# cheukwaylee/ORB_SLAM2_detailed_comments

Hardware: AMD Instinct MI355X
Metric: frames/sec ORB extract+match (1000 kp, 640x480) (higher is better)
Workload: dtype u8; 1 GPU; synthetic 640x480 mono stream, nFeatures=1000, 8 levels, scale 1.2, FAST 20/7, extract+match(t vs t-1), batch 1024 frames/GPU resident in HBM, 1 pipelines/GPU; parallelism=single GPU

## Files before the change

orb_slam2_detailed_comments_amd/csrc/orbx_api.cpp:

```cpp
#include <hip/hip_runtime.h>
#include <dlfcn.h>
#include <cstdio>
#include <cstdlib>
#include <cstring>
#include <string>
#include <vector>
#include <algorithm>
#include "orbx_internal.h"
#include "orbx_launch.h"
#include "orbx_gate.h"

static thread_local std::string g_last_error;
static orbx_status fail(orbx_status s, const std::string &msg) {
    g_last_error = msg;
    return s;
}
#define HIPCHK(expr)                                                                              \
    do {                                                                                          \
        hipError_t _e = (expr);                                                                   \
        if (_e != hipSuccess)                                                                     \
            return fail(ORBX_HIP_ERROR, std::string(#expr) + ": " + hipGetErrorString(_e));      \
    } while (0)

struct ProfPair { hipEvent_t a, b; int kid; };

struct orbx_handle {
    orbx_params p;
    OrbxTables tab;
    OrbxGeom geom;
    DGeom dg;
    bool host_only = false, configured = false;
    int dev = 0;
    hipStream_t own_stream = nullptr, stream = nullptr;
    hipStream_t side_stream = nullptr;
    hipEvent_t ev_fork = nullptr, ev_join = nullptr;
    hipEvent_t ev_stereo = nullptr;
    int fork_level = 0;
    int fork_group = 0;
    int pipeline = 2;
    bool pipe_head = true;
    bool fast_room = false;
    hipEvent_t ev_pipe[ORBX_PIPE_MAX] = {};
    uint8_t *d_pyr = nullptr, *d_blur = nullptr;
    OrbxCell *d_cells = nullptr;
    OrbxFastGroup *d_groups = nullptr;
    bool resize_legacy = false;
    int match_kernel = 0;
    int fast_stop = 0;
    int fast_lcap = 640;
    OrbxTap *d_taps = nullptr;
    uint2 *d_dense = nullptr;
    int *d_cand_count = nullptr, *d_lvl_count = nullptr, *d_status = nullptr;
    uint32_t *d_lvl_kp = nullptr;
    float *d_lvl_angle = nullptr;
    uint16_t *d_knode = nullptr;
    int max_cw = 0, max_ch = 0, ncap = 0, lds_keys = 0, lds_keys_few = 0;
    uint8_t *st_in[2] = {nullptr, nullptr}; size_t d_in_bytes = 0;
    orbx_keypoint *st_kps[2] = {nullptr, nullptr}; uint8_t *st_desc[2] = {nullptr, nullptr}; int *st_cnt[2] = {nullptr, nullptr};
    int out_cap = 0, stage_chunk = 0;
    int *pin_stat = nullptr; size_t pin_stat_ints = 0;
    hipStream_t s_in = nullptr;
    hipEvent_t ev_in[2] = {nullptr, nullptr}, ev_done[2] = {nullptr, nullptr}, ev_out[2] = {nullptr, nullptr};
    int last_batch = 0;
    int mk_w = 0, mk_h = 0, mk_total = 0;
    void *d_match_ws = nullptr; size_t match_ws_bytes = 0;
    uint32_t *d_gate_items = nullptr; size_t gate_items_cap = 0;
    uint8_t *pin = nullptr; size_t pin_bytes = 0;
    size_t gate_guess = 4096;
    uint8_t *d_scratch = nullptr; size_t scratch_bytes = 0, scratch_used = 0;
    uint2 *d_rect = nullptr; int rect_w = 0, rect_h = 0;
    int input_format = ORBX_FMT_GRAY8;
    bool blur_valid = false;
    uint32_t prof_mask = 0;
    std::vector<ProfPair> pending;
    std::vector<hipEvent_t> pool;
    float ms[ORBX_K_COUNT] = {0};
    int launches[ORBX_K_COUNT] = {0};
};

orbx_status orbx_fail(orbx_status s, const std::string &msg) { return fail(s, msg); }
int orbx_handle_fp_mode(const orbx_handle *h) { return h->p.fp_mode; }

static const char *k_names[ORBX_K_COUNT] = {"k_pyr_l0", "k_pyr_resize", "k_fast_rows", "k_quadtree", "k_orient",
                                            "k_blur",   "k_describe",   "k_match",      "misc"};

extern "C" const char *orbx_kernel_name(int k) { return (k >= 0 && k < ORBX_K_COUNT) ? k_names[k] : "?"; }
extern "C" const char *orbx_last_error(void) { return g_last_error.c_str(); }
extern "C" int orbx_abi_version(void) { return ORBX_ABI_VERSION; }
extern "C" const char *orbx_status_string(orbx_status s) {
    switch (s) {
        case ORBX_OK: return "ok";
        case ORBX_EMPTY_IMAGE: return "empty image";
        case ORBX_BAD_ARGUMENT: return "bad argument";
        case ORBX_BAD_ASPECT: return "bad aspect ratio (nIni == 0)";
        case ORBX_CAPACITY: return "capacity exceeded";
// ... 14 lines not shown

struct Roctx {
    int (*push)(const char *) = nullptr;
    int (*pop)() = nullptr;
    Roctx() {
        const char *e = getenv("ORBX_ROCTX");
        if (!e || !atoi(e)) return;
        void *lib = dlopen("librocprofiler-sdk-roctx.so", RTLD_NOW | RTLD_GLOBAL);
        if (!lib) lib = dlopen("libroctx64.so", RTLD_NOW | RTLD_GLOBAL);
        if (!lib) return;
        push = (int (*)(const char *))dlsym(lib, "roctxRangePushA");
        pop = (int (*)())dlsym(lib, "roctxRangePop");
        if (!push || !pop) push = nullptr, pop = nullptr;
    }
};
static const Roctx &roctx() { static Roctx r; return r; }

struct ProfScope {
    orbx_handle *h; int kid; bool on; hipStream_t st; hipEvent_t a = nullptr, b = nullptr; bool marked = false;
    ProfScope(orbx_handle *h_, int kid_, hipStream_t st_ = nullptr)
        : h(h_), kid(kid_), on(((h_->prof_mask >> kid_) & 1u) != 0), st(st_ ? st_ : h_->stream) {
        if (roctx().push) { roctx().push(orbx_kernel_name(kid)); marked = true; }
        if (!on) return;
        a = grab(); b = grab();
        hipEventRecord(a, st);
    }
    hipEvent_t grab() {
        if (!h->pool.empty()) { hipEvent_t e = h->pool.back(); h->pool.pop_back(); return e; }
        hipEvent_t e; hipEventCreate(&e); return e;
    }
    ~ProfScope() {
        if (marked) roctx().pop();
        if (!on) return;
        hipEventRecord(b, st);
        h->pending.push_back({a, b, kid});
    }
};

static void prof_drain(orbx_handle *h) {
    if (h->pending.empty()) return;
    hipStreamSynchronize(h->stream);
    for (auto &pp : h->pending) {
        float ms = 0;
        if (hipEventElapsedTime(&ms, pp.a, pp.b) == hipSuccess) { h->ms[pp.kid] += ms; h->launches[pp.kid]++; }
        h->pool.push_back(pp.a); h->pool.push_back(pp.b);
    }
    h->pending.clear();
}

static orbx_status pin_reserve(orbx_handle *h, size_t bytes);

static void free_geometry_buffers(orbx_handle *h) {
    hipFree(h->d_groups); h->d_groups = nullptr;
    hipFree(h->d_pyr); hipFree(h->d_blur); hipFree(h->d_cells); hipFree(h->d_taps);
    hipFree(h->d_dense); h->d_dense = nullptr;
    hipFree(h->d_cand_count); hipFree(h->d_lvl_count); hipFree(h->d_status); hipFree(h->d_lvl_kp);
    hipFree(h->d_lvl_angle); hipFree(h->d_knode);
    h->d_pyr = h->d_blur = nullptr; h->d_cells = nullptr; h->d_taps = nullptr;
    h->d_cand_count = h->d_lvl_count = h->d_status = nullptr; h->d_lvl_kp = nullptr; h->d_lvl_angle = nullptr;
    h->d_knode = nullptr;
    h->configured = false;
}

static orbx_status configure(orbx_handle *h, int width, int height) {
    if (h->configured && h->geom.width == width && h->geom.height == height) return ORBX_OK;
    if (h->host_only) return fail(ORBX_NO_DEVICE, "host-only handle (device = -2) cannot extract");
    HIPCHK(hipSetDevice(h->dev));
    if (h->configured) {
        HIPCHK(hipStreamSynchronize(h->stream));
        if (h->side_stream) HIPCHK(hipStreamSynchronize(h->side_stream));
        free_geometry_buffers(h);
    }
    const char *why = "";
    OrbxGeom g;
    orbx_status st = orbx_build_geometry(h->p, h->tab, width, height, g, &why);
    if (st != ORBX_OK) return fail(st, why);
    h->geom = g;
    const int B = h->p.max_batch, NL = h->p.nlevels;
    DGeom &d = h->dg;
    memset(&d, 0, sizeof(d));
    d.nlevels = NL; d.ncells = (int)g.cells.size(); d.kp_total = g.kp_total; d.fp_mode = h->p.fp_mode;
    d.ini_th = std::min(std::max(h->p.ini_th_fast, 0), 255);
    d.min_th = std::min(std::max(h->p.min_th_fast, 0), 255);
    d.pyr_bytes = g.pyr_bytes; d.cand_total = g.cand_total;
    for (int i = 0; i < 16; ++i) d.umax[i] = h->tab.umax[i];
    int tiles = 0;
    h->max_cw = h->max_ch = 7;
    for (const auto &c : g.cells) { h->max_cw = std::max<int>(h->max_cw, c.cw); h->max_ch = std::max<int>(h->max_ch, c.ch); }
    for (int l = 0; l < NL; ++l) {
        const OrbxLevelGeom &L = g.lv[l];
        DLevel &D = d.lv[l];
        D.pw = L.pw; D.ph = L.ph; D.pitch = L.pitch; D.sw = L.sw; D.sh = L.sh;
        D.cell_begin = L.cell_begin; D.cell_count = L.cell_count;
        D.qt_w = L.qt_w; D.qt_h = L.qt_h; D.nini = L.nini; D.hx = L.hx;
        D.nfeat = L.nfeat; D.kp_cap = L.kp_cap; D.kp_begin = L.kp_begin; D.cand_cap = L.cand_cap;
        D.tapx = L.tapx_begin; D.tapy = L.tapy_begin; D.scale = L.scale; D.size = L.size;
        D.off = L.off; D.cand_begin = L.cand_begin;
        D.blur_tx = (L.pw + 127) / 128;
        D.blur_tile_begin = tiles;
        tiles += D.blur_tx * ((L.ph + 31) / 32);
    }
    d.blur_tiles = tiles;
    h->ncap = g.node_cap;
    const size_t node_part = orbx_quadtree_smem(h->ncap, 0);
    if (node_part > 120 * 1024) return fail(ORBX_UNSUPPORTED, "nfeatures too large for the LDS quadtree node table");
    {
        const size_t want = std::min<size_t>({(size_t)4096, (size_t)g.max_cand_cap, (size_t)6 * (size_t)std::max(g.lv[0].nfeat, 1)});
        size_t keys = 0;
        auto fit_at = [&](int wg) -> size_t {
            const size_t budget = (size_t)(160 * 1024) / wg - 512;
            return budget <= node_part ? 0 : std::min<size_t>({(budget - node_part) / 6, (size_t)4096, (size_t)g.max_cand_cap});
        };
        size_t keys_few = 0;
        for (int wg = 4; wg >= 2 && keys == 0; --wg)
            if (fit_at(wg) >= want) { keys = std::max<size_t>(want, 1024); keys_few = fit_at(wg); }
        h->lds_keys_few = (int)keys_few;
        if (keys == 0 && fit_at(2) >= 1024) keys = fit_at(2);
        if (keys == 0) keys = fit_at(1);
        if (const char *e = getenv("ORBX_QT_LDS_KEYS")) keys = std::min<size_t>((size_t)std::max(atoi(e), 0), std::min<size_t>(8192, (160 * 1024 - node_part) / 6));
        h->lds_keys = (int)keys;
        if (getenv("ORBX_QT_LDS_KEYS") || h->lds_keys_few < h->lds_keys) h->lds_keys_few = h->lds_keys;
    }
    HIPCHK(orbx_quadtree_prepare(orbx_quadtree_smem(h->ncap, std::max(h->lds_keys, h->lds_keys_few))));
    if (const char *e = getenv("ORBX_RESIZE_IMPL")) h->resize_legacy = strcmp(e, "legacy") == 0;
#ifdef ORBX_TIMING_KNOBS
    if (const char *e = getenv("ORBX_FAST_STOP")) h->fast_stop = atoi(e);
#endif
    if (const char *e = getenv("ORBX_FAST_LCAP")) h->fast_lcap = std::max(64, atoi(e));
// ... 136 lines not shown
    if (inv_sigma2) memcpy(inv_sigma2, h->tab.inv_sigma2, n * sizeof(float));
    return ORBX_OK;
}
extern "C" orbx_status orbx_get_features_per_level(const orbx_handle *h, int32_t *n) {
    if (!h || !n) return fail(ORBX_BAD_ARGUMENT, "null argument");
    memcpy(n, h->tab.nfeat, h->p.nlevels * sizeof(int32_t));
    return ORBX_OK;
}
extern "C" orbx_status orbx_get_umax(const orbx_handle *h, int32_t *umax16) {
    if (!h || !umax16) return fail(ORBX_BAD_ARGUMENT, "null argument");
    memcpy(umax16, h->tab.umax, 16 * sizeof(int32_t));
    return ORBX_OK;
}
extern "C" int orbx_max_keypoints(orbx_handle *h, int width, int height) {
    if (!h || width <= 0 || height <= 0) return -(int)ORBX_BAD_ARGUMENT;
    if (h->configured && h->geom.width == width && h->geom.height == height) return h->geom.kp_total;
    if (h->mk_w == width && h->mk_h == height) return h->mk_total;
    OrbxGeom g; const char *why = "";
    const orbx_status st = orbx_build_geometry(h->p, h->tab, width, height, g, &why);
    if (st != ORBX_OK) { g_last_error = why; return -(int)st; }
    h->mk_w = width; h->mk_h = height; h->mk_total = g.kp_total;
    return g.kp_total;
}

static inline int orbx_fmt_channels(int fmt) { return fmt == ORBX_FMT_GRAY8 ? 1 : (fmt == ORBX_FMT_RGB8 || fmt == ORBX_FMT_BGR8) ? 3 : 4; }
extern "C" orbx_status orbx_set_rectification(orbx_handle *h, const float *map_x, const float *map_y, int width, int height) {
    if (!h || h->host_only) return fail(h ? ORBX_NO_DEVICE : ORBX_BAD_ARGUMENT, "no device handle");
    HIPCHK(hipSetDevice(h->dev));
    HIPCHK(hipStreamSynchronize(h->stream));
    hipFree(h->d_rect); h->d_rect = nullptr; h->rect_w = h->rect_h = 0;
    if (!map_x && !map_y) return ORBX_OK;
    if (!map_x || !map_y || width <= 0 || height <= 0) return fail(ORBX_BAD_ARGUMENT, "bad rectification maps");
    if (h->input_format != ORBX_FMT_GRAY8) return fail(ORBX_BAD_ARGUMENT, "rectification needs 8-bit gray input");
    std::vector<uint2> t((size_t)width * height);
    for (size_t i = 0; i < t.size(); ++i) {
        const int sx = (int)lrintf(map_x[i] * 32.f), sy = (int)lrintf(map_y[i] * 32.f);
        const int ix = std::min(std::max(sx >> 5, -32768), 32767), iy = std::min(std::max(sy >> 5, -32768), 32767);
        t[i].x = (uint32_t)(uint16_t)(int16_t)ix | ((uint32_t)(uint16_t)(int16_t)iy << 16);
        t[i].y = (uint32_t)(((sy & 31) << 5) | (sx & 31));
    }
    HIPCHK(hipMalloc(&h->d_rect, t.size() * sizeof(uint2)));
    HIPCHK(hipMemcpyAsync(h->d_rect, t.data(), t.size() * sizeof(uint2), hipMemcpyHostToDevice, h->stream));
    HIPCHK(hipStreamSynchronize(h->stream));
    h->rect_w = width; h->rect_h = height;
    return ORBX_OK;
}
extern "C" orbx_status orbx_set_input_format(orbx_handle *h, int pixel_format) {
    if (!h) return fail(ORBX_BAD_ARGUMENT, "null handle");
    if (pixel_format < ORBX_FMT_GRAY8 || pixel_format > ORBX_FMT_BGRA8) return fail(ORBX_BAD_ARGUMENT, "unknown pixel format");
    if (h->d_rect && pixel_format != ORBX_FMT_GRAY8) return fail(ORBX_BAD_ARGUMENT, "rectification needs 8-bit gray input");
    h->input_format = pixel_format;
    return ORBX_OK;
}
static orbx_status run_chunk(orbx_handle *h, int B, const uint8_t *d_imgs, int W, int H, int stride,
                             int64_t frame_stride, orbx_keypoint *d_kps, uint8_t *d_desc, int32_t *d_counts,
                             int32_t *d_status, int cap) {
    const DGeom &g = h->dg;
    hipStream_t s = h->stream;
    const int NL = g.nlevels;
    if (h->d_rect && (h->rect_w != W || h->rect_h != H))
        return fail(ORBX_BAD_ARGUMENT, "rectification maps were set for another image size (raw and rectified size must agree)");
    const int ngroups = (int)h->geom.fast_groups.size();
    auto pyramid = [&](hipStream_t st, int f0, int b, int l_end) {
        const uint8_t *im = d_imgs + (int64_t)f0 * frame_stride;
        uint8_t *pyr = h->d_pyr + (size_t)f0 * h->geom.pyr_bytes;
        int32_t *stp = d_status + f0;
        int *cc = h->d_cand_count + (size_t)f0 * NL;
        { ProfScope ps(h, ORBX_K_PYR_L0, st);
          if (h->d_rect) {
              orbx_launch_pyr_l0_remap(st, g, b, im, W, H, stride, frame_stride, pyr, h->d_rect, stp, cc);
          } else if (h->input_format == ORBX_FMT_GRAY8) {
              orbx_launch_pyr_l0(st, g, b, im, W, H, stride, frame_stride, pyr, stp, cc);
          } else {
              const int nch = (h->input_format == ORBX_FMT_RGB8 || h->input_format == ORBX_FMT_BGR8) ? 3 : 4;
              const bool rgb = h->input_format == ORBX_FMT_RGB8 || h->input_format == ORBX_FMT_RGBA8;
              orbx_launch_pyr_l0_color(st, g, b, im, W, H, stride, frame_stride, pyr, nch, rgb ? 0 : 2, rgb ? 2 : 0, stp, cc);
          } }
        for (int l = 1; l < l_end; ++l) {
            ProfScope ps(h, ORBX_K_PYR_RESIZE, st);
            orbx_launch_pyr_resize(st, g, b, l, h->d_taps, pyr, h->geom.lv[l].narrow_taps && !h->resize_legacy);
        }
    };
    auto fast = [&](hipStream_t st, int f0, int b, int g0, int ng, int lds_floor) {
        ProfScope ps(h, ORBX_K_FAST, st);
        orbx_launch_fast_rows(st, g, b, h->d_cells, h->d_groups + g0, ng, h->d_pyr + (size_t)f0 * h->geom.pyr_bytes,
                              h->d_dense + (size_t)f0 * g.cand_total, h->d_cand_count + (size_t)f0 * NL, d_status + f0, h->max_ch,
                              h->fast_lcap, h->fast_stop, lds_floor);
    };
    auto finish = [&](int f0, int b) {
        { ProfScope ps(h, ORBX_K_QUADTREE);
          orbx_launch_quadtree(s, g, b, h->d_dense + (size_t)f0 * g.cand_total, h->d_cand_count + (size_t)f0 * NL,
                               h->d_lvl_kp + (size_t)f0 * g.kp_total, h->d_lvl_count + (size_t)f0 * NL, d_status + f0,
                               h->d_knode + (size_t)f0 * g.cand_total, h->ncap, (long long)b * NL >= 1024 ? h->lds_keys : h->lds_keys_few, 0, NL); }
        { ProfScope ps(h, ORBX_K_DESC);
          orbx_launch_describe(s, g, b, h->d_pyr + (size_t)f0 * h->geom.pyr_bytes, h->d_lvl_kp + (size_t)f0 * g.kp_total,
                               h->d_lvl_count + (size_t)f0 * NL, h->d_lvl_angle + (size_t)f0 * g.kp_total, d_kps + (int64_t)f0 * cap,
                               d_desc + (int64_t)f0 * cap * 32, d_counts + f0, d_status + f0, cap); }
    };
    h->blur_valid = false;
    const int S = h->pipeline > 1 && B >= ORBX_PIPE_MIN_FRAMES && __builtin_popcount(h->prof_mask) <= 1 ? h->pipeline : 1;
    if (S > 1) {
        int off[ORBX_PIPE_MAX + 1];
        const int units = h->pipe_head ? 2 * S - 1 : S;
        off[0] = 0;
        for (int k = 0; k + 1 < S; ++k) {
            const int share = (int)((long long)B * (h->pipe_head && k > 0 ? 2 : 1) / units);
            off[k + 1] = off[k] + std::max(8, share & ~7);
        }
        off[S] = B;
        hipStream_t s2 = h->side_stream;
        if (hipEventRecord(h->ev_fork, s) != hipSuccess || hipStreamWaitEvent(s2, h->ev_fork, 0) != hipSuccess)
            { hipStreamSynchronize(s2); return fail(ORBX_HIP_ERROR, "pipeline fork event"); }
        for (int k = 0; k < S; ++k) {
            pyramid(s2, off[k], off[k + 1] - off[k], NL);
            if (hipEventRecord(h->ev_pipe[k], s2) != hipSuccess)
                { hipStreamSynchronize(s2); return fail(ORBX_HIP_ERROR, "pipeline event"); }
        }
        const int floor = h->fast_room ? ORBX_LDS_PER_CU / ORBX_FAST_PIPE_WAVES : 0;
        for (int k = 0; k < S; ++k) {
            if (hipStreamWaitEvent(s, h->ev_pipe[k], 0) != hipSuccess)
                { hipStreamSynchronize(s2); return fail(ORBX_HIP_ERROR, "pipeline event wait"); }
            fast(s, off[k], off[k + 1] - off[k], 0, ngroups, floor);
            finish(off[k], off[k + 1] - off[k]);
        }
        hipError_t e = hipGetLastError();
        if (e != hipSuccess) { hipStreamSynchronize(s2); return fail(ORBX_HIP_ERROR, std::string("kernel launch: ") + hipGetErrorString(e)); }
        h->last_batch = B;
        return ORBX_OK;
    }
    const bool fork = h->fork_level > 0 && (long long)B * ngroups >= 16384;
    pyramid(s, 0, B, fork ? h->fork_level : NL);
    if (fork) {
        hipStream_t s2 = h->side_stream;
        if (hipEventRecord(h->ev_fork, s) != hipSuccess || hipStreamWaitEvent(s2, h->ev_fork, 0) != hipSuccess)
            return fail(ORBX_HIP_ERROR, "fork event");
        for (int l = h->fork_level; l < NL; ++l) {
            ProfScope ps(h, ORBX_K_PYR_RESIZE, s2);
            orbx_launch_pyr_resize(s2, g, B, l, h->d_taps, h->d_pyr, h->geom.lv[l].narrow_taps && !h->resize_legacy);
        }
        fast(s2, 0, B, h->fork_group, ngroups - h->fork_group, 0);
        fast(s, 0, B, 0, h->fork_group, 0);
        if (hipEventRecord(h->ev_join, s2) != hipSuccess || hipStreamWaitEvent(s, h->ev_join, 0) != hipSuccess)
            { hipStreamSynchronize(s2); return fail(ORBX_HIP_ERROR, "join event"); }
    } else {
        fast(s, 0, B, 0, ngroups, 0);
    }
    finish(0, B);
    hipError_t e = hipGetLastError();
    if (e != hipSuccess) return fail(ORBX_HIP_ERROR, std::string("kernel launch: ") + hipGetErrorString(e));
    h->last_batch = B;
    return ORBX_OK;
}

extern "C" orbx_status orbx_extract_batch_device(orbx_handle *h, int nframes, const uint8_t *d_imgs, int width,
                                                 int height, int stride, int64_t frame_stride, orbx_keypoint *d_kps,
                                                 uint8_t *d_desc, int32_t *d_counts, int32_t *d_status, int cap) {
    if (!h) return fail(ORBX_BAD_ARGUMENT, "null handle");
    if (!d_imgs || width <= 0 || height <= 0 || nframes <= 0) return fail(ORBX_EMPTY_IMAGE, "empty image");
    if (!d_kps || !d_desc || !d_counts || cap <= 0 || stride < width * orbx_fmt_channels(h->input_format)) return fail(ORBX_BAD_ARGUMENT, "bad output buffers / stride");
    orbx_status st = configure(h, width, height);
    if (st != ORBX_OK) return st;
    HIPCHK(hipSetDevice(h->dev));
    const int MB = h->p.max_batch;
    for (int f0 = 0; f0 < nframes; f0 += MB) {
        const int B = std::min(MB, nframes - f0);
        int32_t *stp = d_status ? d_status + f0 : h->d_status;
        st = run_chunk(h, B, d_imgs + (int64_t)f0 * frame_stride, width, height, stride, frame_stride,
                       d_kps + (int64_t)f0 * cap, d_desc + (int64_t)f0 * cap * 32, d_counts + f0, stp, cap);
        if (st != ORBX_OK) return st;
    }
    return ORBX_OK;
}

static orbx_status ensure_staging(orbx_handle *h, size_t in_bytes, int cap, int chunk) {
    if (in_bytes > h->d_in_bytes || cap > h->out_cap || chunk > h->stage_chunk) {
        HIPCHK(hipStreamSynchronize(h->stream));
        const size_t inb = std::max(in_bytes, h->d_in_bytes);
        const int c = std::max(cap, h->out_cap), ch = std::max(chunk, h->stage_chunk);
        for (int s = 0; s < 2; ++s) {
            hipFree(h->st_in[s]); hipFree(h->st_kps[s]);
            h->st_in[s] = nullptr; h->st_kps[s] = nullptr; h->st_desc[s] = nullptr; h->st_cnt[s] = nullptr;
        }
        h->d_in_bytes = 0; h->out_cap = 0; h->stage_chunk = 0;
        for (int s = 0; s < 2; ++s) {
            HIPCHK(hipMalloc(&h->st_in[s], inb));
            const size_t kb = (size_t)ch * c * sizeof(orbx_keypoint), db = (size_t)ch * c * 32;
            uint8_t *blk = nullptr;
            HIPCHK(hipMalloc(&blk, kb + db + (size_t)2 * ch * sizeof(int)));
            h->st_kps[s] = (orbx_keypoint *)blk; h->st_desc[s] = blk + kb; h->st_cnt[s] = (int *)(blk + kb + db);
        }
        h->d_in_bytes = inb; h->out_cap = c; h->stage_chunk = ch;
    }
    if (!h->s_in) {
        int lo = 0, hi = 0;
        HIPCHK(hipDeviceGetStreamPriorityRange(&lo, &hi));
        HIPCHK(hipStreamCreateWithPriority(&h->s_in, hipStreamNonBlocking, hi));
        for (int s = 0; s < 2; ++s) {
            HIPCHK(hipEventCreateWithFlags(&h->ev_in[s], hipEventDisableTiming));
            HIPCHK(hipEventCreateWithFlags(&h->ev_done[s], hipEventDisableTiming));
            HIPCHK(hipEventCreateWithFlags(&h->ev_out[s], hipEventDisableTiming));
        }
    }
    return ORBX_OK;
}

extern "C" void *orbx_host_alloc(size_t bytes) {
    void *p = nullptr;
    if (bytes == 0 || hipHostMalloc(&p, bytes, hipHostMallocDefault) != hipSuccess) { (void)hipGetLastError(); return nullptr; }
    return p;
}
extern "C" void orbx_host_free(void *p) { if (p) hipHostFree(p); }

extern "C" orbx_status orbx_extract_batch(orbx_handle *h, int nframes, const uint8_t *imgs, int width, int height,
                                          int stride, int64_t frame_stride, orbx_keypoint *kps, uint8_t *desc,
                                          int32_t *counts, int cap) {
    if (!h) return fail(ORBX_BAD_ARGUMENT, "null handle");
    if (!imgs || width <= 0 || height <= 0 || nframes <= 0) return fail(ORBX_EMPTY_IMAGE, "empty image");
    if (!kps || !desc || !counts || cap <= 0 || stride < width * orbx_fmt_channels(h->input_format)) return fail(ORBX_BAD_ARGUMENT, "bad output buffers / stride");
    orbx_status st = configure(h, width, height);
    if (st != ORBX_OK) return st;
    HIPCHK(hipSetDevice(h->dev));
// ... 84 lines not shown
            memcpy(desc + (int64_t)i * cap * 32, pin_out + kb + (size_t)i * cap * 32, (size_t)n * 32);
            counts[i] = cnt[i];
            if (cnt[nframes + i] != ORBX_OK) worst = (orbx_status)cnt[nframes + i];
        }
        if (worst != ORBX_OK) return fail(worst, "a frame exceeded the keypoint / candidate capacity");
        return ORBX_OK;
    }
    HIPCHK(upload(0));
    for (int c = 0; c < nchunks; ++c) {
        const int s = c & 1, f0 = c * chunk, B = std::min(chunk, nframes - f0);
        if (piped) HIPCHK(hipStreamWaitEvent(h->stream, h->ev_in[s], 0));
        st = run_chunk(h, B, h->st_in[s], width, height, stride, (int64_t)fbytes, zk ? zk + (int64_t)f0 * cap : h->st_kps[s],
                       zk ? zd + (int64_t)f0 * cap * 32 : h->st_desc[s], h->st_cnt[s], h->st_cnt[s] + chunk, cap);
        if (st != ORBX_OK) { hipStreamSynchronize(h->stream); hipStreamSynchronize(sin); return st; }
        if (piped) HIPCHK(hipEventRecord(h->ev_done[s], h->stream));
        if (c >= 1) HIPCHK(download_enqueue(c - 1));
        if (c + 1 < nchunks) HIPCHK(upload(c + 1));
        if (piped && c >= 1) HIPCHK(hipEventSynchronize(h->ev_out[(c - 1) & 1]));
    }
    HIPCHK(download_enqueue(nchunks - 1));
    HIPCHK(hipStreamSynchronize(sout));
    if (piped) HIPCHK(hipStreamSynchronize(h->stream));
    collect();
    if (worst != ORBX_OK) return fail(worst, "a frame exceeded the keypoint / candidate capacity");
    return ORBX_OK;
}

extern "C" orbx_status orbx_extract(orbx_handle *h, const uint8_t *img, int width, int height, int stride,
                                    orbx_keypoint *kps, uint8_t *desc, int cap, int *n) {
    if (!n) return fail(ORBX_BAD_ARGUMENT, "null count pointer");
    int32_t cnt = 0;
    orbx_status st = orbx_extract_batch(h, 1, img, width, height, stride, (int64_t)stride * height, kps, desc, &cnt, cap);
    if (st == ORBX_OK || st == ORBX_CAPACITY) *n = cnt;
    return st;
}

static orbx_status check_level(orbx_handle *h, int frame, int level) {
    if (!h) return fail(ORBX_BAD_ARGUMENT, "null handle");
    if (!h->configured || h->last_batch == 0) return fail(ORBX_BAD_ARGUMENT, "no frame extracted yet");
    if (level < 0 || level >= h->p.nlevels || frame < 0 || frame >= h->last_batch) return fail(ORBX_BAD_ARGUMENT, "frame/level out of range");
    return ORBX_OK;
}
extern "C" orbx_status orbx_pyramid_level_info(orbx_handle *h, int level, int *width, int *height, int *pitch) {
    orbx_status st = check_level(h, 0, level);
    if (st != ORBX_OK) return st;
    if (width) *width = h->geom.lv[level].pw;
    if (height) *height = h->geom.lv[level].ph;
    if (pitch) *pitch = h->geom.lv[level].pitch;
    return ORBX_OK;
}
extern "C" orbx_status orbx_pyramid_level_device(orbx_handle *h, int frame, int level, const uint8_t **d_ptr) {
    orbx_status st = check_level(h, frame, level);
    if (st != ORBX_OK) return st;
    *d_ptr = h->d_pyr + (size_t)frame * h->geom.pyr_bytes + h->geom.lv[level].off;
    return ORBX_OK;
}
static orbx_status copy_level(orbx_handle *h, const uint8_t *slab, int frame, int level, uint8_t *dst, int dst_stride) {
    orbx_status st = check_level(h, frame, level);
    if (st != ORBX_OK) return st;
    const OrbxLevelGeom &L = h->geom.lv[level];
    if (!dst || dst_stride < L.pw) return fail(ORBX_BAD_ARGUMENT, "dst / dst_stride");
    HIPCHK(hipSetDevice(h->dev));
    HIPCHK(hipStreamSynchronize(h->stream));
    HIPCHK(hipMemcpy2D(dst, dst_stride, slab + (size_t)frame * h->geom.pyr_bytes + L.off, L.pitch, L.pw, L.ph,
                       hipMemcpyDeviceToHost));
    return ORBX_OK;
}
extern "C" orbx_status orbx_pyramid_level_copy(orbx_handle *h, int frame, int level, uint8_t *dst, int dst_stride) {
    return copy_level(h, h ? h->d_pyr : nullptr, frame, level, dst, dst_stride);
}
extern "C" orbx_status orbx_debug_blur_copy(orbx_handle *h, int frame, int level, uint8_t *dst, int dst_stride) {
    orbx_status st = check_level(h, frame, level);
    if (st != ORBX_OK) return st;
    if (!h->blur_valid) {
        HIPCHK(hipSetDevice(h->dev));
        if (!h->d_blur) {
            HIPCHK(hipMalloc(&h->d_blur, (size_t)h->p.max_batch * h->geom.pyr_bytes + 256));
            HIPCHK(hipMemsetAsync(h->d_blur, 0, (size_t)h->p.max_batch * h->geom.pyr_bytes, h->stream));
        }
        { ProfScope ps(h, ORBX_K_BLUR);
          orbx_launch_blur(h->stream, h->dg, h->last_batch, h->d_pyr, h->d_blur); }
        h->blur_valid = true;
    }
    return copy_level(h, h->d_blur, frame, level, dst, dst_stride);
}

extern "C" orbx_status orbx_debug_candidates(orbx_handle *h, int frame, int level, orbx_keypoint *out, int cap, int *n) {
    orbx_status st = check_level(h, frame, level);
    if (st != ORBX_OK) return st;
    HIPCHK(hipSetDevice(h->dev));
    HIPCHK(hipStreamSynchronize(h->stream));
    const OrbxLevelGeom &L = h->geom.lv[level];
    int cnt = 0;
    HIPCHK(hipMemcpy(&cnt, h->d_cand_count + frame * h->p.nlevels + level, sizeof(int), hipMemcpyDeviceToHost));
    if (n) *n = cnt;
    const int m = std::min(cnt, L.cand_cap);
    std::vector<uint2> rec(std::max(m, 1));
    if (m > 0)
        HIPCHK(hipMemcpy(rec.data(), h->d_dense + (size_t)frame * h->geom.cand_total + L.cand_begin, (size_t)m * sizeof(uint2),
                         hipMemcpyDeviceToHost));
    for (int i = 0; i < m && i < cap; ++i) {
        orbx_keypoint k;
        k.x = (float)(rec[i].x & 0xfff); k.y = (float)((rec[i].x >> 12) & 0xfff);
        k.size = 7.f; k.angle = -1.f; k.response = (float)(rec[i].x >> 24);
        k.octave = 0; k.class_id = (int32_t)(rec[i].y & 0xffffff);
        out[i] = k;
    }
    if (cnt > L.cand_cap || m > cap) return fail(ORBX_CAPACITY, "candidate capacity");
    return ORBX_OK;
}

extern "C" orbx_status orbx_debug_level_keypoints(orbx_handle *h, int frame, int level, orbx_keypoint *out, int cap, int *n) {
    orbx_status st = check_level(h, frame, level);
    if (st != ORBX_OK) return st;
    HIPCHK(hipSetDevice(h->dev));
    HIPCHK(hipStreamSynchronize(h->stream));
    const OrbxLevelGeom &L = h->geom.lv[level];
    int cnt = 0;
    HIPCHK(hipMemcpy(&cnt, h->d_lvl_count + frame * h->p.nlevels + level, sizeof(int), hipMemcpyDeviceToHost));
    if (n) *n = cnt;
    std::vector<uint32_t> pos(std::max(cnt, 1));
    std::vector<float> ang(std::max(cnt, 1));
    if (cnt > 0) {
        HIPCHK(hipMemcpy(pos.data(), h->d_lvl_kp + (size_t)frame * h->geom.kp_total + L.kp_begin, cnt * sizeof(uint32_t), hipMemcpyDeviceToHost));
        HIPCHK(hipMemcpy(ang.data(), h->d_lvl_angle + (size_t)frame * h->geom.kp_total + L.kp_begin, cnt * sizeof(float), hipMemcpyDeviceToHost));
    }
    for (int i = 0; i < cnt && i < cap; ++i) {
        orbx_keypoint k;
        k.x = (float)((pos[i] & 0xfff) + ORBX_EDGE - 3); k.y = (float)(((pos[i] >> 12) & 0xfff) + ORBX_EDGE - 3);
        k.size = L.size; k.angle = ang[i]; k.response = (float)(pos[i] >> 24); k.octave = level; k.class_id = -1;
        out[i] = k;
    }
    if (cnt > cap) return fail(ORBX_CAPACITY, "output capacity");
    return ORBX_OK;
}

static orbx_status scratch_reserve(orbx_handle *h, size_t bytes) {
// ... 455 lines not shown
        if (nc == 0) continue;
        const uint32_t *cl = gl.list(i1);
        int bestDist = INT_MAX, bestDist2 = INT_MAX, bestIdx2 = -1;
        for (int c = 0; c < nc; ++c) {
            const int i2 = OrbxGateLists::idx(cl[c]), dist = OrbxGateLists::dist(cl[c]);
            if (matchedDist[i2] <= dist) continue;
            if (dist < bestDist) { bestDist2 = bestDist; bestDist = dist; bestIdx2 = i2; }
            else if (dist < bestDist2) bestDist2 = dist;
        }
        if (bestDist <= TH_LOW_ && (float)bestDist < (float)bestDist2 * nnratio) {
            if (matches21[bestIdx2] >= 0) { matches12[matches21[bestIdx2]] = -1; nmatches--; }
            matches12[i1] = bestIdx2;
            matches21[bestIdx2] = i1;
            matchedDist[bestIdx2] = bestDist;
            nmatches++;
            if (check_orientation) {
                float rot = k1[i1].angle - k2[bestIdx2].angle;
                if (rot < 0.0) rot += 360.0f;
                int bin = (int)roundf(rot * factor);
                if (bin == HISTO) bin = 0;
                if (bin >= 0 && bin < HISTO) rotHist[bin].push_back(i1);
            }
        }
    }
    if (check_orientation) {
        int32_t sizes[30]; int i1, i2, i3;
        for (int i = 0; i < HISTO; ++i) sizes[i] = (int)rotHist[i].size();
        orbx_three_maxima(sizes, HISTO, &i1, &i2, &i3);
        for (int i = 0; i < HISTO; ++i) {
            if (i == i1 || i == i2 || i == i3) continue;
            for (int idx1 : rotHist[i])
                if (matches12[idx1] >= 0) { matches12[idx1] = -1; nmatches--; }
        }
    }
    for (int i = 0; i < n1; ++i)
        if (matches12[i] >= 0) { prev_matched[2 * i] = k2[matches12[i]].x; prev_matched[2 * i + 1] = k2[matches12[i]].y; }
    *nmatches_out = nmatches;
    return ORBX_OK;
}

extern "C" orbx_status orbx_stereo_match(orbx_handle *hl, orbx_handle *hr, int frame_left, int frame_right,
                                         const orbx_keypoint *kl, const uint8_t *dl, int nl, const orbx_keypoint *kr,
                                         const uint8_t *dr, int nr, float mb, float mbf, float *u_right, float *depth,
                                         int *nmatches_out) {
    if (!hl || !hr || hl->host_only || hr->host_only) return fail(ORBX_BAD_ARGUMENT, "two device handles are required");
    if (nl < 0 || nr < 0 || nr > 65535 || (nl > 0 && (!kl || !dl || !u_right || !depth)) || (nr > 0 && (!kr || !dr)) ||
        !(mb > 0.f))
        return fail(ORBX_BAD_ARGUMENT, "bad argument");
    orbx_status st = check_level(hl, frame_left, 0);
    if (st != ORBX_OK) return st;
    st = check_level(hr, frame_right, 0);
    if (st != ORBX_OK) return st;
    if (hl->dev != hr->dev || hl->geom.width != hr->geom.width || hl->geom.height != hr->geom.height ||
        hl->p.nlevels != hr->p.nlevels || hl->p.scale_factor != hr->p.scale_factor)
        return fail(ORBX_BAD_ARGUMENT, "left and right extractor must share device, image size and pyramid parameters");
    if (nmatches_out) *nmatches_out = 0;
    if (nl == 0) return ORBX_OK;
    HIPCHK(hipSetDevice(hl->dev));
    HIPCHK(hipStreamSynchronize(hr->stream));
    OrbxStereoGeom sg;
    memset(&sg, 0, sizeof(sg));
    sg.nlevels = hl->p.nlevels; sg.nrows0 = hl->geom.lv[0].ph; sg.mb = mb; sg.mbf = mbf;
    for (int l = 0; l < sg.nlevels; ++l) {
        sg.scale[l] = hl->tab.scale[l]; sg.inv_scale[l] = hl->tab.inv_scale[l];
        sg.pw[l] = hl->geom.lv[l].pw; sg.ph[l] = hl->geom.lv[l].ph; sg.pitch[l] = hl->geom.lv[l].pitch;
        sg.off[l] = hl->geom.lv[l].off;
    }
    st = scratch_reserve(hl, pad256((size_t)nl * sizeof(orbx_keypoint)) + pad256((size_t)nl * 32) +
                                 pad256((size_t)std::max(nr, 1) * sizeof(orbx_keypoint)) + pad256((size_t)std::max(nr, 1) * 32) +
                                 3 * pad256((size_t)nl * sizeof(float)) + pad256((size_t)(sg.nrows0 + 1) * sizeof(int)) +
                                 pad256((size_t)orbx_stereo_items_per_pair(sg, std::max(nr, 1)) * sizeof(uint2)));
    if (st != ORBX_OK) return st;
    orbx_keypoint *dkl = scratch_take<orbx_keypoint>(hl, nl);
    uint8_t *ddl = scratch_take<uint8_t>(hl, (size_t)nl * 32);
    orbx_keypoint *dkr = scratch_take<orbx_keypoint>(hl, std::max(nr, 1));
    uint8_t *ddr = scratch_take<uint8_t>(hl, (size_t)std::max(nr, 1) * 32);
    float *du = scratch_take<float>(hl, nl), *dz = scratch_take<float>(hl, nl);
    int *dsad = scratch_take<int>(hl, nl);
    int *drow = scratch_take<int>(hl, (size_t)sg.nrows0 + 1);
    uint2 *ditems = scratch_take<uint2>(hl, (size_t)orbx_stereo_items_per_pair(sg, std::max(nr, 1)));
    HIPCHK(hipMemcpyAsync(dkl, kl, (size_t)nl * sizeof(orbx_keypoint), hipMemcpyHostToDevice, hl->stream));
    HIPCHK(hipMemcpyAsync(ddl, dl, (size_t)nl * 32, hipMemcpyHostToDevice, hl->stream));
    if (nr > 0) {
        HIPCHK(hipMemcpyAsync(dkr, kr, (size_t)nr * sizeof(orbx_keypoint), hipMemcpyHostToDevice, hl->stream));
        HIPCHK(hipMemcpyAsync(ddr, dr, (size_t)nr * 32, hipMemcpyHostToDevice, hl->stream));
    }
    { ProfScope ps(hl, ORBX_K_MATCH);
      orbx_launch_stereo(hl->stream, sg, dkl, ddl, nl, dkr, ddr, nr, hl->d_pyr + (size_t)frame_left * hl->geom.pyr_bytes,
                         hr->d_pyr + (size_t)frame_right * hr->geom.pyr_bytes, du, dz, dsad, drow, ditems); }
    std::vector<int> sad(nl);
    HIPCHK(hipMemcpyAsync(u_right, du, (size_t)nl * sizeof(float), hipMemcpyDeviceToHost, hl->stream));
    HIPCHK(hipMemcpyAsync(depth, dz, (size_t)nl * sizeof(float), hipMemcpyDeviceToHost, hl->stream));
    HIPCHK(hipMemcpyAsync(sad.data(), dsad, (size_t)nl * sizeof(int), hipMemcpyDeviceToHost, hl->stream));
    hipError_t e = hipStreamSynchronize(hl->stream);
    if (e != hipSuccess) return fail(ORBX_HIP_ERROR, hipGetErrorString(e));
    std::vector<std::pair<int, int>> v;
    for (int i = 0; i < nl; ++i) if (sad[i] >= 0) v.push_back({sad[i], i});
    int kept = (int)v.size();
    if (!v.empty()) {
        std::sort(v.begin(), v.end());
        const float median = (float)v[v.size() / 2].first;
        const float thDist = 1.5f * 1.4f * median;
        for (int i = (int)v.size() - 1; i >= 0; --i) {
            if ((float)v[i].first < thDist) break;
            u_right[v[i].second] = -1; depth[v[i].second] = -1; --kept;
        }
    }
    if (nmatches_out) *nmatches_out = kept;
    return ORBX_OK;
}

extern "C" orbx_status orbx_stereo_match_batch_device(orbx_handle *hl, orbx_handle *hr, int npairs, const orbx_keypoint *d_kl,
                                                      const uint8_t *d_dl, const int32_t *d_nl, const orbx_keypoint *d_kr,
                                                      const uint8_t *d_dr, const int32_t *d_nr, int cap, float mb, float mbf,
                                                      float *d_u_right, float *d_depth, int32_t *d_nmatches) {
    if (!hl || !hr || hl->host_only || hr->host_only) return fail(ORBX_BAD_ARGUMENT, "two device handles are required");
    if (npairs <= 0 || cap <= 0 || cap > 65535 || !d_kl || !d_dl || !d_nl || !d_kr || !d_dr || !d_nr || !d_u_right || !d_depth ||
        !d_nmatches || !(mb > 0.f))
        return fail(ORBX_BAD_ARGUMENT, "bad argument");
    const bool one_batch = hl == hr;
    orbx_status st = check_level(hl, (one_batch ? 2 * npairs : npairs) - 1, 0);
    if (st != ORBX_OK) return st;
    st = check_level(hr, npairs - 1, 0);
    if (st != ORBX_OK) return st;
    if (hl->dev != hr->dev || hl->geom.width != hr->geom.width || hl->geom.height != hr->geom.height ||
        hl->p.nlevels != hr->p.nlevels || hl->p.scale_factor != hr->p.scale_factor)
        return fail(ORBX_BAD_ARGUMENT, "left and right extractor must share device, image size and pyramid parameters");
    HIPCHK(hipSetDevice(hl->dev));
    const bool two_streams = hr->stream != hl->stream;
    if (two_streams) {
        HIPCHK(hipEventRecord(hr->ev_stereo, hr->stream));
        HIPCHK(hipStreamWaitEvent(hl->stream, hr->ev_stereo, 0));
    }
    OrbxStereoGeom sg;
    memset(&sg, 0, sizeof(sg));
    sg.nlevels = hl->p.nlevels; sg.nrows0 = hl->geom.lv[0].ph; sg.mb = mb; sg.mbf = mbf;
    for (int l = 0; l < sg.nlevels; ++l) {
        sg.scale[l] = hl->tab.scale[l]; sg.inv_scale[l] = hl->tab.inv_scale[l];
        sg.pw[l] = hl->geom.lv[l].pw; sg.ph[l] = hl->geom.lv[l].ph; sg.pitch[l] = hl->geom.lv[l].pitch;
        sg.off[l] = hl->geom.lv[l].off;
    }
    const size_t ipp = (size_t)orbx_stereo_items_per_pair(sg, cap);
    st = scratch_reserve(hl, pad256((size_t)npairs * cap * sizeof(int)) + pad256((size_t)npairs * (sg.nrows0 + 1) * sizeof(int)) +
                                 pad256((size_t)npairs * ipp * sizeof(uint2)));
    if (st != ORBX_OK) return st;
    int *dsad = scratch_take<int>(hl, (size_t)npairs * cap);
    int *drow = scratch_take<int>(hl, (size_t)npairs * (sg.nrows0 + 1));
    uint2 *ditems = scratch_take<uint2>(hl, (size_t)npairs * ipp);
    { ProfScope ps(hl, ORBX_K_MATCH);
      orbx_launch_stereo_batch(hl->stream, sg, npairs, cap, d_kl, d_dl, d_nl, d_kr, d_dr, d_nr, hl->d_pyr,
                               hr->d_pyr + (one_batch ? (size_t)npairs * (size_t)hl->geom.pyr_bytes : 0),
                               (long long)hl->geom.pyr_bytes, d_u_right, d_depth, dsad, d_nmatches, drow, ditems); }
    if (two_streams) {
        HIPCHK(hipEventRecord(hl->ev_stereo, hl->stream));
        HIPCHK(hipStreamWaitEvent(hr->stream, hl->ev_stereo, 0));
    }
    hipError_t e = hipGetLastError();
    if (e != hipSuccess) return fail(ORBX_HIP_ERROR, hipGetErrorString(e));
    return ORBX_OK;
}

static inline float orbx_gemm3(const float *a, const float *b, float c) {
    const float t = a[0] * b[0] + a[1] * b[1] + a[2] * b[2];
    return (float)((double)t * 1.0 + (double)c * 1.0);
}

extern "C" orbx_status orbx_search_by_projection_frame(orbx_handle *h, const orbx_frame_view *cur,
                                                       const orbx_last_frame_view *last, float th, int mono,
                                                       int check_orientation, int32_t *matched_last, int *nmatches_out) {
    if (!h || h->host_only) return fail(h ? ORBX_NO_DEVICE : ORBX_BAD_ARGUMENT, "no device handle");
    if (!cur || !last || !matched_last || !nmatches_out || cur->n < 0 || last->n < 0)
        return fail(ORBX_BAD_ARGUMENT, "bad argument");
    const int nc = cur->n, nl = last->n, HISTO = 30, TH_HIGH_ = 100;
    *nmatches_out = 0;
    for (int i = 0; i < nc; ++i) matched_last[i] = -1;
    if (nc == 0 || nl == 0) return ORBX_OK;
    if (!cur->keys_un || !cur->desc || !cur->u_right || !last->keys_un || !last->has_map_point || !last->world_pos ||
        !last->mp_desc || !last->observations)
        return fail(ORBX_BAD_ARGUMENT, "null frame field");
    const bool fma_mode = h->p.fp_mode == ORBX_FP_GCC_FMA;
    float Rcw[9], tcw[3], Rlw[9], tlw[3], twc[3], tlc[3];
    for (int r = 0; r < 3; ++r) {
        for (int c = 0; c < 3; ++c) { Rcw[3 * r + c] = cur->Tcw[4 * r + c]; Rlw[3 * r + c] = last->Tcw[4 * r + c]; }
        tcw[r] = cur->Tcw[4 * r + 3]; tlw[r] = last->Tcw[4 * r + 3];
    }
    for (int r = 0; r < 3; ++r) {
        const float t = Rcw[0 + r] * tcw[0] + Rcw[3 + r] * tcw[1] + Rcw[6 + r] * tcw[2];
        twc[r] = (float)((double)t * -1.0);
    }
    for (int r = 0; r < 3; ++r) tlc[r] = orbx_gemm3(&Rlw[3 * r], twc, tlw[r]);
    const bool bForward = tlc[2] > cur->mb && !mono, bBackward = -tlc[2] > cur->mb && !mono;
    std::vector<DGateQuery> gq((size_t)nl);
    std::vector<float> q_invz((size_t)nl, 0.f), q_u((size_t)nl, 0.f);
    for (int i = 0; i < nl; ++i) {
// ... 325 lines not shown
```

orb_slam2_detailed_comments_amd/csrc/orbx_device.h:

```cpp
#pragma once
#include <hip/hip_runtime.h>
#include <cstdint>
#include "orbx_internal.h"
#include "orbx_sincos.h"

struct DLevel {
    int pw, ph, pitch, sw, sh;
    int cell_begin, cell_count;
    int qt_w, qt_h, nini;
    float hx;
    int nfeat, kp_cap, kp_begin, cand_cap;
    int tapx, tapy;
    float scale, size;
    int blur_tile_begin, blur_tx;
    long long off;
    long long cand_begin;
};

struct DGeom {
    int nlevels, ncells, kp_total, fp_mode;
    int ini_th, min_th, blur_tiles, pad0;
    long long pyr_bytes, cand_total;
    int umax[16];
    DLevel lv[ORBX_MAX_LEVELS];
};

struct OrbxStereoGeom {
    int nlevels, nrows0;
    float mb, mbf;
    float scale[ORBX_MAX_LEVELS], inv_scale[ORBX_MAX_LEVELS];
    int pw[ORBX_MAX_LEVELS], ph[ORBX_MAX_LEVELS], pitch[ORBX_MAX_LEVELS];
    long long off[ORBX_MAX_LEVELS];
};

struct DGrid { float minx, miny, winv, hinv; };
struct DGateQuery { float x, y, r; int min_level, max_level; int frame = 0; int desc = -1; };
struct DDistRow { uint32_t q, col_begin, ncol, out_off; };
struct DBowItem { uint32_t rbeg, nrow, cbeg, ncol, rbase, cbase, obase, pad; };

#define ORBX_WAVE 64

__device__ __forceinline__ int orbx_reflect101(int i, int n) {
    if (n == 1) return 0;
    while (i < 0 || i >= n) i = i < 0 ? -i : 2 * (n - 1) - i;
    return i;
}

#define ORBX_DPP_ROW_SHR(n) (0x110 + (n))
#define ORBX_DPP_WAVE_SHL1 0x130
#define ORBX_DPP_ROW_BCAST15 0x142
#define ORBX_DPP_ROW_BCAST31 0x143
__device__ __forceinline__ uint32_t orbx_lane_above(uint32_t v) {
    return (uint32_t)__builtin_amdgcn_update_dpp(0, (int)v, ORBX_DPP_WAVE_SHL1, 0xf, 0xf, true);
}
__device__ __forceinline__ int orbx_wave_scan(int v) {
    int t = v + __builtin_amdgcn_update_dpp(0, v, ORBX_DPP_ROW_SHR(1), 0xf, 0xf, true);
    t += __builtin_amdgcn_update_dpp(0, v, ORBX_DPP_ROW_SHR(2), 0xf, 0xf, true);
    t += __builtin_amdgcn_update_dpp(0, v, ORBX_DPP_ROW_SHR(3), 0xf, 0xf, true);
    t += __builtin_amdgcn_update_dpp(0, t, ORBX_DPP_ROW_SHR(4), 0xf, 0xe, true);
    t += __builtin_amdgcn_update_dpp(0, t, ORBX_DPP_ROW_SHR(8), 0xf, 0xc, true);
    t += __builtin_amdgcn_update_dpp(0, t, ORBX_DPP_ROW_BCAST15, 0xa, 0xf, true);
    t += __builtin_amdgcn_update_dpp(0, t, ORBX_DPP_ROW_BCAST31, 0xc, 0xf, true);
    return t;
}
__device__ __forceinline__ uint32_t orbx_wave_min(uint32_t v) {
    const int I = -1;
    const int iv = (int)v;
    uint32_t t = min(v, (uint32_t)__builtin_amdgcn_update_dpp(I, iv, ORBX_DPP_ROW_SHR(1), 0xf, 0xf, false));
    t = min(t, (uint32_t)__builtin_amdgcn_update_dpp(I, iv, ORBX_DPP_ROW_SHR(2), 0xf, 0xf, false));
    t = min(t, (uint32_t)__builtin_amdgcn_update_dpp(I, iv, ORBX_DPP_ROW_SHR(3), 0xf, 0xf, false));
    t = min(t, (uint32_t)__builtin_amdgcn_update_dpp(I, (int)t, ORBX_DPP_ROW_SHR(4), 0xf, 0xe, false));
    t = min(t, (uint32_t)__builtin_amdgcn_update_dpp(I, (int)t, ORBX_DPP_ROW_SHR(8), 0xf, 0xc, false));
    t = min(t, (uint32_t)__builtin_amdgcn_update_dpp(I, (int)t, ORBX_DPP_ROW_BCAST15, 0xa, 0xf, false));
    t = min(t, (uint32_t)__builtin_amdgcn_update_dpp(I, (int)t, ORBX_DPP_ROW_BCAST31, 0xc, 0xf, false));
    return (uint32_t)__builtin_amdgcn_readlane((int)t, 63);
}
__device__ __forceinline__ int orbx_wave_sum(int v) {
    int t = v + __builtin_amdgcn_update_dpp(0, v, ORBX_DPP_ROW_SHR(1), 0xf, 0xf, true);
    t += __builtin_amdgcn_update_dpp(0, v, ORBX_DPP_ROW_SHR(2), 0xf, 0xf, true);
    t += __builtin_amdgcn_update_dpp(0, v, ORBX_DPP_ROW_SHR(3), 0xf, 0xf, true);
    t += __builtin_amdgcn_update_dpp(0, t, ORBX_DPP_ROW_SHR(4), 0xf, 0xe, true);
    t += __builtin_amdgcn_update_dpp(0, t, ORBX_DPP_ROW_SHR(8), 0xf, 0xc, true);
    t += __builtin_amdgcn_update_dpp(0, t, ORBX_DPP_ROW_BCAST15, 0xa, 0xf, true);
    t += __builtin_amdgcn_update_dpp(0, t, ORBX_DPP_ROW_BCAST31, 0xc, 0xf, true);
    return __builtin_amdgcn_readlane(t, 63);
}

__device__ __forceinline__ float orbx_fast_atan2(float y, float x) {
    const float p1 = 0.9997878412794807f * (float)(180 / 3.1415926535897932384626433832795);
    const float p3 = -0.3258083974640975f * (float)(180 / 3.1415926535897932384626433832795);
    const float p5 = 0.1555786518463281f * (float)(180 / 3.1415926535897932384626433832795);
    const float p7 = -0.04432655554792128f * (float)(180 / 3.1415926535897932384626433832795);
    float ax = fabsf(x), ay = fabsf(y);
    float a, c, c2;
    if (ax >= ay) {
        c = ay / (ax + (float)2.2204460492503131e-16);
        c2 = c * c;
        a = (((p7 * c2 + p5) * c2 + p3) * c2 + p1) * c;
// ... 11 lines not shown
```

orb_slam2_detailed_comments_amd/csrc/orbx_geometry.cpp:

```cpp
#include "orbx_internal.h"
#include <cmath>
#include <algorithm>

static inline int cv_round_f(float v) { return (int)lrintf(v); }
static inline int cv_round_d(double v) { return (int)lrint(v); }
static inline int cv_floor_f(float v) { int i = (int)v; return i - (i > v); }
static inline int cv_ceil_f(float v) { int i = (int)v; return i + (i < v); }
static inline int16_t sat16(int v) { return (int16_t)std::min(32767, std::max(-32768, v)); }
static inline int reflect101(int i, int n) {
    if (n == 1) return 0;
    while (i < 0 || i >= n) i = i < 0 ? -i : 2 * (n - 1) - i;
    return i;
}

void orbx_build_tables(const orbx_params &p, OrbxTables &t) {
    const int L = p.nlevels;
    const double sf = (double)p.scale_factor;
    t.scale[0] = 1.0f;
    t.sigma2[0] = 1.0f;
    for (int i = 1; i < L; ++i) {
        t.scale[i] = (float)((double)t.scale[i - 1] * sf);
        t.sigma2[i] = t.scale[i] * t.scale[i];
    }
    for (int i = 0; i < L; ++i) {
        t.inv_scale[i] = 1.0f / t.scale[i];
        t.inv_sigma2[i] = 1.0f / t.sigma2[i];
    }
    const float factor = (float)(1.0 / sf);
    float nd = (float)p.nfeatures * (1 - factor) / (1 - (float)std::pow((double)factor, (double)L));
    int sum = 0;
    for (int l = 0; l < L - 1; ++l) {
        t.nfeat[l] = cv_round_f(nd);
        sum += t.nfeat[l];
        nd *= factor;
    }
    t.nfeat[L - 1] = std::max(p.nfeatures - sum, 0);
    const int vmax = cv_floor_f(ORBX_HALF_PATCH * sqrtf(2.f) / 2 + 1);
    const int vmin = cv_ceil_f(ORBX_HALF_PATCH * sqrtf(2.f) / 2);
    const double hp2 = ORBX_HALF_PATCH * ORBX_HALF_PATCH;
    for (int v = 0; v <= vmax; ++v) t.umax[v] = cv_round_d(std::sqrt(hp2 - v * v));
    for (int v = ORBX_HALF_PATCH, v0 = 0; v >= vmin; --v) {
        while (t.umax[v0] == t.umax[v0 + 1]) ++v0;
        t.umax[v] = v0;
        ++v0;
    }
}

static void build_axis_taps(std::vector<OrbxTap> &out, int pdst, int dcentre, int ssize, bool horizontal) {
    const double inv_scale = (double)dcentre / ssize;
    const double scale = 1. / inv_scale;
    for (int P = 0; P < pdst; ++P) {
        const int d = reflect101(P - ORBX_EDGE, dcentre);
        float f = (float)((d + 0.5) * scale - 0.5);
        int s = cv_floor_f(f);
        f -= s;
        OrbxTap tap;
        if (horizontal) {
            if (s < 0) { f = 0; s = 0; }
            if (s >= ssize - 1) { f = 0; s = ssize - 1; }
            tap.s0 = (int16_t)s;
            tap.s1 = (int16_t)std::min(s + 1, ssize - 1);
        } else {
            tap.s0 = (int16_t)std::min(std::max(s, 0), ssize - 1);
            tap.s1 = (int16_t)std::min(std::max(s + 1, 0), ssize - 1);
        }
        tap.a0 = sat16(cv_round_f((1.f - f) * 2048));
        tap.a1 = sat16(cv_round_f(f * 2048));
        out.push_back(tap);
    }
}

orbx_status orbx_build_geometry(const orbx_params &p, const OrbxTables &t, int width, int height, OrbxGeom &g,
                                const char **why) {
    g = OrbxGeom();
    g.width = width; g.height = height; g.nlevels = p.nlevels;
    int64_t off = 0, cand_off = 0;
    int kp_off = 0;
    for (int l = 0; l < p.nlevels; ++l) {
        OrbxLevelGeom &L = g.lv[l];
        L.sw = cv_round_f((float)width * t.inv_scale[l]);
        L.sh = cv_round_f((float)height * t.inv_scale[l]);
        if (L.sw < 1 || L.sh < 1) { *why = "pyramid level collapses to zero size"; return ORBX_UNSUPPORTED; }
        L.pw = L.sw + 2 * ORBX_EDGE;
        L.ph = L.sh + 2 * ORBX_EDGE;
        L.pitch = (L.pw + 63) & ~63;
        L.off = off;
        off += (int64_t)L.pitch * L.ph;
        off = (off + 255) & ~(int64_t)255;
        L.scale = t.scale[l];
        L.size = (float)(int)(ORBX_PATCH * t.scale[l]);
        L.nfeat = t.nfeat[l];
        const int minB = ORBX_EDGE - 3;
        const int maxBX = L.pw - ORBX_EDGE + 3, maxBY = L.ph - ORBX_EDGE + 3;
        const float fw = (float)(maxBX - minB), fh = (float)(maxBY - minB);
        L.ncols = (int)(fw / 30.f);
        L.nrows = (int)(fh / 30.f);
        L.cell_begin = (int)g.cells.size();
        int nms_bound = 0;
        L.wcell = L.hcell = 0;
        if (L.ncols > 0 && L.nrows > 0) {
            L.wcell = (int)std::ceil(fw / L.ncols);
            L.hcell = (int)std::ceil(fh / L.nrows);
            if (L.wcell + 6 > 67 || L.hcell + 6 > 67) { *why = "cell larger than 67 px"; return ORBX_UNSUPPORTED; }
            int ord = 0;
            for (int i = 0; i < L.nrows; ++i) {
                const float iniY = (float)(minB + i * L.hcell);
                float maxY = iniY + L.hcell + 6;
                if (iniY >= maxBY - 3) continue;
                if (maxY > maxBY) maxY = (float)maxBY;
                for (int j = 0; j < L.ncols; ++j) {
                    const float iniX = (float)(minB + j * L.wcell);
                    float maxX = iniX + L.wcell + 6;
                    if (iniX >= maxBX - 6) continue;
                    if (maxX > maxBX) maxX = (float)maxBX;
                    OrbxCell c;
                    c.x0 = (int16_t)iniX; c.y0 = (int16_t)iniY;
                    c.cw = (int16_t)((int)maxX - (int)iniX); c.ch = (int16_t)((int)maxY - (int)iniY);
                    c.offx = (int16_t)(j * L.wcell); c.offy = (int16_t)(i * L.hcell);
                    c.level = (int16_t)l;
                    c.idx_in_level = (int16_t)ord++;
                    if (c.cw >= 7 && c.ch >= 7) {
                        int bound = ((c.cw - 6 + 1) / 2) * ((c.ch - 6 + 1) / 2);
                        if (p.max_cand_per_cell > 0) bound = std::min(bound, p.max_cand_per_cell);
                        c.slot_begin = nms_bound;
                        c.slot_cap = bound;
                        nms_bound += bound;
                        g.cells.push_back(c);
                    }
                }
            }
            if (ord > 4095) { *why = "more than 4095 FAST cells in one level"; return ORBX_UNSUPPORTED; }
        }
        L.cell_count = (int)g.cells.size() - L.cell_begin;
        L.qt_w = maxBX - minB;
        L.qt_h = maxBY - minB;
        if (L.qt_w >= 4096 || L.qt_h >= 4096) { *why = "level larger than 4095 px"; return ORBX_UNSUPPORTED; }
        L.nini = (int)roundf((float)L.qt_w / L.qt_h);
        if (L.nini <= 0) { *why = "aspect ratio < 0.5: nIni == 0"; return ORBX_BAD_ASPECT; }
        L.hx = (float)L.qt_w / L.nini;
        L.kp_cap = std::max(L.nfeat + 3, 4 * L.nini);
        L.kp_begin = kp_off;
        kp_off += L.kp_cap;
        L.cand_cap = std::max(64, nms_bound);
        L.cand_begin = cand_off;
        cand_off += L.cand_cap;
        g.node_cap = std::max(g.node_cap, (L.kp_cap + 8 + 3) & ~3);
        g.max_cand_cap = std::max(g.max_cand_cap, L.cand_cap);
        L.tapx_begin = L.tapy_begin = 0;
        L.narrow_taps = false;
        if (l > 0) {
            const OrbxLevelGeom &S = g.lv[l - 1];
            L.tapx_begin = (int)g.taps.size();
            build_axis_taps(g.taps, L.pw, L.sw, S.pw, true);
            L.tapy_begin = (int)g.taps.size();
            build_axis_taps(g.taps, L.ph, L.sh, S.ph, false);
            L.narrow_taps = true;
            for (int X = 0; X < L.pw; X += 4) {
                int lo = 0x7fff, hi = 0;
                for (int i = 0; i < 4; ++i) {
                    const OrbxTap &t = g.taps[L.tapx_begin + std::min(X + i, L.pw - 1)];
                    lo = std::min<int>(lo, t.s0); hi = std::max<int>(hi, t.s0);
                    if (t.s1 != t.s0 + 1 && t.a1 != 0) L.narrow_taps = false;
                }
                if (hi + 2 - lo > 8) L.narrow_taps = false;
            }
        }
    }
    for (size_t i = 0; i < g.cells.size();) {
        const OrbxCell &a = g.cells[i];
        OrbxFastGroup grp;
        grp.cell0 = (int32_t)i; grp.ncell = 1;
        if (i + 1 < g.cells.size()) {
            const OrbxCell &b = g.cells[i + 1];
            const bool adjacent = b.level == a.level && b.y0 == a.y0 && b.ch == a.ch && b.x0 == a.x0 + a.cw - 6 &&
                                  b.idx_in_level == a.idx_in_level + 1;
            if (adjacent && (a.cw - 6) + (b.cw - 6) <= 64 + ORBX_FAST_XCOLS) grp.ncell = 2;
        }
        g.fast_groups.push_back(grp);
        i += (size_t)grp.ncell;
    }
    g.pyr_bytes = off;
    g.cand_total = cand_off;
    g.kp_total = kp_off;
    return ORBX_OK;
}
```

orb_slam2_detailed_comments_amd/csrc/orbx_internal.h:

```cpp
#pragma once
#include <cstdint>
#include <vector>
#include "../../include/orbx.h"

#define ORBX_MAX_LEVELS 16
#define ORBX_EDGE 19
#define ORBX_HALF_PATCH 15
#define ORBX_PATCH 31
#define ORBX_NPATCH 749

struct OrbxCell {
    int16_t x0, y0, cw, ch;
    int16_t offx, offy;
    int16_t level;
    int16_t idx_in_level;
    int32_t slot_begin;
    int32_t slot_cap;
};

#define ORBX_FAST_XCOLS 2
struct OrbxFastGroup {
    int32_t cell0;
    int32_t ncell;
};
#define ORBX_LDS_PER_CU (160 * 1024)
#define ORBX_FAST_PIPE_WAVES 16
#define ORBX_PIPE_MAX 8
#define ORBX_PIPE_MIN_FRAMES 256

struct OrbxTap {
    int16_t s0, s1;
    int16_t a0, a1;
};

struct OrbxLevelGeom {
    int sw, sh;
    int pw, ph, pitch;
    int64_t off;
    int ncols, nrows, wcell, hcell;
    int cell_begin, cell_count;
    int qt_w, qt_h;
    int nini;
    float hx;
    int nfeat;
    int kp_cap;
    int kp_begin;
    int cand_cap;
    int64_t cand_begin;
    int tapx_begin, tapy_begin;
    bool narrow_taps;
    float scale;
    float size;
};

struct OrbxGeom {
    int width = 0, height = 0, nlevels = 0;
    OrbxLevelGeom lv[ORBX_MAX_LEVELS];
    std::vector<OrbxCell> cells;
    std::vector<OrbxFastGroup> fast_groups;
    std::vector<OrbxTap> taps;
    int64_t pyr_bytes = 0;
    int64_t cand_total = 0;
    int kp_total = 0;
    int node_cap = 0;
    int max_cand_cap = 0;
};

struct OrbxTables {
    float scale[ORBX_MAX_LEVELS], inv_scale[ORBX_MAX_LEVELS], sigma2[ORBX_MAX_LEVELS], inv_sigma2[ORBX_MAX_LEVELS];
    int nfeat[ORBX_MAX_LEVELS];
    int umax[ORBX_HALF_PATCH + 1];
};

void orbx_build_tables(const orbx_params &p, OrbxTables &t);
orbx_status orbx_build_geometry(const orbx_params &p, const OrbxTables &t, int width, int height, OrbxGeom &g,
                                const char **why);
```

orb_slam2_detailed_comments_amd/csrc/orbx_kernels.hip:

```cpp
#include "orbx_device.h"
#include "../../include/orbx_pattern_data.h"

#define L0_ROWS 8
#ifndef L0_FF
#define L0_FF 1
#endif
#ifndef RR_FF
#define RR_FF 1
#endif
#ifndef QT_FF
#define QT_FF 1
#endif
__global__ __launch_bounds__(256) void k_pyr_l0(DGeom g, const uint8_t *__restrict__ imgs, int W, int H, int stride,
                                                long long frame_stride, uint8_t *__restrict__ pyr, int xe,
                                                int *__restrict__ status, int *__restrict__ cand_cursor) {
    const DLevel &L = g.lv[0];
#if L0_FF
    const int f = blockIdx.x, bx = blockIdx.y, by = blockIdx.z, nbx = gridDim.y;
#else
    const int f = blockIdx.z, bx = blockIdx.x, by = blockIdx.y, nbx = gridDim.x;
#endif
    if (bx == 0 && by == 0 && threadIdx.y == 0) {
        if (threadIdx.x == 0) status[f] = 0;
        if ((int)threadIdx.x < g.nlevels) cand_cursor[f * g.nlevels + threadIdx.x] = 0;
    }
    const int Y0 = (by * 4 + threadIdx.y) * L0_ROWS;
    if (Y0 >= L.ph) return;
    const uint8_t *img = imgs + (long long)f * frame_stride;
    uint8_t *dst = pyr + (long long)f * g.pyr_bytes + L.off;
    if (bx + 1 < nbx) {
        const int X = 32 + (bx * 64 + threadIdx.x) * 16;
        if (X >= xe) return;
        uint4 v[L0_ROWS];
#pragma unroll
        for (int r = 0; r < L0_ROWS; ++r) {
            const int Y = min(Y0 + r, L.ph - 1);
            const uint8_t *sp = img + (long long)orbx_reflect101(Y - ORBX_EDGE, H) * stride + (X - ORBX_EDGE);
            const uint32_t m = (uint32_t)((unsigned long long)sp & 3ull);
            const uint32_t *ap = (const uint32_t *)(sp - m);
            const uint32_t q0 = ap[0], q1 = ap[1], q2 = ap[2], q3 = ap[3], q4 = ap[4];
            v[r] = make_uint4(__builtin_amdgcn_alignbyte(q1, q0, m), __builtin_amdgcn_alignbyte(q2, q1, m),
                              __builtin_amdgcn_alignbyte(q3, q2, m), __builtin_amdgcn_alignbyte(q4, q3, m));
        }
#pragma unroll
        for (int r = 0; r < L0_ROWS; ++r)
            if (Y0 + r < L.ph) *(uint4 *)(dst + (long long)(Y0 + r) * L.pitch + X) = v[r];
    } else {
        const int e = threadIdx.x;
        const int X = e < 8 ? 4 * e : xe + 4 * (e - 8);
        if (X >= L.pitch) return;
#pragma unroll
        for (int r = 0; r < L0_ROWS; ++r) {
            const int Y = Y0 + r;
            if (Y >= L.ph) break;
            const uint8_t *src = img + (long long)orbx_reflect101(Y - ORBX_EDGE, H) * stride;
            uint32_t w = 0;
#pragma unroll
            for (int i = 0; i < 4; ++i) {
                const int x = X + i;
                const uint32_t p = x < L.pw ? src[orbx_reflect101(x - ORBX_EDGE, W)] : 0u;
                w |= p << (8 * i);
            }
            *(uint32_t *)(dst + (long long)Y * L.pitch + X) = w;
        }
    }
}

__global__ __launch_bounds__(256) void k_pyr_l0_color(DGeom g, const uint8_t *__restrict__ imgs, int W, int H, int stride,
                                                      long long frame_stride, uint8_t *__restrict__ pyr, int nch,
                                                      int r_off, int b_off, int *__restrict__ status, int *__restrict__ cand_cursor) {
    const DLevel &L = g.lv[0];
    const int X = (blockIdx.x * 64 + threadIdx.x) * 4;
    const int Y = blockIdx.y * 4 + threadIdx.y;
    const int f = blockIdx.z;
    if (blockIdx.x == 0 && blockIdx.y == 0 && threadIdx.y == 0) {
        if (threadIdx.x == 0) status[f] = 0;
        if ((int)threadIdx.x < g.nlevels) cand_cursor[f * g.nlevels + threadIdx.x] = 0;
    }
    if (X >= L.pw || Y >= L.ph) return;
    const uint8_t *src = imgs + (long long)f * frame_stride + (long long)orbx_reflect101(Y - ORBX_EDGE, H) * stride;
    uint32_t v = 0;
#pragma unroll
    for (int i = 0; i < 4; ++i) {
        const int x = X + i;
        uint32_t p = 0;
        if (x < L.pw) {
            const uint8_t *px = src + (long long)orbx_reflect101(x - ORBX_EDGE, W) * nch;
            p = (uint32_t)(px[r_off] * 4899 + px[1] * 9617 + px[b_off] * 1868 + 8192) >> 14;
        }
        v |= p << (8 * i);
    }
    *(uint32_t *)(pyr + (long long)f * g.pyr_bytes + L.off + (long long)Y * L.pitch + X) = v;
}

__global__ __launch_bounds__(256) void k_pyr_l0_remap(DGeom g, const uint8_t *__restrict__ imgs, int W, int H, int stride,
                                                      long long frame_stride, uint8_t *__restrict__ pyr,
                                                      const uint2 *__restrict__ rect, int *__restrict__ status,
                                                      int *__restrict__ cand_cursor) {
    const DLevel &L = g.lv[0];
    const int X = (blockIdx.x * 64 + threadIdx.x) * 4;
    const int Y = blockIdx.y * 4 + threadIdx.y;
    const int f = blockIdx.z;
    if (blockIdx.x == 0 && blockIdx.y == 0 && threadIdx.y == 0) {
        if (threadIdx.x == 0) status[f] = 0;
        if ((int)threadIdx.x < g.nlevels) cand_cursor[f * g.nlevels + threadIdx.x] = 0;
    }
    if (X >= L.pw || Y >= L.ph) return;
    const uint8_t *src = imgs + (long long)f * frame_stride;
    const uint2 *mrow = rect + (long long)orbx_reflect101(Y - ORBX_EDGE, H) * W;
    uint32_t v = 0;
#pragma unroll
    for (int i = 0; i < 4; ++i) {
        const int x = X + i;
        uint32_t p = 0;
        if (x < L.pw) {
            const uint2 m = mrow[orbx_reflect101(x - ORBX_EDGE, W)];
            const int ix = (int)(short)(m.x & 0xffffu), iy = (int)(short)(m.x >> 16);
            const uint32_t fx = m.y & 31u, fy = (m.y >> 5) & 31u;
            const bool x0 = ix >= 0 && ix < W, x1 = ix + 1 >= 0 && ix + 1 < W, y0 = iy >= 0 && iy < H, y1 = iy + 1 >= 0 && iy + 1 < H;
            const uint8_t *r0 = src + (long long)iy * stride + ix, *r1 = r0 + stride;
            const uint32_t p00 = (x0 && y0) ? r0[0] : 0u, p01 = (x1 && y0) ? r0[1] : 0u, p10 = (x0 && y1) ? r1[0] : 0u,
                           p11 = (x1 && y1) ? r1[1] : 0u;
            const uint32_t acc = __umul24((32u - fx) * (32u - fy) * 32u, p00) + __umul24(fx * (32u - fy) * 32u, p01) +
                                 __umul24((32u - fx) * fy * 32u, p10) + __umul24(fx * fy * 32u, p11);
            p = (acc + (1u << 14)) >> 15;
        }
        v |= p << (8 * i);
    }
    *(uint32_t *)(pyr + (long long)f * g.pyr_bytes + L.off + (long long)Y * L.pitch + X) = v;
}

struct __attribute__((packed, aligned(1))) orbx_uint2_u { uint32_t x, y; };
struct __attribute__((packed, aligned(1))) orbx_uint3_u { uint32_t x, y, z; };
__device__ __forceinline__ uint2 orbx_load8(const void *p) { const orbx_uint2_u v = *(const orbx_uint2_u *)p; return make_uint2(v.x, v.y); }
struct __attribute__((aligned(4))) orbx_uint3_a { uint32_t x, y, z; };
typedef unsigned short orbx_v2u16 __attribute__((ext_vector_type(2)));
__device__ __forceinline__ uint32_t orbx_udot2(uint32_t a, uint32_t b) {
    return __builtin_amdgcn_udot2(__builtin_bit_cast(orbx_v2u16, a), __builtin_bit_cast(orbx_v2u16, b), 0u, false);
}
#define RS_ROWS 2
__global__ __launch_bounds__(256) void k_pyr_resize(DGeom g, int level, const OrbxTap *__restrict__ taps,
                                                    uint8_t *__restrict__ pyr) {
    const DLevel &L = g.lv[level];
    const DLevel &S = g.lv[level - 1];
    const int X = (blockIdx.x * 64 + threadIdx.x) * 4;
    const int Y0 = (blockIdx.y * 4 + threadIdx.y) * RS_ROWS;
    const int f = blockIdx.z;
    if (X >= L.pw || Y0 >= L.ph) return;
    uint8_t *base = pyr + (long long)f * g.pyr_bytes;
    OrbxTap tx[4];
    int smin = 0x7fff, smax = 0;
#pragma unroll
    for (int i = 0; i < 4; ++i) {
        tx[i] = taps[L.tapx + min(X + i, L.pw - 1)];
        smin = min(smin, (int)tx[i].s0);
        smax = max(smax, (int)tx[i].s0);
    }
    OrbxTap ty[RS_ROWS];
    if (smax + 2 - smin <= 8) {
        uint32_t sel[4], wgt[4];
#pragma unroll
        for (int i = 0; i < 4; ++i) {
            const uint32_t d = (uint32_t)(tx[i].s0 - smin);
            sel[i] = d | (0x0cu << 8) | ((d + 1u) << 16) | (0x0cu << 24);
            wgt[i] = (uint32_t)(uint16_t)tx[i].a0 | ((uint32_t)(uint16_t)tx[i].a1 << 16);
        }
        uint2 u[RS_ROWS], w[RS_ROWS];
#pragma unroll
        for (int r = 0; r < RS_ROWS; ++r) {
            ty[r] = taps[L.tapy + min(Y0 + r, L.ph - 1)];
            u[r] = orbx_load8(base + S.off + (long long)ty[r].s0 * S.pitch + smin);
            w[r] = orbx_load8(base + S.off + (long long)ty[r].s1 * S.pitch + smin);
        }
#pragma unroll
        for (int r = 0; r < RS_ROWS; ++r) {
            const int Y = Y0 + r;
            if (Y >= L.ph) break;
            const uint32_t b0 = (uint32_t)ty[r].a0 & 0xfffu, b1 = (uint32_t)ty[r].a1 & 0xfffu;
            uint32_t v = 0;
#pragma unroll
            for (int i = 0; i < 4; ++i) {
                const uint32_t T0 = orbx_udot2(__builtin_amdgcn_perm(u[r].y, u[r].x, sel[i]), wgt[i]);
                const uint32_t T1 = orbx_udot2(__builtin_amdgcn_perm(w[r].y, w[r].x, sel[i]), wgt[i]);
                const uint32_t p = ((__umul24(b0, T0 >> 4) >> 16) + (__umul24(b1, T1 >> 4) >> 16) + 2u) >> 2;
                v |= p << (8 * i);
            }
            *(uint32_t *)(base + L.off + (long long)Y * L.pitch + X) = v;
        }
        return;
    }
    const int xb = smin & ~3;
    const bool windowed = smax + 1 - xb < 12;
    uint32_t u[RS_ROWS][3], w[RS_ROWS][3];
#pragma unroll
    for (int r = 0; r < RS_ROWS; ++r) {
        ty[r] = taps[L.tapy + min(Y0 + r, L.ph - 1)];
        if (windowed) {
            const uint32_t *q0 = (const uint32_t *)(base + S.off + (long long)ty[r].s0 * S.pitch + xb);
            const uint32_t *q1 = (const uint32_t *)(base + S.off + (long long)ty[r].s1 * S.pitch + xb);
            u[r][0] = q0[0]; u[r][1] = q0[1]; u[r][2] = q0[2];
            w[r][0] = q1[0]; w[r][1] = q1[1]; w[r][2] = q1[2];
        }
    }
#pragma unroll
    for (int r = 0; r < RS_ROWS; ++r) {
        const int Y = Y0 + r;
        if (Y >= L.ph) break;
        const int b0 = ty[r].a0, b1 = ty[r].a1;
        uint32_t v = 0;
        if (windowed) {
#pragma unroll
            for (int i = 0; i < 4; ++i) {
                const int idx = tx[i].s0 - xb;
                const uint32_t ulo = idx < 4 ? u[r][0] : idx < 8 ? u[r][1] : u[r][2], uhi = idx < 4 ? u[r][1] : idx < 8 ? u[r][2] : 0u;
                const uint32_t wlo = idx < 4 ? w[r][0] : idx < 8 ? w[r][1] : w[r][2], whi = idx < 4 ? w[r][1] : idx < 8 ? w[r][2] : 0u;
                const uint32_t pu = __builtin_amdgcn_alignbyte(uhi, ulo, (uint32_t)idx & 3u);
                const uint32_t pw_ = __builtin_amdgcn_alignbyte(whi, wlo, (uint32_t)idx & 3u);
                const int T0 = (int)(pu & 0xff) * tx[i].a0 + (int)((pu >> 8) & 0xff) * tx[i].a1;
                const int T1 = (int)(pw_ & 0xff) * tx[i].a0 + (int)((pw_ >> 8) & 0xff) * tx[i].a1;
                const uint32_t p = (uint32_t)((((((b0 & 0xfff) * ((T0 >> 4) & 0xffff))) >> 16) + ((((b1 & 0xfff) * ((T1 >> 4) & 0xffff))) >> 16) + 2) >> 2) & 0xffu;
                v |= p << (8 * i);
            }
        } else {
            const uint8_t *r0 = base + S.off + (long long)ty[r].s0 * S.pitch;
            const uint8_t *r1 = base + S.off + (long long)ty[r].s1 * S.pitch;
#pragma unroll
            for (int i = 0; i < 4; ++i) {
                const int T0 = r0[tx[i].s0] * tx[i].a0 + r0[tx[i].s1] * tx[i].a1;
                const int T1 = r1[tx[i].s0] * tx[i].a0 + r1[tx[i].s1] * tx[i].a1;
                const uint32_t p = (uint32_t)((((((b0 & 0xfff) * ((T0 >> 4) & 0xffff))) >> 16) + ((((b1 & 0xfff) * ((T1 >> 4) & 0xffff))) >> 16) + 2) >> 2) & 0xffu;
                v |= p << (8 * i);
            }
        }
        *(uint32_t *)(base + L.off + (long long)Y * L.pitch + X) = v;
    }
}

#ifndef RR_REVERSE
#define RR_REVERSE 1
#endif
#ifndef RR_WPB
#define RR_WPB 1
#endif
__global__ __launch_bounds__(64 * RR_WPB) void k_pyr_resize_rows(DGeom g, int level, const OrbxTap *__restrict__ taps,
                                                         uint8_t *__restrict__ pyr, int rpw) {
    const DLevel &L = g.lv[level];
    const DLevel &S = g.lv[level - 1];
    const int lane = threadIdx.x;
#if RR_FF
    const int f = blockIdx.x, bx = blockIdx.y;
    const int by = (RR_REVERSE && (level & 1)) ? (int)gridDim.z - 1 - (int)blockIdx.z : (int)blockIdx.z;
#else
    const int f = blockIdx.z, bx = blockIdx.x, by = blockIdx.y;
#endif
    const int X = (bx * 64 + lane) * 4;
    const int y_begin = __builtin_amdgcn_readfirstlane((by * RR_WPB + threadIdx.y) * rpw);
    if (y_begin >= L.ph) return;
    const int y_end = min(y_begin + rpw, L.ph);
    const bool on = X < L.pw;
    uint8_t *base = pyr + (long long)f * g.pyr_bytes;
    const uint8_t *src = base + S.off;
    uint8_t *dst = base + L.off;
    const uint32_t ldst = (uint32_t)X;
    uint32_t sel[4], wgt[4];
    int smin = 0x7fff;
    {
        const uint2 *tq = (const uint2 *)taps + L.tapx;
        uint2 t[4];
#pragma unroll
        for (int i = 0; i < 4; ++i) t[i] = tq[min(X + i, L.pw - 1)];
#pragma unroll
        for (int i = 0; i < 4; ++i) smin = min(smin, (int)(t[i].x & 0xffffu));
#pragma unroll
        for (int i = 0; i < 4; ++i) {
            const uint32_t d = (t[i].x & 0xffffu) - (uint32_t)smin;
            sel[i] = d | (0x0cu << 8) | ((d + 1u) << 16) | (0x0cu << 24);
            wgt[i] = t[i].y;
        }
    }
    const uint32_t sh = (uint32_t)(smin & 3);
    const uint32_t lsrc = (uint32_t)(smin & ~3);
    const uint2 *ty = (const uint2 *)taps + L.tapy;
#ifndef RR_R
#define RR_R 2
#endif
#define RR_H(dst, v)                                                                                                     \
    {                                                                                                                   \
        const uint32_t lo_ = __builtin_amdgcn_alignbyte((v).y, (v).x, sh), hi_ = __builtin_amdgcn_alignbyte((v).z, (v).y, sh); \
        _Pragma("unroll") for (int i = 0; i < 4; ++i)                                                                   \
            dst[i] = orbx_udot2(__builtin_amdgcn_perm(hi_, lo_, sel[i]), wgt[i]) >> 4;                                  \
    }
#define RR_V(out, h0, h1, w0, w1)                                                                                       \
    {                                                                                                                   \
        out = 0;                                                                                                        \
        _Pragma("unroll") for (int i = 0; i < 4; ++i)                                                                   \
            out |= (((__umul24(w0, h0[i]) >> 16) + (__umul24(w1, h1[i]) >> 16) + 2u) >> 2) << (8 * i);                  \
    }
    uint2 t[RR_R];
    orbx_uint3_a u[RR_R], w[RR_R];
    int pid = -1;
    uint32_t hb[2][4] = {{0, 0, 0, 0}, {0, 0, 0, 0}};
#pragma unroll
    for (int r = 0; r < RR_R; ++r) {
        t[r] = ty[min(y_begin + r, L.ph - 1)];
        u[r].x = u[r].y = u[r].z = 0;
        if (r == 0 || (int)(t[r].x & 0xffffu) != (int)(t[r - 1].x >> 16)) u[r] = *(const orbx_uint3_a *)(src + (uint32_t)((t[r].x & 0xffffu) * (uint32_t)S.pitch + lsrc));
        w[r] = *(const orbx_uint3_a *)(src + (uint32_t)((t[r].x >> 16) * (uint32_t)S.pitch + lsrc));
    }
    for (int Y = y_begin; Y < y_end; Y += RR_R) {
        uint2 ct[RR_R];
        orbx_uint3_a cu[RR_R], cw[RR_R];
#pragma unroll
        for (int r = 0; r < RR_R; ++r) { ct[r] = t[r]; cu[r] = u[r]; cw[r] = w[r]; }
        if (Y + RR_R < y_end) {
            int last = (int)(ct[RR_R - 1].x >> 16);
#pragma unroll
            for (int r = 0; r < RR_R; ++r) {
                t[r] = ty[min(Y + RR_R + r, L.ph - 1)];
                const int s0 = (int)(t[r].x & 0xffffu), s1 = (int)(t[r].x >> 16);
                if (s0 != last) u[r] = *(const orbx_uint3_a *)(src + (uint32_t)((uint32_t)s0 * (uint32_t)S.pitch + lsrc));
                w[r] = *(const orbx_uint3_a *)(src + (uint32_t)((uint32_t)s1 * (uint32_t)S.pitch + lsrc));
                last = s1;
            }
        }
#pragma unroll
        for (int r = 0; r < RR_R; ++r) {
            uint32_t (&h0)[4] = hb[r & 1], (&h1)[4] = hb[(r & 1) ^ 1];
            const int s0 = (int)(ct[r].x & 0xffffu);
            if (s0 != pid) RR_H(h0, cu[r])
            RR_H(h1, cw[r])
            uint32_t v;
            RR_V(v, h0, h1, ct[r].y & 0xfffu, (ct[r].y >> 16) & 0xfffu)
            pid = (int)(ct[r].x >> 16);
            if (on && Y + r < y_end) *(uint32_t *)(dst + (uint32_t)((uint32_t)(Y + r) * (uint32_t)L.pitch + ldst)) = v;
        }
    }
#undef RR_H
#undef RR_V
}

__device__ __forceinline__ bool orbx_arc9(uint32_t mask16) {
    uint32_t m = mask16 | (mask16 << 16);
    uint32_t a = m & (m >> 1);
    a &= a >> 2;
    a &= a >> 4;
    a &= m >> 8;
    return (a & 0xffffu) != 0;
}

__device__ __forceinline__ unsigned long long orbx_ballot(bool p) { return __builtin_amdgcn_ballot_w64(p); }
__device__ __forceinline__ int orbx_wave_rank(unsigned long long bal) {
    return __builtin_amdgcn_mbcnt_hi((uint32_t)(bal >> 32), __builtin_amdgcn_mbcnt_lo((uint32_t)bal, 0));
}
__device__ __forceinline__ void orbx_wave_sync() {
    __builtin_amdgcn_fence(__ATOMIC_RELEASE, "wavefront");
    __builtin_amdgcn_wave_barrier();
    __builtin_amdgcn_fence(__ATOMIC_ACQUIRE, "wavefront");
}

#ifndef FR_TP
#define FR_TP 76
#endif
#ifndef FR_WPS
#define FR_WPS 5
#endif
#ifndef FR_CCAP
#define FR_CCAP 512
#endif
#ifndef FR_GPW
#define FR_GPW 2
#endif
typedef unsigned short fr_u16;
typedef short fr_i16;
typedef __attribute__((address_space(3))) uint16_t fr_lds_u16;
__device__ __forceinline__ fr_u16 fr_max(fr_u16 a, fr_u16 b) { return a > b ? a : b; }
__device__ __forceinline__ fr_u16 fr_min(fr_u16 a, fr_u16 b) { return a < b ? a : b; }
__device__ __forceinline__ fr_i16 fr_smax(fr_i16 a, fr_i16 b) { return a > b ? a : b; }
__device__ __forceinline__ fr_i16 fr_smin(fr_i16 a, fr_i16 b) { return a < b ? a : b; }

static_assert(64 + ORBX_FAST_XCOLS + 6 + 3 <= FR_TP, "a cell pair's tile row must fit the LDS tile pitch");
__device__ __forceinline__ bool colx_on_mask(unsigned act) { return (act & 2u) != 0; }
struct FrCtx {
    const uint8_t *tile;
    uint8_t *score;
    uint16_t *list;
    uint16_t *corn;
    int lcap;
    int lane;
};

#ifndef FR_UNIFIED
// ... 170 lines not shown
    orbx_wave_sync();
    return ncorn;
}
#endif


struct FrCells {
    int iw0;
    int offx0, offx1, offy;
    int ord0, ord1;
    int cap0, cap1;
    uint2 *out;
    int *cursor;
    int out_cap;
};
__device__ __forceinline__ void fr_nms(const FrCtx &c, const FrCells &gc, const uint16_t *list, int n, int &ns0, int &ns1) {
    for (int e0 = 0; e0 < n; e0 += 64) {
        const int e = e0 + c.lane;
        const bool valid = e < n;
        const uint16_t code = valid ? list[e] : (uint16_t)(3 << 8);
        const int col = code & 0xff, ly = (code >> 8) & 0x7f;
        const bool second = col >= gc.iw0;
        const uint8_t *sp = c.score + (ly - 1) * FR_TP + 2 + col;
        const int sc = sp[FR_TP + 1];
        const int l0 = sp[0], l1 = sp[FR_TP], l2 = sp[2 * FR_TP];
        const int r0 = sp[2], r1 = sp[FR_TP + 2], r2 = sp[2 * FR_TP + 2];
        const int u = sp[1], dn = sp[2 * FR_TP + 1];
        const bool seam_l = col == gc.iw0, seam_r = col == gc.iw0 - 1;
        const int ml = seam_l ? 0 : max(max(l0, l1), l2), mr = seam_r ? 0 : max(max(r0, r1), r2);
        const bool keep = (int)valid & (int)(sc > max(max(ml, mr), max(u, dn)));
        const unsigned long long m = orbx_ballot(keep), msec = orbx_ballot(keep && second);
        const unsigned long long mfirst = m & ~msec;
        const int slot = second ? ns1 + orbx_wave_rank(msec) : ns0 + orbx_wave_rank(mfirst);
        const bool ok = keep && slot < (second ? gc.cap1 : gc.cap0);
        const unsigned long long mok = orbx_ballot(ok);
        if (mok != 0ull) {
            int base = 0;
            if (c.lane == 0) base = atomicAdd(gc.cursor, (int)__popcll(mok));
            base = __builtin_amdgcn_readfirstlane(base);
            const int pos = base + orbx_wave_rank(mok);
            if (ok && pos < gc.out_cap) {
                const int lx = 3 + col - (second ? gc.iw0 : 0);
                uint2 o;
                o.x = (uint32_t)(lx + (second ? gc.offx1 : gc.offx0)) | ((uint32_t)(ly + gc.offy) << 12) | ((uint32_t)sc << 24);
                o.y = ((uint32_t)(second ? gc.ord1 : gc.ord0) << 12) | ((uint32_t)ly << 6) | (uint32_t)lx;
                gc.out[pos] = o;
            }
        }
        ns0 += __popcll(mfirst);
        ns1 += __popcll(msec);
    }
}

__global__ __launch_bounds__(64, FR_WPS) void k_fast_rows(DGeom g, const OrbxCell *__restrict__ cells,
                                                          const OrbxFastGroup *__restrict__ groups,
                                                          const uint8_t *__restrict__ pyr, uint2 *__restrict__ cand,
                                                          int *__restrict__ cand_cursor, int *__restrict__ status, int rows,
                                                          int lcap, int ngroups, int gpw, int dbg_stop, int ccap) {
#ifndef ORBX_TIMING_KNOBS
    dbg_stop = 0;
#endif
    extern __shared__ __attribute__((aligned(16))) uint8_t fast_smem[];
    uint32_t *s_tile = (uint32_t *)fast_smem;
    const int map_bytes = (rows * FR_TP + 15) & ~15;
    uint8_t *s_score = fast_smem + map_bytes;
    uint16_t *s_list = (uint16_t *)(s_score + map_bytes);
    uint16_t *s_corn = s_list + lcap + 128;
    const int lane = threadIdx.x;
    const int f = blockIdx.x;
    const int g0 = blockIdx.y * gpw;
    const int ng = min(gpw, ngroups - g0);
    const int rq = (lane * 37) >> 8, dq = lane - 7 * rq;
    orbx_uint3_u tv[5];
    OrbxFastGroup grp_n = groups[g0];
    OrbxCell c0_n = cells[grp_n.cell0], c1_n = cells[grp_n.cell0 + grp_n.ncell - 1];
    const uint8_t *fbase = pyr + (long long)f * g.pyr_bytes;
#define FR_PREFETCH()                                                                                                     \
    {                                                                                                                     \
        const DLevel &Ln = g.lv[c0_n.level];                                                                             \
        const uint8_t *srcn = fbase + Ln.off;                                                                             \
        uint32_t vpitch9 = (uint32_t)(9 * Ln.pitch);                                                                      \
        asm("" : "+v"(vpitch9));                      \
        const uint32_t olast = (uint32_t)(__mul24((int)c0_n.y0 + (int)c0_n.ch - 1, Ln.pitch) + (c0_n.x0 & ~3) + 12 * dq); \
        uint32_t o = (uint32_t)(__mul24((int)c0_n.y0 + min(rq, 8), Ln.pitch) + (c0_n.x0 & ~3) + 12 * dq);                \
        _Pragma("unroll") for (int k = 0; k < 5; ++k) {                                                                   \
            tv[k] = *(const orbx_uint3_u *)(srcn + min(o, olast));                                                        \
            o += vpitch9;                                                                                                 \
        }                                                                                                                 \
    }
    FR_PREFETCH()
  for (int gi = 0; gi < ng; ++gi) {
    const OrbxFastGroup grp = grp_n;
    const OrbxCell c0 = c0_n, c1 = c1_n;
    const DLevel &L = g.lv[c0.level];
    const int tw = c1.x0 + c1.cw - c0.x0, th_rows = c0.ch;
    const int niw = tw - 6;
    const int iw0 = grp.ncell == 2 ? c0.cw - 6 : 64;
    {
        const int xa = c0.x0 & ~3;
        uint32_t *trow = s_tile + rq * (FR_TP / 4) + 3 * dq;
#pragma unroll
        for (int k = 0; k < 5; ++k) {
            if (rq < 9 && 9 * k + rq < th_rows) {
                uint32_t *d = trow + 9 * k * (FR_TP / 4);
                d[0] = tv[k].x;
                if (dq < 6) { d[1] = tv[k].y; d[2] = tv[k].z; }
            }
        }
        if (th_rows > 45) {
            const uint8_t *src = fbase + L.off + (long long)c0.y0 * L.pitch + xa + 12 * dq;
            for (int r = 45 + rq; r < th_rows; r += 9) {
                if (rq < 9) {
                    const orbx_uint3_u v = *(const orbx_uint3_u *)(src + (long long)r * L.pitch);
                    uint32_t *d = s_tile + r * (FR_TP / 4) + 3 * dq;
                    d[0] = v.x;
                    if (dq < 6) { d[1] = v.y; d[2] = v.z; }
                }
            }
        }
        for (int i = lane; i < (th_rows * (FR_TP / 4) + 3) / 4; i += 64) ((uint4 *)s_score)[i] = make_uint4(0, 0, 0, 0);
    }
    if (gi + 1 < ng) {
        grp_n = groups[g0 + gi + 1];
        c0_n = cells[grp_n.cell0]; c1_n = cells[grp_n.cell0 + grp_n.ncell - 1];
        FR_PREFETCH()
    }
    FrCtx cx;
    cx.tile = (const uint8_t *)s_tile + (c0.x0 & 3);
    cx.score = s_score;
    cx.list = s_list;
    cx.corn = s_corn;
    cx.lcap = lcap;
    cx.lane = lane;
    FrCells gc;
    gc.iw0 = iw0;
    gc.offx0 = c0.offx; gc.offx1 = c1.offx; gc.offy = c0.offy;
    gc.ord0 = c0.idx_in_level; gc.ord1 = c1.idx_in_level;
    gc.cap0 = c0.slot_cap; gc.cap1 = c1.slot_cap;
    gc.out = cand + (long long)f * g.cand_total + L.cand_begin;
    gc.cursor = cand_cursor + f * g.nlevels + c0.level;
    gc.out_cap = L.cand_cap;
    orbx_wave_sync();
    if (dbg_stop == 1) continue;
    const bool two_th = g.min_th != g.ini_th;
    const bool colv = lane < niw;
    const bool second = lane >= iw0;
    const uint8_t *pc = cx.tile + 3 + (colv ? lane : 0);
    const int yend = th_rows - 3;
    int ns0 = 0, ns1 = 0;
    unsigned act = grp.ncell == 2 ? 3u : 1u;
    for (int pass = 0; pass < 2; ++pass) {
        const int th = pass == 0 ? g.ini_th : g.min_th;
        const bool lane_on = colv && ((act >> (second ? 1 : 0)) & 1u);
        int nctot = 0;
        bool overflow = false;
        int y = 3;
        const fr_i16 thv = lane_on ? (fr_i16)th : (fr_i16)0x4000;
        int xc = 64;
        const fr_i16 thx = (colx_on_mask(act) && 3 + lane < yend) ? (fr_i16)th : (fr_i16)0x4000;
        while (y < yend || xc < niw) {
            const uint8_t *pr = pc + y * FR_TP;
            fr_u16 w0 = pr[-3 * FR_TP], w1 = pr[-2 * FR_TP], w2 = pr[-FR_TP], w3 = pr[0], w4 = pr[FR_TP], w5 = pr[2 * FR_TP], w6;
            const uint32_t list0 = (uint32_t)(uintptr_t)(fr_lds_u16 *)s_list;
            uint32_t nb = list0;
            uint32_t code = (uint32_t)((y << 8) | lane);
            const uint32_t dummy = list0 + 2u * (uint32_t)lcap + 4u * (uint32_t)lane;
            uint32_t nx0 = pr[3 * FR_TP], nx4 = pr[3], nx12 = pr[-3];
            uint32_t probe_s = 0, probe_v = 0; (void)probe_s; (void)probe_v;
#ifndef FR_WALK_IF
#define FR_WALK_IF 1
#endif
#if defined(FR_PROBE_S)
#define FR_PROBE() asm volatile("s_xor_b32 %0, %0, 1\n\ts_xor_b32 %0, %0, 1\n\ts_xor_b32 %0, %0, 1\n\ts_xor_b32 %0, %0, 1" : "+s"(probe_s));
#elif defined(FR_PROBE_V)
#define FR_PROBE() asm volatile("v_xor_b32 %0, 1, %0\n\tv_xor_b32 %0, 1, %0\n\tv_xor_b32 %0, 1, %0\n\tv_xor_b32 %0, 1, %0" : "+v"(probe_v));
#else
#define FR_PROBE()
#endif
#if FR_WALK_IF
#define FR_STORE(cnd, m, nb, dummy, code) (void)(dummy); if (cnd) *(fr_lds_u16 *)(uintptr_t)((nb) + 2u * (uint32_t)orbx_wave_rank(m)) = (uint16_t)(code);
#else
// ... 315 lines not shown
                    }
                }
            } else {
                const int pos = ctot + (int)t2[p];
                nbox0[pos] = box0[p]; nbox1[pos] = box1[p]; ncnt[pos] = cnt[p];
                nmeta[pos] = 0;
                newpos[4 * p] = (uint16_t)pos;
            }
        }
        __syncthreads();
        for (int k = tid; k < K; k += QT_THREADS) {
            const int p = knode[k];
            const int q = ((meta[p] >> 16) & 1) ? qt_quadrant(QT_KPOS(k), box0[p], box1[p]) : 0;
            knode[k] = (uint16_t)newpos[4 * p + q];
        }
        __syncthreads();
        { uint32_t *t;
          t = box0; box0 = nbox0; nbox0 = t;  t = box1; box1 = nbox1; nbox1 = t;
          t = cnt; cnt = ncnt; ncnt = t;      t = meta; meta = nmeta; nmeta = t; }
        const int new_size = ctot + nmtot;
        if (tid == 0) sh->size = new_size;
        __syncthreads();
        if (new_size >= N || new_size == size) break;
        if (!careful && new_size + 3 * nexp_total > N) careful = true;
    }
    const int size = sh->size;
    for (int p = tid; p < size; p += QT_THREADS) best[p] = 0ull;
    __syncthreads();
    for (int k = tid; k < K; k += QT_THREADS) {
        const uint2 c = cand[k];
        const unsigned long long key = ((unsigned long long)(((c.x >> 24) << 24) | (0xffffffu - (c.y & 0xffffffu))) << 32) | c.x;
        atomicMax(&best[knode[k]], key);
    }
    __syncthreads();
    const int nout = min(size, L.kp_cap);
    if (size > L.kp_cap && tid == 0) atomicMax(&status[f], (int)ORBX_CAPACITY);
    uint32_t *out = lvl_kp + (long long)f * g.kp_total + L.kp_begin;
    for (int p = tid; p < nout; p += QT_THREADS) out[p] = (uint32_t)best[p];
    if (tid == 0) lvl_count[f * g.nlevels + level] = nout;
}

__device__ __forceinline__ void orbx_slot_to_level(const DGeom &g, int slot, int &level, int &idx) {
    level = 0;
#pragma unroll
    for (int l = 1; l < ORBX_MAX_LEVELS; ++l)
        if (l < g.nlevels && slot >= g.lv[l].kp_begin) level = l;
    idx = slot - g.lv[level].kp_begin;
}

#define BL_TW 128
#define BL_TH 32
#define BL_SD ((BL_TW + 8) / 4)
#define BL_ROWS (BL_TH + 6)
__global__ __launch_bounds__(256) void k_blur(DGeom g, const uint8_t *__restrict__ pyr, uint8_t *__restrict__ blur) {
    __shared__ uint32_t s_src[BL_ROWS * BL_SD];
    __shared__ __attribute__((aligned(8))) uint16_t s_h[BL_ROWS * BL_TW];
    const int tid = threadIdx.x, f = blockIdx.y;
    int level = 0;
    for (int l = 0; l < g.nlevels; ++l)
        if ((int)blockIdx.x >= g.lv[l].blur_tile_begin) level = l;
    const DLevel &L = g.lv[level];
    const int t = blockIdx.x - L.blur_tile_begin;
    const int ty = t / L.blur_tx, tx = t - ty * L.blur_tx;
    const int X0 = tx * BL_TW, Y0 = ty * BL_TH;
    const uint8_t *img = pyr + (long long)f * g.pyr_bytes + L.off;
    for (int i = tid; i < BL_ROWS * BL_SD; i += 256) {
        const int r = i / BL_SD, d = i - r * BL_SD;
        const int sy = orbx_reflect101(Y0 + r - 3, L.ph);
        const int x = X0 - 4 + 4 * d;
        const uint8_t *row = img + (long long)sy * L.pitch;
        uint32_t v;
        if (x >= 0 && x + 3 < L.pw) {
            v = *(const uint32_t *)(row + x);
        } else {
            v = 0;
#pragma unroll
            for (int k = 0; k < 4; ++k) v |= (uint32_t)row[orbx_reflect101(x + k, L.pw)] << (8 * k);
        }
        s_src[i] = v;
    }
    __syncthreads();
    for (int i = tid; i < BL_ROWS * (BL_TW / 4); i += 256) {
        const int r = i >> 5, q = i & 31;
        const uint32_t *w = s_src + r * BL_SD + q;
        const uint32_t w0 = w[0], w1 = w[1], w2 = w[2];
        int b[12];
#pragma unroll
        for (int k = 0; k < 4; ++k) {
            b[k] = (w0 >> (8 * k)) & 0xff; b[4 + k] = (w1 >> (8 * k)) & 0xff; b[8 + k] = (w2 >> (8 * k)) & 0xff;
        }
        uint32_t h[4];
#pragma unroll
        for (int j = 0; j < 4; ++j)
            h[j] = 18 * (b[j + 1] + b[j + 7]) + 34 * (b[j + 2] + b[j + 6]) + 49 * (b[j + 3] + b[j + 5]) + 55 * b[j + 4];
        uint2 o;
        o.x = h[0] | (h[1] << 16);
        o.y = h[2] | (h[3] << 16);
        *(uint2 *)(s_h + r * BL_TW + 4 * q) = o;
    }
    __syncthreads();
    const int cg = tid & 31, rg = tid >> 5;
    const int X = X0 + 4 * cg;
    if (X >= L.pw) return;
    const int wv = L.pw & ~3;
    const float k0 = 55.f / 65536.f, k1 = 49.f / 65536.f, k2 = 34.f / 65536.f, k3 = 18.f / 65536.f;
    int hh[10][4];
#pragma unroll
    for (int r = 0; r < 10; ++r) {
        const uint2 v = *(const uint2 *)(s_h + (rg * 4 + r) * BL_TW + 4 * cg);
        hh[r][0] = v.x & 0xffff; hh[r][1] = v.x >> 16; hh[r][2] = v.y & 0xffff; hh[r][3] = v.y >> 16;
    }
    uint8_t *out = blur + (long long)f * g.pyr_bytes + L.off;
#pragma unroll
    for (int j = 0; j < 4; ++j) {
        const int Y = Y0 + rg * 4 + j;
        if (Y >= L.ph) break;
        uint32_t outv = 0;
#pragma unroll
        for (int i = 0; i < 4; ++i) {
            const int r0 = hh[j + 3][i], r1 = hh[j + 2][i] + hh[j + 4][i], r2 = hh[j + 1][i] + hh[j + 5][i],
                      r3 = hh[j][i] + hh[j + 6][i];
            int o;
            if (X + i < wv) {
                float s0 = (float)r0 * k0 + 0.f;
                s0 = s0 + (float)r1 * k1;
                s0 = s0 + (float)r2 * k2;
                s0 = s0 + (float)r3 * k3;
                o = (int)__builtin_rintf(s0);
            } else {
                o = (55 * r0 + 49 * r1 + 34 * r2 + 18 * r3 + (1 << 15)) >> 16;
            }
            o = min(max(o, 0), 255);
            outv |= (uint32_t)o << (8 * i);
        }
        *(uint32_t *)(out + (long long)Y * L.pitch + X) = outv;
    }
}

__constant__ int4 c_pattern_lane[64];
__constant__ uint32_t c_orient_w[64][12];
__constant__ uint32_t c_blur_b[3][64][4];

#ifndef DS_ORDER
#define DS_ORDER 1
#endif
#define DS_R 21
#define DS_W (2 * DS_R + 1)
#define DS_PP 44
#define DS_HC 40
#ifndef DS_COLFIRST
#define DS_COLFIRST 1
#endif
#ifndef DS_ALIAS
#define DS_ALIAS 1
#endif
#ifndef DS_MFMA
#define DS_MFMA 1
#endif
#define DS_VC 44
#define DS_VR 40
#ifndef DS_WPB
#define DS_WPB 1
#endif
#ifndef DS_WPS
#define DS_WPS 7
// ... 27 lines not shown
    __shared__ __attribute__((aligned(16))) uint16_t s_h[DS_WPB][DS_VR * DS_VC];
#else
    __shared__ uint32_t s_patch[DS_WPB][DS_W * DS_PP / 4 + 4];
    __shared__ __attribute__((aligned(16))) uint16_t s_h[DS_WPB][DS_COLFIRST ? DS_VR * DS_VC : DS_W * DS_HC];
#endif
    const int lane = threadIdx.x & 63, wv_id = __builtin_amdgcn_readfirstlane(threadIdx.x >> 6);
#if DS_ORDER == 1
    const int f = blockIdx.y * 8 + (blockIdx.x & 7);
    const int oi = (blockIdx.x >> 3) * DS_WPB + wv_id;
    if (f >= nframes) return;
#else
    const int f = blockIdx.x;
    const int oi = blockIdx.y * DS_WPB + wv_id;
#endif
    const int *lc = lvl_count + f * g.nlevels;
    int total = 0, level = 0, slot = oi;
#ifndef DS_LEVELS8
#define DS_LEVELS8 1
#endif
    if (DS_LEVELS8 && g.nlevels == 8) {
        const int4 ca = *(const int4 *)lc, cb = *(const int4 *)(lc + 4);
        const int cnt[8] = {ca.x, ca.y, ca.z, ca.w, cb.x, cb.y, cb.z, cb.w};
        int base = 0;
#pragma unroll
        for (int l = 0; l < 8; ++l) {
            if (oi >= total) { level = l; base = total; }
            total += cnt[l];
        }
        slot = g.lv[level].kp_begin + (oi - base);
    } else {
#pragma unroll
    for (int l = 0; l < ORBX_MAX_LEVELS; ++l) {
        if (l < g.nlevels) {
            if (oi >= total) { level = l; slot = g.lv[l].kp_begin + (oi - total); }
            total += lc[l];
        }
    }
    }
    if (oi == 0 && lane == 0) {
        counts[f] = min(total, cap);
        if (total > cap) atomicMax(&status[f], (int)ORBX_CAPACITY);
    }
    if (oi >= min(total, cap) || dbg_stop == 4) return;
#if DS_COLFIRST && DS_ALIAS
    uint32_t *patch = (uint32_t *)s_h[wv_id];
#else
    uint32_t *patch = s_patch[wv_id];
#endif
    uint16_t *hrow = s_h[wv_id];
    const uint32_t pos = lvl_kp[(long long)f * g.kp_total + slot];
    const int4 pat = c_pattern_lane[lane];
    const DLevel &L = g.lv[level];
    const int x = (int)(pos & 0xfff) + (ORBX_EDGE - 3), y = (int)((pos >> 12) & 0xfff) + (ORBX_EDGE - 3);
    const uint8_t *img = pyr + (long long)f * g.pyr_bytes + L.off;
    const int px0 = x - DS_R, py0 = y - DS_R;
    const int xa = px0 & ~3;
    const bool interior = px0 >= 0 && py0 >= 0 && xa + 48 <= L.pitch && x + DS_R < L.pw && y + DS_R < L.ph;
    {
        if (interior) {
            const int dq = lane & 3, rq = lane >> 2;
            const uint32_t shift = (uint32_t)(px0 & 3);
            const uint8_t *p0 = img + (__mul24(py0, L.pitch) + xa + 12 * dq);
            orbx_uint3_u tv[3];
#pragma unroll
            for (int k = 0; k < 3; ++k) tv[k] = *(const orbx_uint3_u *)(p0 + __mul24(min(16 * k + rq, DS_W - 1), L.pitch));
#pragma unroll
            for (int k = 0; k < 3; ++k) {
                const uint32_t nxt = orbx_lane_above(tv[k].x);
                const int r = 16 * k + rq;
                if (r < DS_W) {
                    uint32_t *d = patch + r * (DS_PP / 4) + 3 * dq;
                    d[0] = __builtin_amdgcn_alignbyte(tv[k].y, tv[k].x, shift);
                    d[1] = __builtin_amdgcn_alignbyte(tv[k].z, tv[k].y, shift);
                    if (dq < 3) d[2] = __builtin_amdgcn_alignbyte(nxt, tv[k].z, shift);
                }
            }
        } else {
            uint8_t *pb = (uint8_t *)patch;
            for (int i = lane; i < DS_W * DS_W; i += 64) {
                const int r = i / DS_W, c = i - r * DS_W;
                const int sy = orbx_reflect101(py0 + r, L.ph), sx = orbx_reflect101(px0 + c, L.pw);
                pb[r * DS_PP + c] = img[(long long)sy * L.pitch + sx];
            }
        }
        orbx_wave_sync();
        if (dbg_stop == 1) return;
        float angle_deg;
        {
            const int row = lane >> 1, half = lane & 1;
            const uint32_t *pr = patch + min(row + (DS_R - ORBX_HALF_PATCH), DS_W - 1) * (DS_PP / 4) + 1 + 5 * half;
            const uint4 wa = *(const uint4 *)&c_orient_w[lane][0], wb = *(const uint4 *)&c_orient_w[lane][4], wc = *(const uint4 *)&c_orient_w[lane][8];
            const uint32_t p0 = pr[0], p1 = pr[1], p2 = pr[2], p3 = pr[3], p4 = pr[4];
            uint32_t A = __builtin_amdgcn_udot4(p0, wa.x, 0u, false), S = __builtin_amdgcn_udot4(p0, wb.y, 0u, false);
            A = __builtin_amdgcn_udot4(p1, wa.y, A, false); S = __builtin_amdgcn_udot4(p1, wb.z, S, false);
            A = __builtin_amdgcn_udot4(p2, wa.z, A, false); S = __builtin_amdgcn_udot4(p2, wb.w, S, false);
            A = __builtin_amdgcn_udot4(p3, wa.w, A, false); S = __builtin_amdgcn_udot4(p3, wc.x, S, false);
            A = __builtin_amdgcn_udot4(p4, wb.x, A, false); S = __builtin_amdgcn_udot4(p4, wc.y, S, false);
            int m10 = (int)A - 16 * (int)S;
            int m01 = __mul24(row - ORBX_HALF_PATCH, (int)S);
            m10 = orbx_wave_sum(m10);
            m01 = orbx_wave_sum(m01);
            angle_deg = orbx_fast_atan2((float)m01, (float)m10);
            if (lane == 0) lvl_angle[(long long)f * g.kp_total + slot] = angle_deg;
        }
        if (dbg_stop == 2) return;
#if DS_COLFIRST && DS_MFMA
        {
            typedef int i32x4 __attribute__((ext_vector_type(4)));
            const int m = lane & 15, gq = lane >> 4;
            i32x4 A[3], Bm[3];
#pragma unroll
            for (int t = 0; t < 3; ++t) {
                const uint32_t *ap = patch + (16 * t + m) * (DS_PP / 4) + 4 * gq;
                A[t][0] = (int)(ap[0] ^ 0x80808080u); A[t][1] = (int)(ap[1] ^ 0x80808080u);
                A[t][2] = (int)(ap[2] ^ 0x80808080u); A[t][3] = (int)(ap[3] ^ 0x80808080u);
            }
#pragma unroll
            for (int j = 0; j < 3; ++j) {
                const uint4 b4 = *(const uint4 *)&c_blur_b[j][lane][0];
                Bm[j][0] = (int)b4.x; Bm[j][1] = (int)b4.y; Bm[j][2] = (int)b4.z; Bm[j][3] = (int)b4.w;
            }
            const i32x4 c0 = {128 * 257, 128 * 257, 128 * 257, 128 * 257};
            uint32_t *vo = (uint32_t *)hrow + m * (DS_VC / 2) + 2 * gq;
#pragma unroll
            for (int j = 0; j < 3; ++j) {
#pragma unroll
                for (int t = 0; t < 3; ++t) {
                    const i32x4 acc = __builtin_amdgcn_mfma_i32_16x16x64_i8(A[t], Bm[j], c0, 0, 0, 0);
                    if ((j < 2 || m < DS_W - 6 - 32) && (t < 2 || gq < 3))
                        *(uint2 *)(vo + (16 * j) * (DS_VC / 2) + 8 * t) =
                            make_uint2((uint32_t)acc[0] | ((uint32_t)acc[1] << 16), (uint32_t)acc[2] | ((uint32_t)acc[3] << 16));
                }
            }
        }
#elif DS_COLFIRST
// ... 469 lines not shown
    if (qi0 < NQ) po[qi0] = make_uint2(best0, second0);
    if (qi1 < NQ) po[qi1] = make_uint2(best1, second1);
}

__global__ __launch_bounds__(256) void k_match_merge(const int *__restrict__ nq, const uint2 *__restrict__ partial,
                                                     int *__restrict__ best_idx, int *__restrict__ best_dist,
                                                     int *__restrict__ second_dist, int out_stride, int nsplit) {
    const int pr = blockIdx.y, qi = blockIdx.x * 256 + threadIdx.x;
    if (qi >= min(nq[pr], out_stride)) return;
    uint32_t best = 0xffffffffu, second = 0xffffffffu;
    for (int k = 0; k < nsplit; ++k) {
        const uint2 p = partial[((long long)pr * nsplit + k) * out_stride + qi];
        second = min(min(second, p.y), max(best, p.x));
        best = min(best, p.x);
    }
    const long long o = (long long)pr * out_stride + qi;
    best_idx[o] = best == 0xffffffffu ? -1 : (int)(best & 0xfffffu);
    best_dist[o] = best == 0xffffffffu ? 0x7fffffff : (int)(best >> 20);
    second_dist[o] = second == 0xffffffffu ? 0x7fffffff : (int)(second >> 20);
}

__global__ __launch_bounds__(256) void k_hamming_matrix(const uint8_t *__restrict__ q, int nq,
                                                        const uint8_t *__restrict__ t, int nt,
                                                        uint16_t *__restrict__ dist) {
    const long long i = (long long)blockIdx.x * 256 + threadIdx.x;
    if (i >= (long long)nq * nt) return;
    const int qi = (int)(i / nt), ti = (int)(i - (long long)qi * nt);
    const uint4 *qp = (const uint4 *)q + 2 * qi, *tp = (const uint4 *)t + 2 * ti;
    const uint4 qa = qp[0], qb = qp[1], ta = tp[0], tb = tp[1];
    dist[i] = (uint16_t)(__popc(qa.x ^ ta.x) + __popc(qa.y ^ ta.y) + __popc(qa.z ^ ta.z) + __popc(qa.w ^ ta.w) +
                         __popc(qb.x ^ tb.x) + __popc(qb.y ^ tb.y) + __popc(qb.z ^ tb.z) + __popc(qb.w ^ tb.w));
}

__device__ __forceinline__ uint32_t st_row16_min(uint32_t v) {
    v = min(v, (uint32_t)__builtin_amdgcn_update_dpp((int)v, (int)v, 0x121, 0xf, 0xf, false));
    v = min(v, (uint32_t)__builtin_amdgcn_update_dpp((int)v, (int)v, 0x122, 0xf, 0xf, false));
    v = min(v, (uint32_t)__builtin_amdgcn_update_dpp((int)v, (int)v, 0x124, 0xf, 0xf, false));
    v = min(v, (uint32_t)__builtin_amdgcn_update_dpp((int)v, (int)v, 0x128, 0xf, 0xf, false));
    return v;
}
__device__ __forceinline__ uint32_t st_row16_sum(uint32_t v) {
    v += (uint32_t)__builtin_amdgcn_update_dpp((int)v, (int)v, 0x121, 0xf, 0xf, false);
    v += (uint32_t)__builtin_amdgcn_update_dpp((int)v, (int)v, 0x122, 0xf, 0xf, false);
    v += (uint32_t)__builtin_amdgcn_update_dpp((int)v, (int)v, 0x124, 0xf, 0xf, false);
    v += (uint32_t)__builtin_amdgcn_update_dpp((int)v, (int)v, 0x128, 0xf, 0xf, false);
    return v;
}
#define ST_KPB 16
__device__ __forceinline__ void orbx_stereo_body(const OrbxStereoGeom &sg, const orbx_keypoint *__restrict__ kL,
                                                 const uint8_t *__restrict__ dL, int nL,
                                                 const orbx_keypoint *__restrict__ kR,
                                                 const uint8_t *__restrict__ dR, int nR,
                                                 const uint8_t *__restrict__ pyrL, const uint8_t *__restrict__ pyrR,
                                                 float *__restrict__ uRight, float *__restrict__ depth,
                                                 int *__restrict__ sad, const int *__restrict__ row_begin,
                                                 const uint2 *__restrict__ row_items) {
    const int l16 = threadIdx.x & 15;
    const int iL = blockIdx.x * ST_KPB + (threadIdx.x >> 4);
    bool act = iL < nL;
    float uL = 0.f, vL = 0.f;
    int levelL = 0;
    if (act) { const orbx_keypoint kp = kL[iL]; uL = kp.x; vL = kp.y; levelL = kp.octave; }
    if (act && l16 == 0) { uRight[iL] = -1.0f; depth[iL] = -1.0f; sad[iL] = -1; }
    const long long row = (long long)vL;
    act = act && row >= 0 && row < sg.nrows0;
    const float maxD = sg.mbf / sg.mb, minD = 0.f;
    const float minU = uL - maxD, maxU = uL - minD;
    act = act && !(maxU < 0);
    uint4 qa = make_uint4(0, 0, 0, 0), qb = qa;
    if (act) { const uint4 *qp = (const uint4 *)(dL + (long long)iL * 32); qa = qp[0]; qb = qp[1]; }
    uint32_t best = 0xffffffffu;
    if (row_begin) {
        int j = 0, j1 = 0;
        if (act) { j = row_begin[row] + l16; j1 = row_begin[row + 1]; }
        for (; j < j1; j += 16) {
            const uint2 it = row_items[j];
            const int iR = (int)(it.y & 0xffffu), octR = (int)(it.y >> 16);
            const float xR = __uint_as_float(it.x);
            const bool cand = (int)(octR >= levelL - 1) & (int)(octR <= levelL + 1) & (int)(xR >= minU) & (int)(xR <= maxU);
            if (cand) {
                const uint4 *tp = (const uint4 *)(dR + (long long)iR * 32);
                const uint4 ta = tp[0], tb = tp[1];
                const uint32_t d = __popc(qa.x ^ ta.x) + __popc(qa.y ^ ta.y) + __popc(qa.z ^ ta.z) + __popc(qa.w ^ ta.w) +
                                   __popc(qb.x ^ tb.x) + __popc(qb.y ^ tb.y) + __popc(qb.z ^ tb.z) + __popc(qb.w ^ tb.w);
                if (d < 100u) best = min(best, (d << 16) | (uint32_t)iR);
            }
        }
    } else {
        for (int iR = act ? l16 : nR; iR < nR; iR += 16) {
            const orbx_keypoint kr = kR[iR];
            const float r = 2.0f * sg.scale[kr.octave];
            const int maxr = (int)ceilf(kr.y + r), minr = (int)floorf(kr.y - r);
            const bool cand = (int)(row >= minr) & (int)(row <= maxr) & (int)(kr.octave >= levelL - 1) &
                              (int)(kr.octave <= levelL + 1) & (int)(kr.x >= minU) & (int)(kr.x <= maxU);
            if (cand) {
                const uint4 *tp = (const uint4 *)(dR + (long long)iR * 32);
                const uint4 ta = tp[0], tb = tp[1];
                const uint32_t d = __popc(qa.x ^ ta.x) + __popc(qa.y ^ ta.y) + __popc(qa.z ^ ta.z) + __popc(qa.w ^ ta.w) +
                                   __popc(qb.x ^ tb.x) + __popc(qb.y ^ tb.y) + __popc(qb.z ^ tb.z) + __popc(qb.w ^ tb.w);
                if (d < 100u) best = min(best, (d << 16) | (uint32_t)iR);
            }
        }
    }
    best = st_row16_min(best);
    act = act && best != 0xffffffffu && (best >> 16) < 75u;
    const int bestIdxR = act ? (int)(best & 0xffffu) : 0;
    float uR0 = 0.f;
    if (act) uR0 = kR[bestIdxR].x;
    const float scaleFactor = sg.inv_scale[levelL];
    const float scaleduL = roundf(uL * scaleFactor), scaledvL = roundf(vL * scaleFactor);
    const float scaleduR0 = roundf(uR0 * scaleFactor);
    const int w = 5, Lh = 5;
    const int W = sg.pw[levelL], H = sg.ph[levelL], pitch = sg.pitch[levelL];
    const int y0 = (int)(scaledvL - w), x0 = (int)(scaleduL - w);
    act = act && !(y0 < 0 || y0 + 2 * w + 1 > H || x0 < 0 || x0 + 2 * w + 1 > W);
    const float iniu = scaleduR0 - Lh - w, endu = scaleduR0 + Lh + w + 1;
    act = act && !(iniu < 0 || endu >= W);
    uint32_t acc[11];
#pragma unroll
    for (int s = 0; s < 11; ++s) acc[s] = 0u;
    if (act) {
        const uint8_t *IL = pyrL + sg.off[levelL] + (long long)y0 * pitch + x0;
        const uint8_t *IR = pyrR + sg.off[levelL] + (long long)y0 * pitch + ((int)scaleduR0 - w);
        const uint32_t cL = IL[w * pitch + w];
        const orbx_uint3_u cw = *(const orbx_uint3_u *)(IR + w * pitch);
        uint32_t Cs[11];
#pragma unroll
        for (int s = 0; s < 11; ++s) {
            const uint32_t cwd = s < 4 ? cw.x : s < 8 ? cw.y : cw.z;
            Cs[s] = (((cwd >> (8 * (s & 3))) & 0xffu) + 511u - cL) * 0x10001u;
        }
#pragma unroll
        for (int k = 0; k < 4; ++k) {
            int q0 = l16 + 16 * k, q1 = q0 + 64;
            if (q1 >= 121) q1 = 60;
            const int y_0 = q0 / 11, x_0 = q0 - 11 * y_0, y_1 = q1 / 11, x_1 = q1 - 11 * y_1;
            const uint32_t L0 = IL[y_0 * pitch + x_0], L1 = IL[y_1 * pitch + x_1];
            const orbx_uint3_u r0 = *(const orbx_uint3_u *)(IR + y_0 * pitch + x_0 - Lh);
            const orbx_uint3_u r1 = *(const orbx_uint3_u *)(IR + y_1 * pitch + x_1 - Lh);
            const uint32_t A0 = L0 | (L1 << 16);
#pragma unroll
            for (int s = 0; s < 11; ++s) {
                const uint32_t lo = s < 4 ? r0.x : s < 8 ? r0.y : r0.z, hi = s < 4 ? r1.x : s < 8 ? r1.y : r1.z;
                const uint32_t sel = (uint32_t)(s & 3) | (0x0cu << 8) | ((uint32_t)(4 + (s & 3)) << 16) | (0x0cu << 24);
                const uint32_t B = __builtin_amdgcn_perm(hi, lo, sel) + 0x01ff01ffu;
                acc[s] = __builtin_amdgcn_sad_u16(A0 + Cs[s], B, acc[s]);
            }
        }
    }
#pragma unroll
    for (int s = 0; s < 11; ++s) acc[s] = st_row16_sum(acc[s]);
    if (!act || l16 != 0) return;
    int bestDistS = 0x7fffffff, bestinc = 0;
#pragma unroll
    for (int s = 0; s < 11; ++s)
        if ((int)acc[s] < bestDistS) { bestDistS = (int)acc[s]; bestinc = s - Lh; }
    if (bestinc == -Lh || bestinc == Lh) return;
    float dist1 = 0.f, dist2 = 0.f, dist3 = 0.f;
#pragma unroll
    for (int s = 1; s < 10; ++s)
        if (s - Lh == bestinc) { dist1 = (float)(int)acc[s - 1]; dist2 = (float)(int)acc[s]; dist3 = (float)(int)acc[s + 1]; }
    const float deltaR = (dist1 - dist3) / (2.0f * (dist1 + dist3 - 2.0f * dist2));
    if (deltaR < -1 || deltaR > 1) return;
    float bestuR = sg.scale[levelL] * ((float)scaleduR0 + (float)bestinc + deltaR);
    float disparity = uL - bestuR;
    if (disparity >= minD && disparity < maxD) {
        if (disparity <= 0) { disparity = (float)0.01; bestuR = (float)((double)uL - 0.01); }
        depth[iL] = sg.mbf / disparity;
        uRight[iL] = bestuR;
        sad[iL] = bestDistS;
    }
}

__global__ __launch_bounds__(256) void k_stereo(OrbxStereoGeom sg, const orbx_keypoint *__restrict__ kL,
                                                const uint8_t *__restrict__ dL, int nL,
                                                const orbx_keypoint *__restrict__ kR,
                                                const uint8_t *__restrict__ dR, int nR,
                                                const uint8_t *__restrict__ pyrL, const uint8_t *__restrict__ pyrR,
                                                float *__restrict__ uRight, float *__restrict__ depth,
                                                int *__restrict__ sad, const int *__restrict__ row_begin,
                                                const uint2 *__restrict__ row_items) {
    orbx_stereo_body(sg, kL, dL, nL, kR, dR, nR, pyrL, pyrR, uRight, depth, sad, row_begin, row_items);
}
__global__ __launch_bounds__(256) void k_stereo_batch(OrbxStereoGeom sg, const orbx_keypoint *__restrict__ kL,
                                                      const uint8_t *__restrict__ dL, const int *__restrict__ nL,
                                                      const orbx_keypoint *__restrict__ kR,
                                                      const uint8_t *__restrict__ dR, const int *__restrict__ nR, int cap,
                                                      const uint8_t *__restrict__ pyrL, const uint8_t *__restrict__ pyrR,
                                                      long long pyr_bytes, float *__restrict__ uRight,
                                                      float *__restrict__ depth, int *__restrict__ sad,
                                                      const int *__restrict__ row_begin, const uint2 *__restrict__ row_items,
                                                      int items_per_pair) {
    const long long p = blockIdx.y;
    orbx_stereo_body(sg, kL + p * cap, dL + p * cap * 32, min(nL[p], cap), kR + p * cap, dR + p * cap * 32, min(nR[p], cap),
                     pyrL + p * pyr_bytes, pyrR + p * pyr_bytes, uRight + p * cap, depth + p * cap, sad + p * cap,
                     row_begin ? row_begin + p * (sg.nrows0 + 1) : nullptr, row_items ? row_items + p * items_per_pair : nullptr);
}
#define ST_MAX_ROWS 4096
__global__ __launch_bounds__(1024) void k_stereo_rows(OrbxStereoGeom sg, const orbx_keypoint *__restrict__ kR,
                                                      const int *__restrict__ nR, int cap, int *__restrict__ row_begin,
                                                      uint2 *__restrict__ row_items, int items_per_pair, int n_direct) {
    __shared__ int s_cnt[ST_MAX_ROWS + 1];
    __shared__ int s_part[1024];
    const long long p = blockIdx.x;
    const int t = threadIdx.x, n = nR ? min(nR[p], cap) : n_direct, rows = sg.nrows0;
    const orbx_keypoint *k = kR + p * cap;
    for (int i = t; i <= rows; i += 1024) s_cnt[i] = 0;
    __syncthreads();
    for (int i = t; i < n; i += 1024) {
        const float r = 2.0f * sg.scale[k[i].octave];
        const int maxr = min((int)ceilf(k[i].y + r), rows - 1), minr = max((int)floorf(k[i].y - r), 0);
        for (int y = minr; y <= maxr; ++y) atomicAdd(&s_cnt[y], 1);
    }
    __syncthreads();
    const int chunk = (rows + 1023) / 1024, r0 = t * chunk, r1 = min(r0 + chunk, rows);
    int sum = 0;
    for (int y = r0; y < r1; ++y) sum += s_cnt[y];
    s_part[t] = sum;
    __syncthreads();
    for (int o = 1; o < 1024; o <<= 1) {
        const int v = t >= o ? s_part[t - o] : 0;
        __syncthreads();
        s_part[t] += v;
        __syncthreads();
    }
    int run = s_part[t] - sum;
    int *rb = row_begin + p * (rows + 1);
    for (int y = r0; y < r1; ++y) { const int c = s_cnt[y]; s_cnt[y] = run; rb[y] = run; run += c; }
    if (t == 1023) rb[rows] = s_part[1023];
    __syncthreads();
    uint2 *items = row_items + p * items_per_pair;
    for (int i = t; i < n; i += 1024) {
        const float r = 2.0f * sg.scale[k[i].octave];
        const int maxr = min((int)ceilf(k[i].y + r), rows - 1), minr = max((int)floorf(k[i].y - r), 0);
        for (int y = minr; y <= maxr; ++y) {
            const int pos = atomicAdd(&s_cnt[y], 1);
            if (pos < items_per_pair) items[pos] = make_uint2(__float_as_uint(k[i].x), (uint32_t)i | ((uint32_t)k[i].octave << 16));
        }
    }
}
__global__ __launch_bounds__(256) void k_stereo_cut(const int *__restrict__ nL, int cap, const int *__restrict__ sad,
                                                    float *__restrict__ uRight, float *__restrict__ depth,
                                                    int *__restrict__ nmatches) {
    __shared__ int hist[256];
    __shared__ int wsum[4];
    __shared__ int s_sel, s_rank, s_kept;
    const long long p = blockIdx.x;
    const int n = min(nL[p], cap), t = threadIdx.x, wv = t >> 6;
// ... 429 lines not shown
                if (col < DS_W && u >= -d && u <= d) {
                    w[lane][k] |= (uint32_t)(u + 16) << (8 * b);
                    w[lane][5 + k] |= 1u << (8 * b);
                }
            }
    }
    e = hipMemcpyToSymbol(HIP_SYMBOL(c_orient_w), w, sizeof(w));
    if (e != hipSuccess) return e;
    static uint32_t bb[3][64][4];
    memset(bb, 0, sizeof(bb));
    const int K7[7] = {18, 34, 49, 55, 49, 34, 18};
    for (int j = 0; j < 3; ++j)
        for (int lane = 0; lane < 64; ++lane)
            for (int sl = 0; sl < 16; ++sl) {
                const int k = 16 * (lane >> 4) + sl, i = k - (16 * j + (lane & 15));
                if (i >= 0 && i <= 6) bb[j][lane][sl >> 2] |= (uint32_t)K7[i] << (8 * (sl & 3));
            }
    return hipMemcpyToSymbol(HIP_SYMBOL(c_blur_b), bb, sizeof(bb));
}

size_t orbx_quadtree_smem(int ncap, int lds_keys) {
    return 128 + (size_t)ncap * (8 * 4 + 16 + 8 + 6 * 4) + 16 + (size_t)lds_keys * 6 + 16;
}

void orbx_launch_clear(hipStream_t s, int *a, int na, int *b, int nb, int *c, int nc) {
    const int n = na > nb ? (na > nc ? na : nc) : (nb > nc ? nb : nc);
    hipLaunchKernelGGL(k_clear, dim3((n + 255) / 256), dim3(256), 0, s, a, na, b, nb, c, nc);
}
void orbx_launch_pyr_l0(hipStream_t s, const DGeom &g, int B, const uint8_t *imgs, int W, int H, int stride,
                        long long frame_stride, uint8_t *pyr, int *status, int *cand_cursor) {
    const DLevel &L = g.lv[0];
    int xe = 32;
    while (xe + 1 <= W) xe += 16;
    const int icols = (xe - 32 + 1023) / 1024;
#if L0_FF
    dim3 grid(B, icols + 1, (L.ph + 4 * L0_ROWS - 1) / (4 * L0_ROWS));
#else
    dim3 grid(icols + 1, (L.ph + 4 * L0_ROWS - 1) / (4 * L0_ROWS), B);
#endif
    hipLaunchKernelGGL(k_pyr_l0, grid, dim3(64, 4), 0, s, g, imgs, W, H, stride, frame_stride, pyr, xe, status, cand_cursor);
}
void orbx_launch_pyr_l0_color(hipStream_t s, const DGeom &g, int B, const uint8_t *imgs, int W, int H, int stride,
                              long long frame_stride, uint8_t *pyr, int nch, int r_off, int b_off, int *status, int *cand_cursor) {
    const DLevel &L = g.lv[0];
    dim3 grid((L.pw + 255) / 256, (L.ph + 3) / 4, B);
    hipLaunchKernelGGL(k_pyr_l0_color, grid, dim3(64, 4), 0, s, g, imgs, W, H, stride, frame_stride, pyr, nch, r_off, b_off, status, cand_cursor);
}
void orbx_launch_pyr_l0_remap(hipStream_t s, const DGeom &g, int B, const uint8_t *imgs, int W, int H, int stride,
                              long long frame_stride, uint8_t *pyr, const uint2 *rect, int *status, int *cand_cursor) {
    const DLevel &L = g.lv[0];
    dim3 grid((L.pw + 255) / 256, (L.ph + 3) / 4, B);
    hipLaunchKernelGGL(k_pyr_l0_remap, grid, dim3(64, 4), 0, s, g, imgs, W, H, stride, frame_stride, pyr, rect, status, cand_cursor);
}
void orbx_launch_pyr_resize(hipStream_t s, const DGeom &g, int B, int level, const OrbxTap *taps, uint8_t *pyr, bool narrow) {
    const DLevel &L = g.lv[level];
    if (narrow) {
        int rpw = 16;
        while (rpw > 2 && (long long)((L.pw + 255) / 256) * ((L.ph + rpw - 1) / rpw) * B < 4096) rpw >>= 1;
#if RR_FF
        dim3 grid(B, (L.pw + 255) / 256, (L.ph + RR_WPB * rpw - 1) / (RR_WPB * rpw));
#else
        dim3 grid((L.pw + 255) / 256, (L.ph + RR_WPB * rpw - 1) / (RR_WPB * rpw), B);
#endif
        hipLaunchKernelGGL(k_pyr_resize_rows, grid, dim3(64, RR_WPB), 0, s, g, level, taps, pyr, rpw);
        return;
    }
    dim3 grid((L.pw + 255) / 256, (L.ph + 4 * RS_ROWS - 1) / (4 * RS_ROWS), B);
    hipLaunchKernelGGL(k_pyr_resize, grid, dim3(64, 4), 0, s, g, level, taps, pyr);
}
void orbx_launch_fast_rows(hipStream_t s, const DGeom &g, int B, const OrbxCell *cells, const OrbxFastGroup *groups,
                           int ngroups, const uint8_t *pyr, uint2 *cand, int *cand_cursor, int *status, int max_ch, int lcap,
                           int dbg_stop, int lds_floor) {
    if (ngroups <= 0) return;
    lcap = (max(lcap, 64) + 1) & ~1;
    const int ccap = min(lcap, FR_CCAP);
    const size_t map_bytes = ((size_t)max_ch * FR_TP + 15) & ~(size_t)15;
    const size_t need = 2 * map_bytes + (size_t)2 * lcap + 256 + (size_t)2 * ccap;
    const size_t smem = lds_floor > 0 && (size_t)lds_floor > need ? (size_t)lds_floor : need;
    const int gpw = (long long)B * ngroups >= 16384 ? FR_GPW : 1;
    hipLaunchKernelGGL(k_fast_rows, dim3(B, (ngroups + gpw - 1) / gpw), dim3(64), smem, s, g, cells, groups, pyr, cand,
                       cand_cursor, status, max_ch, lcap, ngroups, gpw, dbg_stop, ccap);
}
void orbx_launch_undistort(hipStream_t s, int B, int max_n, int cap, const double *K4, const double *k14, int identity,
                           const orbx_keypoint *kps, const int *counts, orbx_keypoint *out) {
    if (B <= 0 || max_n <= 0) return;
    DUndist u;
    u.fx = K4[0]; u.fy = K4[1]; u.cx = K4[2]; u.cy = K4[3];
    for (int i = 0; i < 14; ++i) u.k[i] = k14[i];
    u.identity = identity;
    hipLaunchKernelGGL(k_undistort, dim3((max_n + 255) / 256, B), dim3(256), 0, s, u, kps, counts, max_n, cap, out);
}
void orbx_launch_bow_transform(hipStream_t s, int B, int max_n, const int *child_begin, const uint32_t *child_ids,
                               const uint8_t *node_desc, int n_nodes, int L, const uint8_t *desc, const int *counts,
                               long long frame_stride, int levelsup, uint32_t *out_leaf, uint32_t *out_nid, int out_stride) {
    if (B <= 0 || max_n <= 0) return;
    DVoc v;
    v.child_begin = child_begin; v.child_ids = child_ids; v.desc = node_desc; v.n_nodes = n_nodes; v.L = L;
    hipLaunchKernelGGL(k_bow_transform, dim3((max_n + 15) / 16, B), dim3(256), 0, s, v, desc, counts, frame_stride, levelsup,
                       out_leaf, out_nid, out_stride);
}
static int g_qt_cus = 0;
void orbx_launch_quadtree(hipStream_t s, const DGeom &g, int B, const uint2 *dense, const int *cand_count, uint32_t *lvl_kp, int *lvl_count,
                          int *status, uint16_t *knode_glob, int ncap, int lds_keys, int level_begin, int level_count) {
    if (level_count <= 0) return;
    const size_t smem = orbx_quadtree_smem(ncap, lds_keys);
    static int forced = -1;
    if (forced < 0) { const char *e = getenv("ORBX_QT_THREADS"); forced = e ? atoi(e) : 0; }
    const long long wgs = (long long)B * level_count, cus = g_qt_cus > 0 ? g_qt_cus : 256;
    int nfeat = 0;
    for (int l = 0; l < g.nlevels; ++l) nfeat += g.lv[l].nfeat;
    int threads = wgs >= 4 * cus && nfeat <= 1600 ? 256 : wgs >= 2 * cus ? 512 : 1024;
    if (forced == 256 || forced == 512 || forced == 1024) threads = forced;
    const dim3 grid = QT_FF ? dim3(B, level_count) : dim3(level_count, B);
    if (threads == 256)
        hipLaunchKernelGGL(k_quadtree<256>, grid, dim3(256), smem, s, g, dense, cand_count, lvl_kp, lvl_count, status, knode_glob, ncap, lds_keys, level_begin);
    else if (threads == 512)
        hipLaunchKernelGGL(k_quadtree<512>, grid, dim3(512), smem, s, g, dense, cand_count, lvl_kp, lvl_count, status, knode_glob, ncap, lds_keys, level_begin);
    else
        hipLaunchKernelGGL(k_quadtree<1024>, grid, dim3(1024), smem, s, g, dense, cand_count, lvl_kp, lvl_count, status, knode_glob, ncap, lds_keys, level_begin);
}
hipError_t orbx_quadtree_prepare(size_t smem) {
    static std::mutex mu;
    static size_t cur[64] = {0};
    int dev = 0;
    hipError_t e = hipGetDevice(&dev);
    if (e != hipSuccess) return e;
    std::lock_guard<std::mutex> lock(mu);
    if (g_qt_cus == 0) { hipDeviceProp_t pr; if (hipGetDeviceProperties(&pr, dev) == hipSuccess) g_qt_cus = pr.multiProcessorCount; }
    if (dev >= 0 && dev < 64 && smem <= cur[dev]) return hipSuccess;
    e = hipFuncSetAttribute((const void *)k_quadtree<256>, hipFuncAttributeMaxDynamicSharedMemorySize, (int)smem);
    if (e == hipSuccess) e = hipFuncSetAttribute((const void *)k_quadtree<512>, hipFuncAttributeMaxDynamicSharedMemorySize, (int)smem);
    if (e == hipSuccess) e = hipFuncSetAttribute((const void *)k_quadtree<1024>, hipFuncAttributeMaxDynamicSharedMemorySize, (int)smem);
    if (e == hipSuccess && dev >= 0 && dev < 64) cur[dev] = smem;
    return e;
}
void orbx_launch_blur(hipStream_t s, const DGeom &g, int B, const uint8_t *pyr, uint8_t *blur) {
    hipLaunchKernelGGL(k_blur, dim3(g.blur_tiles, B), dim3(256), 0, s, g, pyr, blur);
}
void orbx_launch_describe(hipStream_t s, const DGeom &g, int B, const uint8_t *pyr, const uint32_t *lvl_kp,
                          const int *lvl_count, float *lvl_angle, orbx_keypoint *kps, uint8_t *desc,
                          int *counts, int *status, int cap) {
#ifdef ORBX_TIMING_KNOBS
    static int dbg_stop = -1;
    if (dbg_stop < 0) { const char *e = getenv("ORBX_DESC_STOP"); dbg_stop = e ? atoi(e) : 0; }
#else
    const int dbg_stop = 0;
#endif
#if DS_ORDER == 1
    const dim3 grid(8 * ((g.kp_total + DS_WPB - 1) / DS_WPB), (B + 7) / 8);
#else
    const dim3 grid(B, (g.kp_total + DS_WPB - 1) / DS_WPB);
#endif
    if (g.fp_mode == ORBX_FP_GCC_FMA)
        hipLaunchKernelGGL(k_describe<ORBX_FP_GCC_FMA>, grid, dim3(64 * DS_WPB), 0, s, g, pyr, lvl_kp, lvl_count, lvl_angle, kps, desc, counts, status, cap, dbg_stop, B);
    else
        hipLaunchKernelGGL(k_describe<ORBX_FP_STRICT>, grid, dim3(64 * DS_WPB), 0, s, g, pyr, lvl_kp, lvl_count, lvl_angle, kps, desc, counts, status, cap, dbg_stop, B);
}
void orbx_launch_grid_build(hipStream_t s, const DGrid &gp, int nframes, const orbx_keypoint *kps, const int *counts, int fixed_n,
                            int cap, int *cell_begin, uint16_t *items) {
    if (nframes <= 0) return;
    hipLaunchKernelGGL(k_grid_build, dim3(nframes), dim3(1024), 0, s, gp, kps, counts, fixed_n, cap, cell_begin, items);
}
void orbx_launch_gate(hipStream_t s, const DGrid &gp, const orbx_keypoint *kps, const uint8_t *desc, const int *cell_begin,
                      const uint16_t *items, const DGateQuery *q, const uint8_t *qdesc, int nq, uint2 *span, uint32_t *cursor,
                      uint32_t *out_items, uint32_t cap, int fstride) {
    if (nq <= 0) return;
    hipLaunchKernelGGL(k_gate, dim3((nq + 3) / 4), dim3(256), 0, s, gp, kps, desc, cell_begin, items, q, qdesc, nq, span, cursor,
                       out_items, cap, fstride);
}
void orbx_launch_block_dist(hipStream_t s, const uint8_t *d1, const uint8_t *d2, const DDistRow *rows, const uint32_t *col_idx,
                            int nrows, uint16_t *out) {
    if (nrows <= 0) return;
    hipLaunchKernelGGL(k_block_dist, dim3((nrows + 3) / 4), dim3(256), 0, s, d1, d2, rows, col_idx, nrows, out);
}
void orbx_launch_bow_select(hipStream_t s, bool kk, const DBowItem *items, int nitems, const uint32_t *idx, const uint8_t *desc,
                            const uint8_t *hmp, float nnratio, int words, int32_t *out) {
    if (nitems <= 0) return;
    const size_t smem = (size_t)4 * words * sizeof(uint32_t);
    if (kk) hipLaunchKernelGGL(k_bow_select<true>, dim3((nitems + 3) / 4), dim3(256), smem, s, items, nitems, idx, desc, hmp, nnratio, words, out);
    else hipLaunchKernelGGL(k_bow_select<false>, dim3((nitems + 3) / 4), dim3(256), smem, s, items, nitems, idx, desc, hmp, nnratio, words, out);
}
void orbx_launch_bow_rot(hipStream_t s, bool kk, int nproblems, int nout, const uint32_t *cand_base, const float *ang, int check,
                         int32_t *out, int32_t *counts) {
    if (nproblems <= 0) return;
    if (kk) hipLaunchKernelGGL(k_bow_rot<true>, dim3(nproblems), dim3(BOW_ROT_THREADS), 0, s, nout, cand_base, ang, check, out, counts);
    else hipLaunchKernelGGL(k_bow_rot<false>, dim3(nproblems), dim3(BOW_ROT_THREADS), 0, s, nout, cand_base, ang, check, out, counts);
}
size_t orbx_match_workspace_bytes(int npairs, int out_stride) { return (size_t)npairs * MT_SPLIT * out_stride * sizeof(uint2); }
void orbx_launch_match(hipStream_t s, int npairs, int max_nq, const uint8_t *q, const int *nq, long long q_stride,
                       const uint8_t *t, const int *nt, long long t_stride, int *best_idx, int *best_dist,
// ... 64 lines not shown
```

orb_slam2_detailed_comments_amd/csrc/orbx_launch.h:

```cpp
#pragma once
#include <hip/hip_runtime.h>
#include "orbx_device.h"

hipError_t orbx_upload_pattern();
size_t orbx_quadtree_smem(int ncap, int lds_keys);
hipError_t orbx_quadtree_prepare(size_t smem);
void orbx_launch_clear(hipStream_t s, int *a, int na, int *b, int nb, int *c, int nc);
void orbx_launch_pyr_l0(hipStream_t s, const DGeom &g, int B, const uint8_t *imgs, int W, int H, int stride,
                        long long frame_stride, uint8_t *pyr, int *status, int *cand_cursor);
void orbx_launch_pyr_l0_color(hipStream_t s, const DGeom &g, int B, const uint8_t *imgs, int W, int H, int stride,
                              long long frame_stride, uint8_t *pyr, int nch, int r_off, int b_off, int *status, int *cand_cursor);
void orbx_launch_pyr_l0_remap(hipStream_t s, const DGeom &g, int B, const uint8_t *imgs, int W, int H, int stride,
                              long long frame_stride, uint8_t *pyr, const uint2 *rect, int *status, int *cand_cursor);
void orbx_launch_pyr_resize(hipStream_t s, const DGeom &g, int B, int level, const OrbxTap *taps, uint8_t *pyr, bool narrow);
void orbx_launch_fast_rows(hipStream_t s, const DGeom &g, int B, const OrbxCell *cells, const OrbxFastGroup *groups,
                           int ngroups, const uint8_t *pyr, uint2 *cand, int *cand_cursor, int *status, int max_ch, int lcap,
                           int dbg_stop, int lds_floor = 0);
void orbx_launch_undistort(hipStream_t s, int B, int max_n, int cap, const double *K4, const double *k14, int identity,
                           const orbx_keypoint *kps, const int *counts, orbx_keypoint *out);
void orbx_launch_bow_transform(hipStream_t s, int B, int max_n, const int *child_begin, const uint32_t *child_ids,
                               const uint8_t *node_desc, int n_nodes, int L, const uint8_t *desc, const int *counts,
                               long long frame_stride, int levelsup, uint32_t *out_leaf, uint32_t *out_nid, int out_stride);
void orbx_launch_quadtree(hipStream_t s, const DGeom &g, int B, const uint2 *dense, const int *cand_count, uint32_t *lvl_kp, int *lvl_count,
                          int *status, uint16_t *knode_glob, int ncap, int lds_keys, int level_begin, int level_count);
void orbx_launch_blur(hipStream_t s, const DGeom &g, int B, const uint8_t *pyr, uint8_t *blur);
void orbx_launch_describe(hipStream_t s, const DGeom &g, int B, const uint8_t *pyr, const uint32_t *lvl_kp,
                          const int *lvl_count, float *lvl_angle, orbx_keypoint *kps, uint8_t *desc,
                          int *counts, int *status, int cap);
void orbx_launch_match(hipStream_t s, int npairs, int max_nq, const uint8_t *q, const int *nq, long long q_stride,
                       const uint8_t *t, const int *nt, long long t_stride, int *best_idx, int *best_dist,
                       int *second_dist, int out_stride, void *workspace, int kernel);
size_t orbx_match_workspace_bytes(int npairs, int out_stride);
void orbx_launch_grid_build(hipStream_t s, const DGrid &gp, int nframes, const orbx_keypoint *kps, const int *counts, int fixed_n,
                            int cap, int *cell_begin, uint16_t *items);
void orbx_launch_gate(hipStream_t s, const DGrid &gp, const orbx_keypoint *kps, const uint8_t *desc, const int *cell_begin,
                      const uint16_t *items, const DGateQuery *q, const uint8_t *qdesc, int nq, uint2 *span, uint32_t *cursor,
                      uint32_t *out_items, uint32_t cap, int fstride);
void orbx_launch_block_dist(hipStream_t s, const uint8_t *d1, const uint8_t *d2, const DDistRow *rows, const uint32_t *col_idx,
                            int nrows, uint16_t *out);
void orbx_launch_bow_select(hipStream_t s, bool kk, const DBowItem *items, int nitems, const uint32_t *idx, const uint8_t *desc,
                            const uint8_t *hmp, float nnratio, int words, int32_t *out);
void orbx_launch_bow_rot(hipStream_t s, bool kk, int nproblems, int nout, const uint32_t *cand_base, const float *ang, int check,
                         int32_t *out, int32_t *counts);
void orbx_launch_hamming_matrix(hipStream_t s, const uint8_t *q, int nq, const uint8_t *t, int nt, uint16_t *dist);

void orbx_launch_stereo_batch(hipStream_t s, const OrbxStereoGeom &sg, int npairs, int cap, const orbx_keypoint *kL,
                              const uint8_t *dL, const int *nL, const orbx_keypoint *kR, const uint8_t *dR, const int *nR,
                              const uint8_t *pyrL, const uint8_t *pyrR, long long pyr_bytes, float *uRight, float *depth,
                              int *sad, int *nmatches, int *row_begin, uint2 *row_items);
int orbx_stereo_items_per_pair(const OrbxStereoGeom &sg, int cap);
void orbx_launch_stereo(hipStream_t s, const OrbxStereoGeom &sg, const orbx_keypoint *kL, const uint8_t *dL, int nL,
                        const orbx_keypoint *kR, const uint8_t *dR, int nR, const uint8_t *pyrL, const uint8_t *pyrR,
                        float *uRight, float *depth, int *sad, int *row_begin, uint2 *row_items);
```

orb_slam2_detailed_comments_amd/extractor.py:

```python
from __future__ import annotations
import ctypes as C
import numpy as np
from . import _capi
from ._capi import KP_DTYPE, Params, check, ptr, lib


class ORBextractor:
    HARRIS_SCORE, FAST_SCORE = 0, 1

    def __init__(self, nfeatures=1000, scaleFactor=1.2, nlevels=8, iniThFAST=20, minThFAST=7, *,
                 fp_mode=_capi.FP_GCC_FMA, device=-1, max_batch=1, max_cand_per_cell=0):
        self._L = lib()
        p = Params()
        self._L.orbx_default_params(C.byref(p))
        p.nfeatures, p.scale_factor, p.nlevels = int(nfeatures), float(scaleFactor), int(nlevels)
        p.ini_th_fast, p.min_th_fast = int(iniThFAST), int(minThFAST)
        p.fp_mode, p.device, p.max_batch, p.max_cand_per_cell = fp_mode, device, max_batch, max_cand_per_cell
        self.params = p
        self._h = C.c_void_p()
        check(self._L.orbx_create(C.byref(p), C.byref(self._h)))
        self.nfeatures, self.nlevels, self.max_batch = int(nfeatures), int(nlevels), int(max_batch)

    def close(self):
        if getattr(self, "_h", None):
            self._L.orbx_destroy(self._h)
            self._h = None

    __del__ = close

    @property
    def handle(self):
        return self._h

    def GetLevels(self):
        return self._L.orbx_get_levels(self._h)

    def GetScaleFactor(self):
        return self._L.orbx_get_scale_factor(self._h)

    def _tables(self):
        n = self.nlevels
        t = [np.zeros(n, np.float32) for _ in range(4)]
        check(self._L.orbx_get_scale_tables(self._h, *[ptr(a) for a in t]))
        return t

    def GetScaleFactors(self):
        return self._tables()[0]

    def GetInverseScaleFactors(self):
        return self._tables()[1]

    def GetScaleSigmaSquares(self):
        return self._tables()[2]

    def GetInverseScaleSigmaSquares(self):
        return self._tables()[3]

    def features_per_level(self):
        a = np.zeros(self.nlevels, np.int32)
        check(self._L.orbx_get_features_per_level(self._h, ptr(a)))
        return a

    def umax(self):
        a = np.zeros(16, np.int32)
        check(self._L.orbx_get_umax(self._h, ptr(a)))
        return a

    def max_keypoints(self, width, height):
        n = self._L.orbx_max_keypoints(self._h, width, height)
        if n < 0:
            raise _capi.OrbxError(-n, self._L.orbx_last_error().decode())
        return n

    def set_input_format(self, fmt):
        check(self._L.orbx_set_input_format(self._h, int(fmt)))
        self._nch = 1 if fmt == _capi.FMT_GRAY8 else 3 if fmt in (_capi.FMT_RGB8, _capi.FMT_BGR8) else 4

    def __call__(self, image, mask=None):
        if image is None or image.size == 0:
            return None, None
        img = np.ascontiguousarray(image)
        nch = getattr(self, "_nch", 1)
        assert img.dtype == np.uint8 and (img.ndim == 2 if nch == 1 else (img.ndim == 3 and img.shape[2] == nch)), \
            "image.type() == CV_8UC1 (src/ORBextractor.cc:1972), or the colour format set with set_input_format"
        h, w = img.shape[:2]
        cap = self.max_keypoints(w, h)
        kps = np.zeros(cap, KP_DTYPE)
        desc = np.zeros((cap, 32), np.uint8)
        n = C.c_int(0)
        check(self._L.orbx_extract(self._h, ptr(img), w, h, img.strides[0], ptr(kps), ptr(desc), cap, C.byref(n)))
        return kps[:n.value].copy(), desc[:n.value].copy()

    def extract_batch(self, images):
        imgs = np.ascontiguousarray(images)
        assert imgs.dtype == np.uint8 and imgs.ndim == 3
        b, h, w = imgs.shape
        cap = self.max_keypoints(w, h)
        kps = np.zeros((b, cap), KP_DTYPE)
        desc = np.zeros((b, cap, 32), np.uint8)
        counts = np.zeros(b, np.int32)
        check(self._L.orbx_extract_batch(self._h, b, ptr(imgs), w, h, imgs.strides[1], imgs.strides[0], ptr(kps),
                                         ptr(desc), ptr(counts), cap))
        return [(kps[i, :counts[i]].copy(), desc[i, :counts[i]].copy()) for i in range(b)]

    def set_rectification(self, map_x=None, map_y=None):
        if map_x is None:
            check(self._L.orbx_set_rectification(self._h, None, None, 0, 0))
            return
        mx, my = np.ascontiguousarray(map_x, np.float32), np.ascontiguousarray(map_y, np.float32)
        assert mx.shape == my.shape and mx.ndim == 2
        check(self._L.orbx_set_rectification(self._h, ptr(mx), ptr(my), mx.shape[1], mx.shape[0]))

    def extract_batch_device(self, d_imgs, nframes, width, height, stride, frame_stride, d_kps, d_desc, d_counts,
                             d_status, cap):
        check(self._L.orbx_extract_batch_device(self._h, nframes, ptr(d_imgs), width, height, stride, frame_stride,
                                                ptr(d_kps), ptr(d_desc), ptr(d_counts), ptr(d_status), cap))

    def pyramid_level(self, level, frame=0, blur=False):
        w, h, p = C.c_int(), C.c_int(), C.c_int()
        check(self._L.orbx_pyramid_level_info(self._h, level, C.byref(w), C.byref(h), C.byref(p)))
        out = np.zeros((h.value, w.value), np.uint8)
        fn = self._L.orbx_debug_blur_copy if blur else self._L.orbx_pyramid_level_copy
        check(fn(self._h, frame, level, ptr(out), w.value))
        return out

    def debug_candidates(self, level, frame=0, cap=1 << 16):
        out = np.zeros(cap, KP_DTYPE)
        n = C.c_int(0)
        check(self._L.orbx_debug_candidates(self._h, frame, level, ptr(out), cap, C.byref(n)))
        return out[:n.value].copy()

    def debug_level_keypoints(self, level, frame=0, cap=1 << 14):
        out = np.zeros(cap, KP_DTYPE)
        n = C.c_int(0)
        check(self._L.orbx_debug_level_keypoints(self._h, frame, level, ptr(out), cap, C.byref(n)))
        return out[:n.value].copy()

    def stream(self):
        return self._L.orbx_get_stream(self._h)

    def set_stream(self, s):
        check(self._L.orbx_set_stream(self._h, C.c_void_p(s) if s else None))

    def synchronize(self):
        check(self._L.orbx_synchronize(self._h))

    def profile_enable(self, mask):
        check(self._L.orbx_profile_enable(self._h, mask))

    def profile_read(self, reset=True):
        ms = np.zeros(_capi.K_COUNT, np.float32)
        n = np.zeros(_capi.K_COUNT, np.int32)
        check(self._L.orbx_profile_read(self._h, ptr(ms), ptr(n), 1 if reset else 0))
        return {k: (float(ms[i]), int(n[i])) for i, k in enumerate(_capi.K_NAMES)}
```

Baseline: 335,100 frames/s.

## Read pyramid level 0 directly from input frames instead of copying to padded slab

Adds an in-place level-0 mode in which device-resident gray input frames are used directly as pyramid level 0. Consumers (level-1 resize, FAST, describe, stereo) apply reflect-101 border handling on the fly, and the padded copy is built lazily only when debug or pyramid-access APIs need it. This removes the level-0 copy kernel and its full-frame write and read traffic. In exchange, kernels that touch level 0 gain border-index arithmetic, the output depends on the input buffer staying alive, and a fallback path is kept for colour, rectified or misaligned inputs.

```diff
diff --git a/orb_slam2_detailed_comments_amd/csrc/orbx_api.cpp b/orb_slam2_detailed_comments_amd/csrc/orbx_api.cpp
--- a/orb_slam2_detailed_comments_amd/csrc/orbx_api.cpp
+++ b/orb_slam2_detailed_comments_amd/csrc/orbx_api.cpp
@@ -41,6 +41,11 @@
     bool pipe_head = true;
     bool fast_room = false;
     hipEvent_t ev_pipe[ORBX_PIPE_MAX] = {};
+    bool l0_inplace = true;
+    uint8_t *d_l0 = nullptr;
+    DL0View l0_view = {};
+    const uint8_t *l0_src = nullptr; int l0_src_stride = 0; int64_t l0_src_fstride = 0;
+    bool l0_padded_ready = false;
     uint8_t *d_pyr = nullptr, *d_blur = nullptr;
     OrbxCell *d_cells = nullptr;
     OrbxFastGroup *d_groups = nullptr;
@@ -161,7 +166,8 @@
 
 static void free_geometry_buffers(orbx_handle *h) {
     hipFree(h->d_groups); h->d_groups = nullptr;
-    hipFree(h->d_pyr); hipFree(h->d_blur); hipFree(h->d_cells); hipFree(h->d_taps);
+    hipFree(h->d_pyr); hipFree(h->d_blur); hipFree(h->d_cells); hipFree(h->d_taps); hipFree(h->d_l0);
+    h->d_l0 = nullptr; h->l0_view = DL0View{}; h->l0_src = nullptr; h->l0_padded_ready = false;
     hipFree(h->d_dense); h->d_dense = nullptr;
     hipFree(h->d_cand_count); hipFree(h->d_lvl_count); hipFree(h->d_status); hipFree(h->d_lvl_kp);
     hipFree(h->d_lvl_angle); hipFree(h->d_knode);
@@ -182,7 +188,9 @@
     }
     const char *why = "";
     OrbxGeom g;
-    orbx_status st = orbx_build_geometry(h->p, h->tab, width, height, g, &why);
+    h->l0_inplace = true;
+    if (const char *e = getenv("ORBX_L0_INPLACE")) h->l0_inplace = atoi(e) != 0;
+    orbx_status st = orbx_build_geometry(h->p, h->tab, width, height, g, &why, !h->l0_inplace);
     if (st != ORBX_OK) return fail(st, why);
     h->geom = g;
     const int B = h->p.max_batch, NL = h->p.nlevels;
@@ -425,38 +433,86 @@
     h->input_format = pixel_format;
     return ORBX_OK;
 }
+static orbx_status padded_l0_view(orbx_handle *h, DL0View &v) {
+    const OrbxGeom &G = h->geom;
+    if (G.l0_in_slab) {
+        v = DL0View{h->d_pyr + G.lv[0].off, (long long)G.pyr_bytes, G.lv[0].pitch, 0, G.width, G.height};
+        return ORBX_OK;
+    }
+    if (!h->d_l0) {
+        HIPCHK(hipMalloc(&h->d_l0, (size_t)h->p.max_batch * G.l0_bytes + 256));
+        HIPCHK(hipMemsetAsync(h->d_l0, 0, (size_t)h->p.max_batch * G.l0_bytes + 256, h->stream));
+    }
+    v = DL0View{h->d_l0, (long long)G.l0_bytes, G.lv[0].pitch, 0, G.width, G.height};
+    return ORBX_OK;
+}
+static orbx_status padded_l0(orbx_handle *h, DL0View &v) {
+    if (!h->l0_view.raw) { v = h->l0_view; return ORBX_OK; }
+    orbx_status st = padded_l0_view(h, v);
+    if (st != ORBX_OK) return st;
+    if (!h->l0_padded_ready) {
+        DGeom gm = h->dg;
+        gm.l0 = v;
+        { ProfScope ps(h, ORBX_K_PYR_L0);
+          orbx_launch_pyr_l0(h->stream, gm, h->last_batch, h->l0_src, h->geom.width, h->geom.height, h->l0_src_stride,
+                             h->l0_src_fstride, h->d_l0, nullptr, nullptr); }
+        HIPCHK(hipGetLastError());
+        h->l0_padded_ready = true;
+    }
+    return ORBX_OK;
+}
+
 static orbx_status run_chunk(orbx_handle *h, int B, const uint8_t *d_imgs, int W, int H, int stride,
                              int64_t frame_stride, orbx_keypoint *d_kps, uint8_t *d_desc, int32_t *d_counts,
-                             int32_t *d_status, int cap) {
-    const DGeom &g = h->dg;
+                             int32_t *d_status, int cap, bool may_inplace = false) {
     hipStream_t s = h->stream;
-    const int NL = g.nlevels;
+    const int NL = h->dg.nlevels;
     if (h->d_rect && (h->rect_w != W || h->rect_h != H))
         return fail(ORBX_BAD_ARGUMENT, "rectification maps were set for another image size (raw and rectified size must agree)");
     const int ngroups = (int)h->geom.fast_groups.size();
+    const bool fork = h->fork_level > 0 && (long long)B * ngroups >= 16384;
+    const bool raw = h->l0_inplace && may_inplace && !h->d_rect && h->input_format == ORBX_FMT_GRAY8 && NL >= 2 &&
+                     h->geom.narrow1_raw && h->geom.lv[1].narrow_taps && !h->resize_legacy && !(fork && h->fork_level == 1) &&
+                     W >= 20 && H >= 20 && ((uintptr_t)d_imgs & 3) == 0 && (stride & 3) == 0 && (frame_stride & 3) == 0;
+    DGeom gb = h->dg;
+    if (raw) {
+        gb.l0 = DL0View{d_imgs, (long long)frame_stride, stride, 1, W, H};
+        gb.lv[1].tapx = h->geom.tap1x_raw;
+        gb.lv[1].tapy = h->geom.tap1y_raw;
+    } else {
+        orbx_status st = padded_l0_view(h, gb.l0);
+        if (st != ORBX_OK) return st;
+    }
+    h->l0_view = gb.l0;
+    h->l0_src = d_imgs; h->l0_src_stride = stride; h->l0_src_fstride = frame_stride;
+    h->l0_padded_ready = !raw;
+    auto gsub = [&](int f0) { DGeom r = gb; r.l0.base += (long long)f0 * r.l0.fstride; return r; };
+    const DGeom &g = gb;
     auto pyramid = [&](hipStream_t st, int f0, int b, int l_end) {
         const uint8_t *im = d_imgs + (int64_t)f0 * frame_stride;
         uint8_t *pyr = h->d_pyr + (size_t)f0 * h->geom.pyr_bytes;
         int32_t *stp = d_status + f0;
         int *cc = h->d_cand_count + (size_t)f0 * NL;
-        { ProfScope ps(h, ORBX_K_PYR_L0, st);
+        const DGeom g = gsub(f0);
+        uint8_t *l0 = const_cast<uint8_t *>(g.l0.base);
+        if (!raw) { ProfScope ps(h, ORBX_K_PYR_L0, st);
           if (h->d_rect) {
-              orbx_launch_pyr_l0_remap(st, g, b, im, W, H, stride, frame_stride, pyr, h->d_rect, stp, cc);
+              orbx_launch_pyr_l0_remap(st, g, b, im, W, H, stride, frame_stride, l0, h->d_rect, stp, cc);
           } else if (h->input_format == ORBX_FMT_GRAY8) {
-              orbx_launch_pyr_l0(st, g, b, im, W, H, stride, frame_stride, pyr, stp, cc);
+              orbx_launch_pyr_l0(st, g, b, im, W, H, stride, frame_stride, l0, stp, cc);
           } else {
               const int nch = (h->input_format == ORBX_FMT_RGB8 || h->input_format == ORBX_FMT_BGR8) ? 3 : 4;
               const bool rgb = h->input_format == ORBX_FMT_RGB8 || h->input_format == ORBX_FMT_RGBA8;
-              orbx_launch_pyr_l0_color(st, g, b, im, W, H, stride, frame_stride, pyr, nch, rgb ? 0 : 2, rgb ? 2 : 0, stp, cc);
+              orbx_launch_pyr_l0_color(st, g, b, im, W, H, stride, frame_stride, l0, nch, rgb ? 0 : 2, rgb ? 2 : 0, stp, cc);
           } }
         for (int l = 1; l < l_end; ++l) {
             ProfScope ps(h, ORBX_K_PYR_RESIZE, st);
-            orbx_launch_pyr_resize(st, g, b, l, h->d_taps, pyr, h->geom.lv[l].narrow_taps && !h->resize_legacy);
+            orbx_launch_pyr_resize(st, g, b, l, h->d_taps, pyr, h->geom.lv[l].narrow_taps && !h->resize_legacy, stp, cc);
         }
     };
     auto fast = [&](hipStream_t st, int f0, int b, int g0, int ng, int lds_floor) {
         ProfScope ps(h, ORBX_K_FAST, st);
-        orbx_launch_fast_rows(st, g, b, h->d_cells, h->d_groups + g0, ng, h->d_pyr + (size_t)f0 * h->geom.pyr_bytes,
+        orbx_launch_fast_rows(st, gsub(f0), b, h->d_cells, h->d_groups + g0, ng, h->d_pyr + (size_t)f0 * h->geom.pyr_bytes,
                               h->d_dense + (size_t)f0 * g.cand_total, h->d_cand_count + (size_t)f0 * NL, d_status + f0, h->max_ch,
                               h->fast_lcap, h->fast_stop, lds_floor);
     };
@@ -466,7 +522,7 @@
                                h->d_lvl_kp + (size_t)f0 * g.kp_total, h->d_lvl_count + (size_t)f0 * NL, d_status + f0,
                                h->d_knode + (size_t)f0 * g.cand_total, h->ncap, (long long)b * NL >= 1024 ? h->lds_keys : h->lds_keys_few, 0, NL); }
         { ProfScope ps(h, ORBX_K_DESC);
-          orbx_launch_describe(s, g, b, h->d_pyr + (size_t)f0 * h->geom.pyr_bytes, h->d_lvl_kp + (size_t)f0 * g.kp_total,
+          orbx_launch_describe(s, gsub(f0), b, h->d_pyr + (size_t)f0 * h->geom.pyr_bytes, h->d_lvl_kp + (size_t)f0 * g.kp_total,
                                h->d_lvl_count + (size_t)f0 * NL, h->d_lvl_angle + (size_t)f0 * g.kp_total, d_kps + (int64_t)f0 * cap,
                                d_desc + (int64_t)f0 * cap * 32, d_counts + f0, d_status + f0, cap); }
     };
@@ -501,7 +557,6 @@
         h->last_batch = B;
         return ORBX_OK;
     }
-    const bool fork = h->fork_level > 0 && (long long)B * ngroups >= 16384;
     pyramid(s, 0, B, fork ? h->fork_level : NL);
     if (fork) {
         hipStream_t s2 = h->side_stream;
@@ -539,7 +594,7 @@
         const int B = std::min(MB, nframes - f0);
         int32_t *stp = d_status ? d_status + f0 : h->d_status;
         st = run_chunk(h, B, d_imgs + (int64_t)f0 * frame_stride, width, height, stride, frame_stride,
-                       d_kps + (int64_t)f0 * cap, d_desc + (int64_t)f0 * cap * 32, d_counts + f0, stp, cap);
+                       d_kps + (int64_t)f0 * cap, d_desc + (int64_t)f0 * cap * 32, d_counts + f0, stp, cap, true);
         if (st != ORBX_OK) return st;
     }
     return ORBX_OK;
@@ -730,37 +785,63 @@
 extern "C" orbx_status orbx_pyramid_level_device(orbx_handle *h, int frame, int level, const uint8_t **d_ptr) {
     orbx_status st = check_level(h, frame, level);
     if (st != ORBX_OK) return st;
+    if (level == 0) {
+        HIPCHK(hipSetDevice(h->dev));
+        DL0View v;
+        st = padded_l0(h, v);
+        if (st != ORBX_OK) return st;
+        *d_ptr = v.base + (size_t)frame * (size_t)v.fstride;
+        return ORBX_OK;
+    }
     *d_ptr = h->d_pyr + (size_t)frame * h->geom.pyr_bytes + h->geom.lv[level].off;
     return ORBX_OK;
 }
-static orbx_status copy_level(orbx_handle *h, const uint8_t *slab, int frame, int level, uint8_t *dst, int dst_stride) {
+static orbx_status copy_level(orbx_handle *h, const uint8_t *slab, const uint8_t *l0, long long l0_fstride, int frame, int level,
+                              uint8_t *dst, int dst_stride) {
     orbx_status st = check_level(h, frame, level);
     if (st != ORBX_OK) return st;
     const OrbxLevelGeom &L = h->geom.lv[level];
     if (!dst || dst_stride < L.pw) return fail(ORBX_BAD_ARGUMENT, "dst / dst_stride");
     HIPCHK(hipSetDevice(h->dev));
     HIPCHK(hipStreamSynchronize(h->stream));
-    HIPCHK(hipMemcpy2D(dst, dst_stride, slab + (size_t)frame * h->geom.pyr_bytes + L.off, L.pitch, L.pw, L.ph,
-                       hipMemcpyDeviceToHost));
+    const uint8_t *src = level == 0 ? l0 + (size_t)frame * (size_t)l0_fstride : slab + (size_t)frame * h->geom.pyr_bytes + L.off;
+    HIPCHK(hipMemcpy2D(dst, dst_stride, src, L.pitch, L.pw, L.ph, hipMemcpyDeviceToHost));
     return ORBX_OK;
 }
 extern "C" orbx_status orbx_pyramid_level_copy(orbx_handle *h, int frame, int level, uint8_t *dst, int dst_stride) {
-    return copy_level(h, h ? h->d_pyr : nullptr, frame, level, dst, dst_stride);
+    orbx_status st = check_level(h, frame, level);
+    if (st != ORBX_OK) return st;
+    DL0View v = h->l0_view;
+    if (level == 0) {
+        HIPCHK(hipSetDevice(h->dev));
+        st = padded_l0(h, v);
+        if (st != ORBX_OK) return st;
+    }
+    return copy_level(h, h->d_pyr, v.base, v.fstride, frame, level, dst, dst_stride);
 }
 extern "C" orbx_status orbx_debug_blur_copy(orbx_handle *h, int frame, int level, uint8_t *dst, int dst_stride) {
     orbx_status st = check_level(h, frame, level);
     if (st != ORBX_OK) return st;
+    const size_t l0_part = h->geom.l0_in_slab ? 0 : (size_t)h->p.max_batch * h->geom.l0_bytes;
+    HIPCHK(hipSetDevice(h->dev));
+    DL0View v;
+    st = padded_l0(h, v);
+    if (st != ORBX_OK) return st;
+    uint8_t *blur0 = nullptr;
+    if (h->d_blur) blur0 = h->geom.l0_in_slab ? h->d_blur + h->geom.lv[0].off : h->d_blur + (size_t)h->p.max_batch * h->geom.pyr_bytes;
     if (!h->blur_valid) {
-        HIPCHK(hipSetDevice(h->dev));
         if (!h->d_blur) {
-            HIPCHK(hipMalloc(&h->d_blur, (size_t)h->p.max_batch * h->geom.pyr_bytes + 256));
-            HIPCHK(hipMemsetAsync(h->d_blur, 0, (size_t)h->p.max_batch * h->geom.pyr_bytes, h->stream));
-        }
+            HIPCHK(hipMalloc(&h->d_blur, (size_t)h->p.max_batch * h->geom.pyr_bytes + l0_part + 256));
+            HIPCHK(hipMemsetAsync(h->d_blur, 0, (size_t)h->p.max_batch * h->geom.pyr_bytes + l0_part, h->stream));
+            blur0 = h->geom.l0_in_slab ? h->d_blur + h->geom.lv[0].off : h->d_blur + (size_t)h->p.max_batch * h->geom.pyr_bytes;
+        }
+        DGeom gm = h->dg;
+        gm.l0 = v;
         { ProfScope ps(h, ORBX_K_BLUR);
-          orbx_launch_blur(h->stream, h->dg, h->last_batch, h->d_pyr, h->d_blur); }
+          orbx_launch_blur(h->stream, gm, h->last_batch, h->d_pyr, h->d_blur, blur0); }
         h->blur_valid = true;
     }
-    return copy_level(h, h->d_blur, frame, level, dst, dst_stride);
+    return copy_level(h, h->d_blur, blur0, v.fstride, frame, level, dst, dst_stride);
 }
 
 extern "C" orbx_status orbx_debug_candidates(orbx_handle *h, int frame, int level, orbx_keypoint *out, int cap, int *n) {
@@ -1322,7 +1403,7 @@
     st = check_level(hr, frame_right, 0);
     if (st != ORBX_OK) return st;
     if (hl->dev != hr->dev || hl->geom.width != hr->geom.width || hl->geom.height != hr->geom.height ||
-        hl->p.nlevels != hr->p.nlevels || hl->p.scale_factor != hr->p.scale_factor)
+        hl->p.nlevels != hr->p.nlevels || hl->p.scale_factor != hr->p.scale_factor || hl->geom.pyr_bytes != hr->geom.pyr_bytes)
         return fail(ORBX_BAD_ARGUMENT, "left and right extractor must share device, image size and pyramid parameters");
     if (nmatches_out) *nmatches_out = 0;
     if (nl == 0) return ORBX_OK;
@@ -1336,6 +1417,8 @@
         sg.pw[l] = hl->geom.lv[l].pw; sg.ph[l] = hl->geom.lv[l].ph; sg.pitch[l] = hl->geom.lv[l].pitch;
         sg.off[l] = hl->geom.lv[l].off;
     }
+    sg.l0[0] = hl->l0_view; sg.l0[0].base += (long long)frame_left * sg.l0[0].fstride;
+    sg.l0[1] = hr->l0_view; sg.l0[1].base += (long long)frame_right * sg.l0[1].fstride;
     st = scratch_reserve(hl, pad256((size_t)nl * sizeof(orbx_keypoint)) + pad256((size_t)nl * 32) +
                                  pad256((size_t)std::max(nr, 1) * sizeof(orbx_keypoint)) + pad256((size_t)std::max(nr, 1) * 32) +
                                  3 * pad256((size_t)nl * sizeof(float)) + pad256((size_t)(sg.nrows0 + 1) * sizeof(int)) +
@@ -1394,7 +1477,7 @@
     st = check_level(hr, npairs - 1, 0);
     if (st != ORBX_OK) return st;
     if (hl->dev != hr->dev || hl->geom.width != hr->geom.width || hl->geom.height != hr->geom.height ||
-        hl->p.nlevels != hr->p.nlevels || hl->p.scale_factor != hr->p.scale_factor)
+        hl->p.nlevels != hr->p.nlevels || hl->p.scale_factor != hr->p.scale_factor || hl->geom.pyr_bytes != hr->geom.pyr_bytes)
         return fail(ORBX_BAD_ARGUMENT, "left and right extractor must share device, image size and pyramid parameters");
     HIPCHK(hipSetDevice(hl->dev));
     const bool two_streams = hr->stream != hl->stream;
@@ -1410,6 +1493,9 @@
         sg.pw[l] = hl->geom.lv[l].pw; sg.ph[l] = hl->geom.lv[l].ph; sg.pitch[l] = hl->geom.lv[l].pitch;
         sg.off[l] = hl->geom.lv[l].off;
     }
+    sg.l0[0] = hl->l0_view;
+    sg.l0[1] = hr->l0_view;
+    if (one_batch) sg.l0[1].base += (long long)npairs * sg.l0[1].fstride;
     const size_t ipp = (size_t)orbx_stereo_items_per_pair(sg, cap);
     st = scratch_reserve(hl, pad256((size_t)npairs * cap * sizeof(int)) + pad256((size_t)npairs * (sg.nrows0 + 1) * sizeof(int)) +
                                  pad256((size_t)npairs * ipp * sizeof(uint2)));
diff --git a/orb_slam2_detailed_comments_amd/csrc/orbx_device.h b/orb_slam2_detailed_comments_amd/csrc/orbx_device.h
--- a/orb_slam2_detailed_comments_amd/csrc/orbx_device.h
+++ b/orb_slam2_detailed_comments_amd/csrc/orbx_device.h
@@ -17,12 +17,19 @@
     long long cand_begin;
 };
 
+struct DL0View {
+    const uint8_t *base;
+    long long fstride;
+    int pitch, raw, w, h;
+};
+
 struct DGeom {
     int nlevels, ncells, kp_total, fp_mode;
     int ini_th, min_th, blur_tiles, pad0;
     long long pyr_bytes, cand_total;
     int umax[16];
     DLevel lv[ORBX_MAX_LEVELS];
+    DL0View l0;
 };
 
 struct OrbxStereoGeom {
@@ -31,6 +38,7 @@
     float scale[ORBX_MAX_LEVELS], inv_scale[ORBX_MAX_LEVELS];
     int pw[ORBX_MAX_LEVELS], ph[ORBX_MAX_LEVELS], pitch[ORBX_MAX_LEVELS];
     long long off[ORBX_MAX_LEVELS];
+    DL0View l0[2];
 };
 
 struct DGrid { float minx, miny, winv, hinv; };
@@ -44,6 +52,11 @@
     if (n == 1) return 0;
     while (i < 0 || i >= n) i = i < 0 ? -i : 2 * (n - 1) - i;
     return i;
+}
+
+__device__ __forceinline__ uint32_t orbx_l0_px(const DL0View &v, const uint8_t *b, int X, int Y) {
+    if (!v.raw) return b[(long long)Y * v.pitch + X];
+    return b[(long long)orbx_reflect101(Y - ORBX_EDGE, v.h) * v.pitch + orbx_reflect101(X - ORBX_EDGE, v.w)];
 }
 
 #define ORBX_DPP_ROW_SHR(n) (0x110 + (n))
diff --git a/orb_slam2_detailed_comments_amd/csrc/orbx_geometry.cpp b/orb_slam2_detailed_comments_amd/csrc/orbx_geometry.cpp
--- a/orb_slam2_detailed_comments_amd/csrc/orbx_geometry.cpp
+++ b/orb_slam2_detailed_comments_amd/csrc/orbx_geometry.cpp
@@ -71,9 +71,10 @@
 }
 
 orbx_status orbx_build_geometry(const orbx_params &p, const OrbxTables &t, int width, int height, OrbxGeom &g,
-                                const char **why) {
+                                const char **why, bool l0_in_slab) {
     g = OrbxGeom();
     g.width = width; g.height = height; g.nlevels = p.nlevels;
+    g.l0_in_slab = l0_in_slab;
     int64_t off = 0, cand_off = 0;
     int kp_off = 0;
     for (int l = 0; l < p.nlevels; ++l) {
@@ -84,9 +85,12 @@
         L.pw = L.sw + 2 * ORBX_EDGE;
         L.ph = L.sh + 2 * ORBX_EDGE;
         L.pitch = (L.pw + 63) & ~63;
+        if (l == 0) g.l0_bytes = ((int64_t)L.pitch * L.ph + 255) & ~(int64_t)255;
         L.off = off;
-        off += (int64_t)L.pitch * L.ph;
-        off = (off + 255) & ~(int64_t)255;
+        if (l > 0 || l0_in_slab) {
+            off += (int64_t)L.pitch * L.ph;
+            off = (off + 255) & ~(int64_t)255;
+        }
         L.scale = t.scale[l];
         L.size = (float)(int)(ORBX_PATCH * t.scale[l]);
         L.nfeat = t.nfeat[l];
@@ -164,6 +168,31 @@
                 }
                 if (hi + 2 - lo > 8) L.narrow_taps = false;
             }
+            if (l == 1) {
+                g.tap1x_raw = (int)g.taps.size();
+                for (int X = 0; X < L.pw; ++X) {
+                    OrbxTap t = g.taps[L.tapx_begin + X];
+                    t.s0 = (int16_t)reflect101(t.s0 - ORBX_EDGE, width);
+                    t.s1 = (int16_t)reflect101(t.s1 - ORBX_EDGE, width);
+                    g.taps.push_back(t);
+                }
+                g.tap1y_raw = (int)g.taps.size();
+                for (int Y = 0; Y < L.ph; ++Y) {
+                    OrbxTap t = g.taps[L.tapy_begin + Y];
+                    t.s0 = (int16_t)reflect101(t.s0 - ORBX_EDGE, height);
+                    t.s1 = (int16_t)reflect101(t.s1 - ORBX_EDGE, height);
+                    g.taps.push_back(t);
+                }
+                g.narrow1_raw = true;
+                for (int X = 0; X < L.pw; X += 4) {
+                    int lo = 0x7fff, hi = 0;
+                    for (int i = 0; i < 4; ++i) {
+                        const OrbxTap &t = g.taps[g.tap1x_raw + std::min(X + i, L.pw - 1)];
+                        lo = std::min<int>({lo, t.s0, t.s1}); hi = std::max<int>({hi, t.s0, t.s1});
+                    }
+                    if (hi - lo > 7) g.narrow1_raw = false;
+                }
+            }
         }
     }
     for (size_t i = 0; i < g.cells.size();) {
diff --git a/orb_slam2_detailed_comments_amd/csrc/orbx_internal.h b/orb_slam2_detailed_comments_amd/csrc/orbx_internal.h
--- a/orb_slam2_detailed_comments_amd/csrc/orbx_internal.h
+++ b/orb_slam2_detailed_comments_amd/csrc/orbx_internal.h
@@ -60,6 +60,10 @@
     std::vector<OrbxFastGroup> fast_groups;
     std::vector<OrbxTap> taps;
     int64_t pyr_bytes = 0;
+    bool l0_in_slab = true;
+    int64_t l0_bytes = 0;
+    int tap1x_raw = 0, tap1y_raw = 0;
+    bool narrow1_raw = false;
     int64_t cand_total = 0;
     int kp_total = 0;
     int node_cap = 0;
@@ -74,4 +78,4 @@
 
 void orbx_build_tables(const orbx_params &p, OrbxTables &t);
 orbx_status orbx_build_geometry(const orbx_params &p, const OrbxTables &t, int width, int height, OrbxGeom &g,
-                                const char **why);
+                                const char **why, bool l0_in_slab = true);
diff --git a/orb_slam2_detailed_comments_amd/csrc/orbx_kernels.hip b/orb_slam2_detailed_comments_amd/csrc/orbx_kernels.hip
--- a/orb_slam2_detailed_comments_amd/csrc/orbx_kernels.hip
+++ b/orb_slam2_detailed_comments_amd/csrc/orbx_kernels.hip
@@ -20,14 +20,14 @@
 #else
     const int f = blockIdx.z, bx = blockIdx.x, by = blockIdx.y, nbx = gridDim.x;
 #endif
-    if (bx == 0 && by == 0 && threadIdx.y == 0) {
+    if (status && bx == 0 && by == 0 && threadIdx.y == 0) {
         if (threadIdx.x == 0) status[f] = 0;
         if ((int)threadIdx.x < g.nlevels) cand_cursor[f * g.nlevels + threadIdx.x] = 0;
     }
     const int Y0 = (by * 4 + threadIdx.y) * L0_ROWS;
     if (Y0 >= L.ph) return;
     const uint8_t *img = imgs + (long long)f * frame_stride;
-    uint8_t *dst = pyr + (long long)f * g.pyr_bytes + L.off;
+    uint8_t *dst = pyr + (long long)f * g.l0.fstride;
     if (bx + 1 < nbx) {
         const int X = 32 + (bx * 64 + threadIdx.x) * 16;
         if (X >= xe) return;
@@ -73,7 +73,7 @@
     const int X = (blockIdx.x * 64 + threadIdx.x) * 4;
     const int Y = blockIdx.y * 4 + threadIdx.y;
     const int f = blockIdx.z;
-    if (blockIdx.x == 0 && blockIdx.y == 0 && threadIdx.y == 0) {
+    if (status && blockIdx.x == 0 && blockIdx.y == 0 && threadIdx.y == 0) {
         if (threadIdx.x == 0) status[f] = 0;
         if ((int)threadIdx.x < g.nlevels) cand_cursor[f * g.nlevels + threadIdx.x] = 0;
     }
@@ -90,7 +90,7 @@
         }
         v |= p << (8 * i);
     }
-    *(uint32_t *)(pyr + (long long)f * g.pyr_bytes + L.off + (long long)Y * L.pitch + X) = v;
+    *(uint32_t *)(pyr + (long long)f * g.l0.fstride + (long long)Y * L.pitch + X) = v;
 }
 
 __global__ __launch_bounds__(256) void k_pyr_l0_remap(DGeom g, const uint8_t *__restrict__ imgs, int W, int H, int stride,
@@ -101,7 +101,7 @@
     const int X = (blockIdx.x * 64 + threadIdx.x) * 4;
     const int Y = blockIdx.y * 4 + threadIdx.y;
     const int f = blockIdx.z;
-    if (blockIdx.x == 0 && blockIdx.y == 0 && threadIdx.y == 0) {
+    if (status && blockIdx.x == 0 && blockIdx.y == 0 && threadIdx.y == 0) {
         if (threadIdx.x == 0) status[f] = 0;
         if ((int)threadIdx.x < g.nlevels) cand_cursor[f * g.nlevels + threadIdx.x] = 0;
     }
@@ -127,7 +127,7 @@
         }
         v |= p << (8 * i);
     }
-    *(uint32_t *)(pyr + (long long)f * g.pyr_bytes + L.off + (long long)Y * L.pitch + X) = v;
+    *(uint32_t *)(pyr + (long long)f * g.l0.fstride + (long long)Y * L.pitch + X) = v;
 }
 
 struct __attribute__((packed, aligned(1))) orbx_uint2_u { uint32_t x, y; };
@@ -148,6 +148,7 @@
     const int f = blockIdx.z;
     if (X >= L.pw || Y0 >= L.ph) return;
     uint8_t *base = pyr + (long long)f * g.pyr_bytes;
+    const uint8_t *sbase = level == 1 ? g.l0.base + (long long)f * g.l0.fstride : base + S.off;
     OrbxTap tx[4];
     int smin = 0x7fff, smax = 0;
 #pragma unroll
@@ -169,8 +170,8 @@
 #pragma unroll
         for (int r = 0; r < RS_ROWS; ++r) {
             ty[r] = taps[L.tapy + min(Y0 + r, L.ph - 1)];
-            u[r] = orbx_load8(base + S.off + (long long)ty[r].s0 * S.pitch + smin);
-            w[r] = orbx_load8(base + S.off + (long long)ty[r].s1 * S.pitch + smin);
+            u[r] = orbx_load8(sbase + (long long)ty[r].s0 * S.pitch + smin);
+            w[r] = orbx_load8(sbase + (long long)ty[r].s1 * S.pitch + smin);
         }
 #pragma unroll
         for (int r = 0; r < RS_ROWS; ++r) {
@@ -196,8 +197,8 @@
     for (int r = 0; r < RS_ROWS; ++r) {
         ty[r] = taps[L.tapy + min(Y0 + r, L.ph - 1)];
         if (windowed) {
-            const uint32_t *q0 = (const uint32_t *)(base + S.off + (long long)ty[r].s0 * S.pitch + xb);
-            const uint32_t *q1 = (const uint32_t *)(base + S.off + (long long)ty[r].s1 * S.pitch + xb);
+            const uint32_t *q0 = (const uint32_t *)(sbase + (long long)ty[r].s0 * S.pitch + xb);
+            const uint32_t *q1 = (const uint32_t *)(sbase + (long long)ty[r].s1 * S.pitch + xb);
             u[r][0] = q0[0]; u[r][1] = q0[1]; u[r][2] = q0[2];
             w[r][0] = q1[0]; w[r][1] = q1[1]; w[r][2] = q1[2];
         }
@@ -222,8 +223,8 @@
                 v |= p << (8 * i);
             }
         } else {
-            const uint8_t *r0 = base + S.off + (long long)ty[r].s0 * S.pitch;
-            const uint8_t *r1 = base + S.off + (long long)ty[r].s1 * S.pitch;
+            const uint8_t *r0 = sbase + (long long)ty[r].s0 * S.pitch;
+            const uint8_t *r1 = sbase + (long long)ty[r].s1 * S.pitch;
 #pragma unroll
             for (int i = 0; i < 4; ++i) {
                 const int T0 = r0[tx[i].s0] * tx[i].a0 + r0[tx[i].s1] * tx[i].a1;
@@ -243,23 +244,30 @@
 #define RR_WPB 1
 #endif
 __global__ __launch_bounds__(64 * RR_WPB) void k_pyr_resize_rows(DGeom g, int level, const OrbxTap *__restrict__ taps,
-                                                         uint8_t *__restrict__ pyr, int rpw) {
+                                                         uint8_t *__restrict__ pyr, int rpw, int *__restrict__ status,
+                                                         int *__restrict__ cand_cursor) {
     const DLevel &L = g.lv[level];
     const DLevel &S = g.lv[level - 1];
     const int lane = threadIdx.x;
+    const bool RAW = level == 1 && g.l0.raw;
 #if RR_FF
     const int f = blockIdx.x, bx = blockIdx.y;
     const int by = (RR_REVERSE && (level & 1)) ? (int)gridDim.z - 1 - (int)blockIdx.z : (int)blockIdx.z;
 #else
     const int f = blockIdx.z, bx = blockIdx.x, by = blockIdx.y;
 #endif
+    if (RAW && blockIdx.y == 0 && blockIdx.z == 0 && threadIdx.y == 0) {
+        if (lane == 0) status[f] = 0;
+        if (lane < g.nlevels) cand_cursor[f * g.nlevels + lane] = 0;
+    }
     const int X = (bx * 64 + lane) * 4;
     const int y_begin = __builtin_amdgcn_readfirstlane((by * RR_WPB + threadIdx.y) * rpw);
     if (y_begin >= L.ph) return;
     const int y_end = min(y_begin + rpw, L.ph);
     const bool on = X < L.pw;
     uint8_t *base = pyr + (long long)f * g.pyr_bytes;
-    const uint8_t *src = base + S.off;
+    const uint8_t *src = level == 1 ? g.l0.base + (long long)f * g.l0.fstride : base + S.off;
+    const uint32_t spitch = (uint32_t)(level == 1 ? g.l0.pitch : S.pitch);
     uint8_t *dst = base + L.off;
     const uint32_t ldst = (uint32_t)X;
     uint32_t sel[4], wgt[4];
@@ -270,16 +278,27 @@
 #pragma unroll
         for (int i = 0; i < 4; ++i) t[i] = tq[min(X + i, L.pw - 1)];
 #pragma unroll
-        for (int i = 0; i < 4; ++i) smin = min(smin, (int)(t[i].x & 0xffffu));
+        for (int i = 0; i < 4; ++i) smin = min(smin, min((int)(t[i].x & 0xffffu), (int)(t[i].x >> 16)));
 #pragma unroll
         for (int i = 0; i < 4; ++i) {
-            const uint32_t d = (t[i].x & 0xffffu) - (uint32_t)smin;
-            sel[i] = d | (0x0cu << 8) | ((d + 1u) << 16) | (0x0cu << 24);
+            const uint32_t d0 = (t[i].x & 0xffffu) - (uint32_t)smin, d1 = (t[i].x >> 16) - (uint32_t)smin;
+            sel[i] = d0 | (0x0cu << 8) | (d1 << 16) | (0x0cu << 24);
             wgt[i] = t[i].y;
         }
     }
     const uint32_t sh = (uint32_t)(smin & 3);
-    const uint32_t lsrc = (uint32_t)(smin & ~3);
+    uint32_t lsrc = (uint32_t)(smin & ~3);
+    uint32_t kd = 0;
+    if (RAW) {
+        const int lim = (g.l0.w + 3) & ~3;
+        if ((int)lsrc + 12 > lim) { kd = (uint32_t)((int)lsrc + 12 - lim) >> 2; lsrc -= 4u * kd; }
+    }
+#define RR_FIX(v)                                                                                                       \
+    if (RAW) {                                                                                                          \
+        (v).x = kd == 0 ? (v).x : kd == 1 ? (v).y : (v).z;                                                            \
+        (v).y = kd == 0 ? (v).y : kd == 1 ? (v).z : 0u;                                                                \
+        (v).z = kd == 0 ? (v).z : 0u;                                                                                  \
+    }
     const uint2 *ty = (const uint2 *)taps + L.tapy;
 #ifndef RR_R
 #define RR_R 2
@@ -304,8 +323,12 @@
     for (int r = 0; r < RR_R; ++r) {
         t[r] = ty[min(y_begin + r, L.ph - 1)];
         u[r].x = u[r].y = u[r].z = 0;
-        if (r == 0 || (int)(t[r].x & 0xffffu) != (int)(t[r - 1].x >> 16)) u[r] = *(const orbx_uint3_a *)(src + (uint32_t)((t[r].x & 0xffffu) * (uint32_t)S.pitch + lsrc));
-        w[r] = *(const orbx_uint3_a *)(src + (uint32_t)((t[r].x >> 16) * (uint32_t)S.pitch + lsrc));
+        if (r == 0 || (int)(t[r].x & 0xffffu) != (int)(t[r - 1].x >> 16)) {
+            u[r] = *(const orbx_uint3_a *)(src + (uint32_t)((t[r].x & 0xffffu) * spitch + lsrc));
+            RR_FIX(u[r])
+        }
+        w[r] = *(const orbx_uint3_a *)(src + (uint32_t)((t[r].x >> 16) * spitch + lsrc));
+        RR_FIX(w[r])
     }
     for (int Y = y_begin; Y < y_end; Y += RR_R) {
         uint2 ct[RR_R];
@@ -318,8 +341,12 @@
             for (int r = 0; r < RR_R; ++r) {
                 t[r] = ty[min(Y + RR_R + r, L.ph - 1)];
                 const int s0 = (int)(t[r].x & 0xffffu), s1 = (int)(t[r].x >> 16);
-                if (s0 != last) u[r] = *(const orbx_uint3_a *)(src + (uint32_t)((uint32_t)s0 * (uint32_t)S.pitch + lsrc));
-                w[r] = *(const orbx_uint3_a *)(src + (uint32_t)((uint32_t)s1 * (uint32_t)S.pitch + lsrc));
+                if (s0 != last) {
+                    u[r] = *(const orbx_uint3_a *)(src + (uint32_t)((uint32_t)s0 * spitch + lsrc));
+                    RR_FIX(u[r])
+                }
+                w[r] = *(const orbx_uint3_a *)(src + (uint32_t)((uint32_t)s1 * spitch + lsrc));
+                RR_FIX(w[r])
                 last = s1;
             }
         }
@@ -337,6 +364,7 @@
     }
 #undef RR_H
 #undef RR_V
+#undef RR_FIX
 }
 
 __device__ __forceinline__ bool orbx_arc9(uint32_t mask16) {
@@ -613,6 +641,28 @@
     }
 }
 
+template <bool ALIGNED = true>
+__device__ __forceinline__ orbx_uint3_u fr_l0_piece(const DL0View &v, const uint8_t *b, int yr, int cx) {
+    const int ry = yr < 0 ? -yr : yr >= v.h ? 2 * v.h - 2 - yr : yr;
+    const uint8_t *row = b + (long long)ry * v.pitch;
+    orbx_uint3_u out;
+    if (cx >= 0 && cx + 12 <= v.w) {
+        if (!ALIGNED) return *(const orbx_uint3_u *)(row + cx);
+        const orbx_uint3_a a = *(const orbx_uint3_a *)(row + cx);
+        out.x = a.x; out.y = a.y; out.z = a.z;
+        return out;
+    }
+    uint32_t d[3] = {0u, 0u, 0u};
+#pragma unroll
+    for (int i = 0; i < 12; ++i) {
+        int c = cx + i;
+        c = c < 0 ? -c : c >= v.w ? 2 * v.w - 2 - c : c;
+        d[i >> 2] |= (uint32_t)row[c] << (8 * (i & 3));
+    }
+    out.x = d[0]; out.y = d[1]; out.z = d[2];
+    return out;
+}
+
 __global__ __launch_bounds__(64, FR_WPS) void k_fast_rows(DGeom g, const OrbxCell *__restrict__ cells,
                                                           const OrbxFastGroup *__restrict__ groups,
                                                           const uint8_t *__restrict__ pyr, uint2 *__restrict__ cand,
@@ -636,17 +686,31 @@
     OrbxFastGroup grp_n = groups[g0];
     OrbxCell c0_n = cells[grp_n.cell0], c1_n = cells[grp_n.cell0 + grp_n.ncell - 1];
     const uint8_t *fbase = pyr + (long long)f * g.pyr_bytes;
+    const uint8_t *l0b = g.l0.base + (long long)f * g.l0.fstride;
 #define FR_PREFETCH()                                                                                                     \
     {                                                                                                                     \
         const DLevel &Ln = g.lv[c0_n.level];                                                                             \
-        const uint8_t *srcn = fbase + Ln.off;                                                                             \
-        uint32_t vpitch9 = (uint32_t)(9 * Ln.pitch);                                                                      \
-        asm("" : "+v"(vpitch9));                      \
-        const uint32_t olast = (uint32_t)(__mul24((int)c0_n.y0 + (int)c0_n.ch - 1, Ln.pitch) + (c0_n.x0 & ~3) + 12 * dq); \
-        uint32_t o = (uint32_t)(__mul24((int)c0_n.y0 + min(rq, 8), Ln.pitch) + (c0_n.x0 & ~3) + 12 * dq);                \
-        _Pragma("unroll") for (int k = 0; k < 5; ++k) {                                                                   \
-            tv[k] = *(const orbx_uint3_u *)(srcn + min(o, olast));                                                        \
-            o += vpitch9;                                                                                                 \
+        const bool l0n = c0_n.level == 0;                                                                                 \
+        const int lpitch = l0n ? g.l0.pitch : Ln.pitch;                                                                   \
+        const uint8_t *srcn = l0n ? l0b : fbase + Ln.off;                                                                 \
+        int xo = c0_n.x0, yo = c0_n.y0;                                                                                   \
+        bool lin = true;                                                                                                  \
+        if (l0n && g.l0.raw) {                                                                                            \
+            xo -= ORBX_EDGE; yo -= ORBX_EDGE;                                                                             \
+            lin = (xo & ~3) >= 0 && (xo & ~3) + 84 <= g.l0.w && yo >= 0 && yo + (int)c0_n.ch <= g.l0.h;                  \
+        }                                                                                                                 \
+        if (lin) {                                                                                                        \
+            uint32_t vpitch9 = (uint32_t)(9 * lpitch);                                                                    \
+            asm("" : "+v"(vpitch9));                  \
+            const uint32_t olast = (uint32_t)(__mul24(yo + (int)c0_n.ch - 1, lpitch) + (xo & ~3) + 12 * dq);              \
+            uint32_t o = (uint32_t)(__mul24(yo + min(rq, 8), lpitch) + (xo & ~3) + 12 * dq);                              \
+            _Pragma("unroll") for (int k = 0; k < 5; ++k) {                                                               \
+                tv[k] = *(const orbx_uint3_u *)(srcn + min(o, olast));                                                    \
+                o += vpitch9;                                                                                             \
+            }                                                                                                             \
+        } else {                                                                                                          \
+            _Pragma("unroll") for (int k = 0; k < 5; ++k)                                                                 \
+                tv[k] = fr_l0_piece(g.l0, l0b, yo + min(min(rq, 8) + 9 * k, (int)c0_n.ch - 1), (xo & ~3) + 12 * dq);     \
         }                                                                                                                 \
     }
     FR_PREFETCH()
@@ -669,10 +733,13 @@
             }
         }
         if (th_rows > 45) {
-            const uint8_t *src = fbase + L.off + (long long)c0.y0 * L.pitch + xa + 12 * dq;
+            const bool l0 = c0.level == 0, raw = l0 && g.l0.raw;
+            const int lpitch = l0 ? g.l0.pitch : L.pitch;
+            const uint8_t *src = (l0 ? l0b : fbase + L.off) + (long long)c0.y0 * lpitch + xa + 12 * dq;
             for (int r = 45 + rq; r < th_rows; r += 9) {
                 if (rq < 9) {
-                    const orbx_uint3_u v = *(const orbx_uint3_u *)(src + (long long)r * L.pitch);
+                    const orbx_uint3_u v = raw ? fr_l0_piece(g.l0, l0b, c0.y0 - ORBX_EDGE + r, ((c0.x0 - ORBX_EDGE) & ~3) + 12 * dq)
+                                               : *(const orbx_uint3_u *)(src + (long long)r * lpitch);
                     uint32_t *d = s_tile + r * (FR_TP / 4) + 3 * dq;
                     d[0] = v.x;
                     if (dq < 6) { d[1] = v.y; d[2] = v.z; }
@@ -687,7 +754,7 @@
         FR_PREFETCH()
     }
     FrCtx cx;
-    cx.tile = (const uint8_t *)s_tile + (c0.x0 & 3);
+    cx.tile = (const uint8_t *)s_tile + ((c0.level == 0 && g.l0.raw ? c0.x0 - ORBX_EDGE : c0.x0) & 3);
     cx.score = s_score;
     cx.list = s_list;
     cx.corn = s_corn;
@@ -1109,7 +1176,8 @@
 #define BL_TH 32
 #define BL_SD ((BL_TW + 8) / 4)
 #define BL_ROWS (BL_TH + 6)
-__global__ __launch_bounds__(256) void k_blur(DGeom g, const uint8_t *__restrict__ pyr, uint8_t *__restrict__ blur) {
+__global__ __launch_bounds__(256) void k_blur(DGeom g, const uint8_t *__restrict__ pyr, uint8_t *__restrict__ blur,
+                                              uint8_t *__restrict__ blur0) {
     __shared__ uint32_t s_src[BL_ROWS * BL_SD];
     __shared__ __attribute__((aligned(8))) uint16_t s_h[BL_ROWS * BL_TW];
     const int tid = threadIdx.x, f = blockIdx.y;
@@ -1120,7 +1188,7 @@
     const int t = blockIdx.x - L.blur_tile_begin;
     const int ty = t / L.blur_tx, tx = t - ty * L.blur_tx;
     const int X0 = tx * BL_TW, Y0 = ty * BL_TH;
-    const uint8_t *img = pyr + (long long)f * g.pyr_bytes + L.off;
+    const uint8_t *img = level == 0 ? g.l0.base + (long long)f * g.l0.fstride : pyr + (long long)f * g.pyr_bytes + L.off;
     for (int i = tid; i < BL_ROWS * BL_SD; i += 256) {
         const int r = i / BL_SD, d = i - r * BL_SD;
         const int sy = orbx_reflect101(Y0 + r - 3, L.ph);
@@ -1167,7 +1235,7 @@
         const uint2 v = *(const uint2 *)(s_h + (rg * 4 + r) * BL_TW + 4 * cg);
         hh[r][0] = v.x & 0xffff; hh[r][1] = v.x >> 16; hh[r][2] = v.y & 0xffff; hh[r][3] = v.y >> 16;
     }
-    uint8_t *out = blur + (long long)f * g.pyr_bytes + L.off;
+    uint8_t *out = level == 0 ? blur0 + (long long)f * g.l0.fstride : blur + (long long)f * g.pyr_bytes + L.off;
 #pragma unroll
     for (int j = 0; j < 4; ++j) {
         const int Y = Y0 + rg * 4 + j;
@@ -1301,18 +1369,22 @@
     const int4 pat = c_pattern_lane[lane];
     const DLevel &L = g.lv[level];
     const int x = (int)(pos & 0xfff) + (ORBX_EDGE - 3), y = (int)((pos >> 12) & 0xfff) + (ORBX_EDGE - 3);
-    const uint8_t *img = pyr + (long long)f * g.pyr_bytes + L.off;
+    const bool l0 = level == 0, raw = l0 && g.l0.raw;
+    const uint8_t *img = l0 ? g.l0.base + (long long)f * g.l0.fstride : pyr + (long long)f * g.pyr_bytes + L.off;
+    const int ipitch = l0 ? g.l0.pitch : L.pitch;
     const int px0 = x - DS_R, py0 = y - DS_R;
-    const int xa = px0 & ~3;
-    const bool interior = px0 >= 0 && py0 >= 0 && xa + 48 <= L.pitch && x + DS_R < L.pw && y + DS_R < L.ph;
+    const int ex0 = raw ? px0 - ORBX_EDGE : px0, ey0 = raw ? py0 - ORBX_EDGE : py0;
+    const int xa = ex0 & ~3;
+    const bool interior = raw ? ex0 >= 0 && ey0 >= 0 && xa + 48 <= g.l0.w && ey0 + 2 * DS_R < g.l0.h
+                              : px0 >= 0 && py0 >= 0 && xa + 48 <= L.pitch && x + DS_R < L.pw && y + DS_R < L.ph;
     {
         if (interior) {
             const int dq = lane & 3, rq = lane >> 2;
-            const uint32_t shift = (uint32_t)(px0 & 3);
-            const uint8_t *p0 = img + (__mul24(py0, L.pitch) + xa + 12 * dq);
+            const uint32_t shift = (uint32_t)(ex0 & 3);
+            const uint8_t *p0 = img + (__mul24(ey0, ipitch) + xa + 12 * dq);
             orbx_uint3_u tv[3];
 #pragma unroll
-            for (int k = 0; k < 3; ++k) tv[k] = *(const orbx_uint3_u *)(p0 + __mul24(min(16 * k + rq, DS_W - 1), L.pitch));
+            for (int k = 0; k < 3; ++k) tv[k] = *(const orbx_uint3_u *)(p0 + __mul24(min(16 * k + rq, DS_W - 1), ipitch));
 #pragma unroll
             for (int k = 0; k < 3; ++k) {
                 const uint32_t nxt = orbx_lane_above(tv[k].x);
@@ -1326,10 +1398,16 @@
             }
         } else {
             uint8_t *pb = (uint8_t *)patch;
-            for (int i = lane; i < DS_W * DS_W; i += 64) {
-                const int r = i / DS_W, c = i - r * DS_W;
-                const int sy = orbx_reflect101(py0 + r, L.ph), sx = orbx_reflect101(px0 + c, L.pw);
-                pb[r * DS_PP + c] = img[(long long)sy * L.pitch + sx];
+            int sx = 0;
+            if (lane < DS_W) {
+                sx = orbx_reflect101(px0 + lane, L.pw);
+                if (raw) sx = orbx_reflect101(sx - ORBX_EDGE, g.l0.w);
+            }
+#pragma unroll 4
+            for (int r = 0; r < DS_W; ++r) {
+                int sy = orbx_reflect101(py0 + r, L.ph);
+                if (raw) sy = orbx_reflect101(sy - ORBX_EDGE, g.l0.h);
+                if (lane < DS_W) pb[r * DS_PP + lane] = img[(long long)sy * ipitch + sx];
             }
         }
         orbx_wave_sync();
@@ -1905,6 +1983,7 @@
                                                  const orbx_keypoint *__restrict__ kR,
                                                  const uint8_t *__restrict__ dR, int nR,
                                                  const uint8_t *__restrict__ pyrL, const uint8_t *__restrict__ pyrR,
+                                                 const uint8_t *__restrict__ l0L, const uint8_t *__restrict__ l0R,
                                                  float *__restrict__ uRight, float *__restrict__ depth,
                                                  int *__restrict__ sad, const int *__restrict__ row_begin,
                                                  const uint2 *__restrict__ row_items) {
@@ -1973,10 +2052,19 @@
 #pragma unroll
     for (int s = 0; s < 11; ++s) acc[s] = 0u;
     if (act) {
-        const uint8_t *IL = pyrL + sg.off[levelL] + (long long)y0 * pitch + x0;
-        const uint8_t *IR = pyrR + sg.off[levelL] + (long long)y0 * pitch + ((int)scaleduR0 - w);
-        const uint32_t cL = IL[w * pitch + w];
-        const orbx_uint3_u cw = *(const orbx_uint3_u *)(IR + w * pitch);
+        const bool lz = levelL == 0, rawL = lz && sg.l0[0].raw, rawR = lz && sg.l0[1].raw;
+        const int pitchL = lz ? sg.l0[0].pitch : pitch, pitchR = lz ? sg.l0[1].pitch : pitch;
+        const uint8_t *bL = lz ? l0L : pyrL + sg.off[levelL], *bR = lz ? l0R : pyrR + sg.off[levelL];
+        const int xr0 = (int)scaleduR0 - w;
+        const uint8_t *IL = bL + (long long)y0 * pitchL + x0;
+        const uint8_t *IR = bR + (long long)y0 * pitchR + xr0;
+        auto pxL = [&](int yy, int xx) -> uint32_t { return rawL ? orbx_l0_px(sg.l0[0], bL, x0 + xx, y0 + yy) : IL[yy * pitchL + xx]; };
+        auto winR = [&](int yy, int xx) -> orbx_uint3_u {
+            return rawR ? fr_l0_piece<false>(sg.l0[1], bR, y0 + yy - ORBX_EDGE, xr0 + xx - ORBX_EDGE)
+                        : *(const orbx_uint3_u *)(IR + yy * pitchR + xx);
+        };
+        const uint32_t cL = pxL(w, w);
+        const orbx_uint3_u cw = winR(w, 0);
         uint32_t Cs[11];
 #pragma unroll
         for (int s = 0; s < 11; ++s) {
@@ -1988,9 +2076,9 @@
             int q0 = l16 + 16 * k, q1 = q0 + 64;
             if (q1 >= 121) q1 = 60;
             const int y_0 = q0 / 11, x_0 = q0 - 11 * y_0, y_1 = q1 / 11, x_1 = q1 - 11 * y_1;
-            const uint32_t L0 = IL[y_0 * pitch + x_0], L1 = IL[y_1 * pitch + x_1];
-            const orbx_uint3_u r0 = *(const orbx_uint3_u *)(IR + y_0 * pitch + x_0 - Lh);
-            const orbx_uint3_u r1 = *(const orbx_uint3_u *)(IR + y_1 * pitch + x_1 - Lh);
+            const uint32_t L0 = pxL(y_0, x_0), L1 = pxL(y_1, x_1);
+            const orbx_uint3_u r0 = winR(y_0, x_0 - Lh);
+            const orbx_uint3_u r1 = winR(y_1, x_1 - Lh);
             const uint32_t A0 = L0 | (L1 << 16);
 #pragma unroll
             for (int s = 0; s < 11; ++s) {
@@ -2033,7 +2121,7 @@
                                                 float *__restrict__ uRight, float *__restrict__ depth,
                                                 int *__restrict__ sad, const int *__restrict__ row_begin,
                                                 const uint2 *__restrict__ row_items) {
-    orbx_stereo_body(sg, kL, dL, nL, kR, dR, nR, pyrL, pyrR, uRight, depth, sad, row_begin, row_items);
+    orbx_stereo_body(sg, kL, dL, nL, kR, dR, nR, pyrL, pyrR, sg.l0[0].base, sg.l0[1].base, uRight, depth, sad, row_begin, row_items);
 }
 __global__ __launch_bounds__(256) void k_stereo_batch(OrbxStereoGeom sg, const orbx_keypoint *__restrict__ kL,
                                                       const uint8_t *__restrict__ dL, const int *__restrict__ nL,
@@ -2046,7 +2134,8 @@
                                                       int items_per_pair) {
     const long long p = blockIdx.y;
     orbx_stereo_body(sg, kL + p * cap, dL + p * cap * 32, min(nL[p], cap), kR + p * cap, dR + p * cap * 32, min(nR[p], cap),
-                     pyrL + p * pyr_bytes, pyrR + p * pyr_bytes, uRight + p * cap, depth + p * cap, sad + p * cap,
+                     pyrL + p * pyr_bytes, pyrR + p * pyr_bytes, sg.l0[0].base + p * sg.l0[0].fstride,
+                     sg.l0[1].base + p * sg.l0[1].fstride, uRight + p * cap, depth + p * cap, sad + p * cap,
                      row_begin ? row_begin + p * (sg.nrows0 + 1) : nullptr, row_items ? row_items + p * items_per_pair : nullptr);
 }
 #define ST_MAX_ROWS 4096
@@ -2582,7 +2671,8 @@
     dim3 grid((L.pw + 255) / 256, (L.ph + 3) / 4, B);
     hipLaunchKernelGGL(k_pyr_l0_remap, grid, dim3(64, 4), 0, s, g, imgs, W, H, stride, frame_stride, pyr, rect, status, cand_cursor);
 }
-void orbx_launch_pyr_resize(hipStream_t s, const DGeom &g, int B, int level, const OrbxTap *taps, uint8_t *pyr, bool narrow) {
+void orbx_launch_pyr_resize(hipStream_t s, const DGeom &g, int B, int level, const OrbxTap *taps, uint8_t *pyr, bool narrow,
+                            int *status, int *cand_cursor) {
     const DLevel &L = g.lv[level];
     if (narrow) {
         int rpw = 16;
@@ -2592,7 +2682,7 @@
 #else
         dim3 grid((L.pw + 255) / 256, (L.ph + RR_WPB * rpw - 1) / (RR_WPB * rpw), B);
 #endif
-        hipLaunchKernelGGL(k_pyr_resize_rows, grid, dim3(64, RR_WPB), 0, s, g, level, taps, pyr, rpw);
+        hipLaunchKernelGGL(k_pyr_resize_rows, grid, dim3(64, RR_WPB), 0, s, g, level, taps, pyr, rpw, status, cand_cursor);
         return;
     }
     dim3 grid((L.pw + 255) / 256, (L.ph + 4 * RS_ROWS - 1) / (4 * RS_ROWS), B);
@@ -2664,8 +2754,8 @@
     if (e == hipSuccess && dev >= 0 && dev < 64) cur[dev] = smem;
     return e;
 }
-void orbx_launch_blur(hipStream_t s, const DGeom &g, int B, const uint8_t *pyr, uint8_t *blur) {
-    hipLaunchKernelGGL(k_blur, dim3(g.blur_tiles, B), dim3(256), 0, s, g, pyr, blur);
+void orbx_launch_blur(hipStream_t s, const DGeom &g, int B, const uint8_t *pyr, uint8_t *blur, uint8_t *blur0) {
+    hipLaunchKernelGGL(k_blur, dim3(g.blur_tiles, B), dim3(256), 0, s, g, pyr, blur, blur0);
 }
 void orbx_launch_describe(hipStream_t s, const DGeom &g, int B, const uint8_t *pyr, const uint32_t *lvl_kp,
                           const int *lvl_count, float *lvl_angle, orbx_keypoint *kps, uint8_t *desc,
diff --git a/orb_slam2_detailed_comments_amd/csrc/orbx_launch.h b/orb_slam2_detailed_comments_amd/csrc/orbx_launch.h
--- a/orb_slam2_detailed_comments_amd/csrc/orbx_launch.h
+++ b/orb_slam2_detailed_comments_amd/csrc/orbx_launch.h
@@ -12,7 +12,8 @@
                               long long frame_stride, uint8_t *pyr, int nch, int r_off, int b_off, int *status, int *cand_cursor);
 void orbx_launch_pyr_l0_remap(hipStream_t s, const DGeom &g, int B, const uint8_t *imgs, int W, int H, int stride,
                               long long frame_stride, uint8_t *pyr, const uint2 *rect, int *status, int *cand_cursor);
-void orbx_launch_pyr_resize(hipStream_t s, const DGeom &g, int B, int level, const OrbxTap *taps, uint8_t *pyr, bool narrow);
+void orbx_launch_pyr_resize(hipStream_t s, const DGeom &g, int B, int level, const OrbxTap *taps, uint8_t *pyr, bool narrow,
+                            int *status = nullptr, int *cand_cursor = nullptr);
 void orbx_launch_fast_rows(hipStream_t s, const DGeom &g, int B, const OrbxCell *cells, const OrbxFastGroup *groups,
                            int ngroups, const uint8_t *pyr, uint2 *cand, int *cand_cursor, int *status, int max_ch, int lcap,
                            int dbg_stop, int lds_floor = 0);
@@ -23,7 +24,7 @@
                                long long frame_stride, int levelsup, uint32_t *out_leaf, uint32_t *out_nid, int out_stride);
 void orbx_launch_quadtree(hipStream_t s, const DGeom &g, int B, const uint2 *dense, const int *cand_count, uint32_t *lvl_kp, int *lvl_count,
                           int *status, uint16_t *knode_glob, int ncap, int lds_keys, int level_begin, int level_count);
-void orbx_launch_blur(hipStream_t s, const DGeom &g, int B, const uint8_t *pyr, uint8_t *blur);
+void orbx_launch_blur(hipStream_t s, const DGeom &g, int B, const uint8_t *pyr, uint8_t *blur, uint8_t *blur0);
 void orbx_launch_describe(hipStream_t s, const DGeom &g, int B, const uint8_t *pyr, const uint32_t *lvl_kp,
                           const int *lvl_count, float *lvl_angle, orbx_keypoint *kps, uint8_t *desc,
                           int *counts, int *status, int cap);
diff --git a/orb_slam2_detailed_comments_amd/extractor.py b/orb_slam2_detailed_comments_amd/extractor.py
--- a/orb_slam2_detailed_comments_amd/extractor.py
+++ b/orb_slam2_detailed_comments_amd/extractor.py
@@ -23,6 +23,9 @@
 
     def close(self):
         if getattr(self, "_h", None):
+            if getattr(self, "_frames", None) is not None:
+                self._L.orbx_synchronize(self._h)
+                self._frames = None
             self._L.orbx_destroy(self._h)
             self._h = None
 
@@ -115,6 +118,7 @@
                              d_status, cap):
         check(self._L.orbx_extract_batch_device(self._h, nframes, ptr(d_imgs), width, height, stride, frame_stride,
                                                 ptr(d_kps), ptr(d_desc), ptr(d_counts), ptr(d_status), cap))
+        self._frames = d_imgs
 
     def pyramid_level(self, level, frame=0, blur=False):
         w, h, p = C.c_int(), C.c_int(), C.c_int()
```

Result: no change. 335,200 frames/s, median of 6 (+0.0%).
